# mlvlab/RPO

Measured on AMD Instinct MI355X. Metric: images/sec (train step, ViT-B/16 K=24), higher is better.
Workload: dtype bf16

## Files before the change

### include/rpo_amd.h

```cpp
#ifndef RPO_AMD_H
#define RPO_AMD_H

#include <stddef.h>
#include <stdint.h>

#if defined(__GNUC__)
#pragma GCC visibility push(default)
#endif
#ifdef __cplusplus
extern "C" {
#endif

#define RPO_ABI_VERSION 8

enum { RPO_F32 = 0, RPO_BF16 = 1, RPO_F16 = 2 };

enum {
  RPO_E_BADARG = -1,
  RPO_E_SHAPE = -2,
  RPO_E_DTYPE = -3,
  RPO_E_ALIGN = -4,
  RPO_E_WORKSPACE = -5,
  RPO_E_JPEG_CORRUPT = -20,
  RPO_E_JPEG_PROGRESSIVE = -21,
// ... 33 lines not shown
  int32_t group;
  int32_t split_k;
  int64_t split_stride;
  int32_t tile_config;
  void* out2; int64_t ldout2;
  float* ln_stats;
  const float* ln_colsum;
  float ln_eps;
  int32_t seg_rows0, seg_rows1, seg1_row0;
  int32_t ln_group;
  int32_t aux_dtype;
  const void* prefetch;
  int64_t prefetch_bytes;
  const void* resid_hi; const void* resid_lo; int64_t ldr16;
  void* out_lo;
  int32_t c_row0;
} rpo_gemm_args;

int rpo_version(void);
const char* rpo_error_string(int code);

int rpo_gemm_nt(const rpo_gemm_args* args, void* stream);

int rpo_gemm_ws(const rpo_gemm_args* args, void* stream);
int rpo_gemm_ws_pack(const void* W, int64_t ldw, void* Wp, int N, int K, int dtype, void* stream);
int rpo_gemm_ws_ok(const rpo_gemm_args* args);

int rpo_gemm_stats_group(const rpo_gemm_args* args);

int rpo_gemm_hilo_ok(const rpo_gemm_args* args);

int rpo_gemm_nt_plan(const rpo_gemm_args* args);
int rpo_gemm_ws_plan(const rpo_gemm_args* args);

int rpo_layernorm_fwd(const float* x, int64_t ldx, const float* gamma, const float* beta,
                      void* y, int64_t ldy, int y_dtype, int rows, int d, float eps, void* stream);

int rpo_layernorm_bwd(const void* dy, int dy_dtype, int64_t lddy, const float* x, int64_t ldx,
                      const float* gamma, const float* dres, int64_t lddres,
                      float* dx, int64_t lddx, void* dx_cast, int cast_dtype, int64_t ldcast,
                      int rows, int d, float eps, int dy_splits, int64_t dy_split_stride, void* stream);

int rpo_im2col_patches(const float* img, void* out, int out_dtype, int64_t ldo,
                       int B, int H, int W, int patch, void* stream);

int rpo_img_assemble(float* x, int64_t ldx, const float* cls, const float* pos0,
                     const float* img_prompt, int B, int N, int Kp, int d, void* stream);

int rpo_img_embed_norm(float* x_pre, int64_t ldx, const float* cls, const float* pos0, const float* img_prompt,
                       const float* g_pre, const float* b_pre, float* x0, int64_t ldx0, const float* g1, const float* b1,
                       void* h, int64_t ldh, int h_dtype, int B, int N, int Kp, int d, float eps, void* stream);
int rpo_img_embed_norm_rows(float* x_pre, int64_t ldx, const float* cls, const float* pos0, const float* img_prompt,
                            const float* g_pre, const float* b_pre, float* x0, int64_t ldx0, const float* g1,
                            const float* b1, void* h, int64_t ldh, int h_dtype, int B, int N, int Kp, int d,
                            float eps, int row0, int row1, void* stream);

int rpo_img_embed_norm_grouped(float* x_pre, int64_t ldx, const float* cls, const float* pos0, const float* img_prompt,
                               const float* g_pre, const float* b_pre, float* x0, int64_t ldx0, const float* g1,
                               const float* b1, void* h, int64_t ldh, int h_dtype, int B, int N, int Kp, int d,
                               float eps, int row0, int row1, int images_per_group, int64_t prompt_stride, void* stream);

int rpo_broadcast_rows(const float* src, float* dst, int64_t ld, int groups, int rows, int d, void* stream);

int rpo_reduce_groups(const float* src, int64_t ld, float* out, int groups, int rows, int d, void* stream);

int rpo_broadcast_rows_sets(const float* src, int64_t src_set_stride, float* dst, int64_t ld, int sets, int groups, int rows,
                            int d, void* stream);
int rpo_reduce_groups_sets(const float* src, int64_t ld, float* out, int64_t out_set_stride, int sets, int groups, int rows,
                           int d, void* stream);

int rpo_attn_readonly_fwd(const void* q, const void* k, const void* v, int64_t ld,
                          void* out, int64_t ldo, int dtype, int B, int H, int N, int Kp,
                          float scale, void* stream);
int rpo_attn_readonly_fwd_rows(const void* q, const void* k, const void* v, int64_t ld,
                               void* out, int64_t ldo, int dtype, int B, int H, int N, int Kp, float scale,
                               int q_first, void* stream);

int rpo_attn_prompt_fwd(const void* q_rows, int64_t ldq, const void* k, const void* v, int64_t ldkv,
                        void* out, int64_t ldo, int dtype, int B, int H, int N, int Kp, int sets,
                        const int32_t* first_image, float scale, void* stream);

int rpo_attn_readonly_bwd(const void* q_rows, int64_t ldq, const void* k, const void* v, int64_t ldkv,
                          const void* da, int64_t ldda, void* dq, int64_t lddq, int dtype,
                          int B, int H, int N, int Kp, float scale, void* stream);

int rpo_attn_readonly_bwd_proj(const void* q_rows, int64_t ldq, const void* k, const void* v, int64_t ldkv,
                               const void* dx, int64_t lddx, const void* w_out_t, int64_t ldw, void* dq, int64_t lddq,
                               int dtype, int B, int H, int N, int Kp, float scale, void* stream);

int rpo_text_attn_fwd(const void* q, int64_t ldq, const void* kc, const void* vc, int64_t ldkv,
                      void* out, int64_t ldo, int dtype, const int32_t* len, int n_cls, int rows,
                      int Lmax, int H, int causal, float scale, void* stream);

int rpo_text_attn_bwd(const void* q, int64_t ldq, const void* kc, const void* vc, int64_t ldkv,
                      const void* da, int64_t ldda, void* dq, int64_t lddq, int dtype,
                      const int32_t* len, int n_cls, int rows, int Lmax, int H, float scale, void* stream);

int rpo_text_attn_fwd_shared(const void* q, int64_t ldq, const void* kc, const void* vc, int64_t ldkv,
                             void* out, int64_t ldo, int dtype, const int32_t* len, int n_cls, int n_kv, int rows,
                             int Lmax, int H, float scale, void* stream);
int rpo_text_attn_bwd_shared(const void* q, int64_t ldq, const void* kc, const void* vc, int64_t ldkv,
                             const void* da, int64_t ldda, void* dq, int64_t lddq, int dtype,
                             const int32_t* len, int n_cls, int n_kv, int rows, int Lmax, int H, float scale, void* stream);

int rpo_text_attn_bwd_dense(const void* q, const void* k, const void* v, int64_t ld, const void* d_out, int64_t lddo,
                            void* dq, void* dk, void* dv, int64_t ldd, int dtype, const int32_t* len, int n_cls,
                            int Lmax, int H, float scale, void* stream);

int rpo_metanet_fwd(const float* img_f, const float* w1, const float* b1, const float* w2, const float* b2,
                    float* f_norm, float* hidden, float* bias, int B, int e, int h, int d, void* stream);
int rpo_metanet_bwd(const float* d_bias, const float* f_norm, const float* hidden, const float* w2,
                    float* g_w1, float* g_b1, float* g_w2, float* g_b2, int B, int e, int h, int d, void* stream);

int64_t rpo_head_workspace_floats(int B, int C, int K, int e);
int rpo_head_fwd_bwd(const float* img_f, const float* text_f, const int64_t* label, float scale_exp,
                     float* logits, float* loss, float* d_img_f, float* d_text_f,
                     int B, int C, int K, int e, float* workspace, void* stream);
int rpo_head_fwd_bwd_act(const float* img_f, const float* text_f, const int64_t* label, float scale_exp,
                         float* logits, float* loss, float* d_img_f, float* d_text_f, void* d_img_f_act,
                         void* d_text_f_act, int act_dtype, int B, int C, int K, int e, float* workspace, void* stream);

int rpo_head_fwd_bwd_grouped(const float* img_f, const float* text_f, const int64_t* label, float scale_exp,
                             float* logits, float* loss, float* d_img_f, float* d_text_f,
                             int S, int B, int C, int K, int e, float* workspace, void* stream);
int rpo_head_fwd_bwd_grouped_act(const float* img_f, const float* text_f, const int64_t* label, float scale_exp,
                                 float* logits, float* loss, float* d_img_f, float* d_text_f, void* d_img_f_act,
                                 void* d_text_f_act, int act_dtype, int S, int B, int C, int K, int e, float* workspace,
                                 void* stream);

int64_t rpo_lp_head_workspace_floats(int B, int C, int e);
int rpo_lp_head_fwd_bwd(const float* img_f, const float* w, const float* bias, const float* text_f_n,
                        const int64_t* label, float scale_exp, float* z, float* logits, float* loss,
                        float* g_w, float* g_bias, int B, int C, int e, float* workspace, void* stream);

int rpo_eval_accumulate(const float* logits, int64_t ldl, const int64_t* label, int B, int C, int64_t* counts,
                        int32_t* cmat, int32_t* pred, void* stream);

int rpo_conv2d_plan(int B, int H, int W, int Cout);
int rpo_conv2d_nhwc(const void* x, const void* w, const float* bias, const void* resid, void* y, int dtype,
                    int B, int H, int W, int Cin, int Cout, int ksize, int relu, int tile_config, void* stream);
int rpo_conv_stem(const float* image, const void* w, const float* bias, void* y, int dtype, int B, int H, int W,
                  int Cout, int relu, void* stream);
int rpo_avgpool_nhwc(const void* x, void* y, int dtype, int B, int H, int W, int C, int k, void* stream);
int rpo_attnpool_tokens(const void* x, const float* pos, void* tokens, int dtype, int B, int HW, int C, void* stream);
int rpo_attnpool_attn(const float* q, int64_t ldq, const void* kv, void* out, int dtype, int B, int T, int C, int heads,
                      float scale, void* stream);

int rpo_sgd_step(float* p, const float* g, float* buf, int64_t n, float lr, float momentum, float wd,
                 float grad_scale, int first_step, void* stream);

int rpo_sgd_step_guarded(float* p, const float* g, float* buf, int64_t n, float lr, float momentum, float wd,
                         float grad_scale, int first_step, int32_t* found_inf, void* stream);

int rpo_convert(const float* src, int64_t lds, void* dst, int dst_dtype, int64_t ldd,
                int rows, int cols, void* stream);

int rpo_probe_mfma(int which, const float* a, const float* b, float* d, void* stream);

typedef struct rpo_image_desc {
  int64_t src_offset;
  int32_t width, height;
  int32_t crop_x, crop_y, crop_w, crop_h;
  int32_t resize_w, resize_h;
  int32_t win_x, win_y;
  int32_t flip;
  int32_t reserved;
} rpo_image_desc;

int rpo_preprocess_ksize(int in_size, int out_size);
size_t rpo_preprocess_workspace_bytes(int B, int size, int max_rows, int kmax);
int rpo_preprocess_batch(const uint8_t* src, int64_t src_bytes, const rpo_image_desc* desc_host,
                         const rpo_image_desc* desc_dev, int B, int size, int max_rows, int kmax,
                         const float* mean3, const float* std3, float* out, void* workspace,
                         size_t workspace_bytes, void* stream);

typedef struct rpo_jpeg_info {
  int32_t width, height;
  int32_t components;
  int32_t h_samp, v_samp;
  int32_t restart_interval;
  int32_t mcus_x, mcus_y;
  int32_t units;
  int32_t reserved;
  int64_t scan_offset;
  int64_t scan_bytes;
  int64_t table_bytes;
  int64_t coef_bytes;
} rpo_jpeg_info;

typedef struct rpo_jpeg_desc {
  int64_t file_offset;
  int64_t file_bytes;
  int64_t table_offset;
  int64_t out_offset;
  int64_t coef_offset;
  int32_t unit_base;
  int32_t reserved;
  rpo_jpeg_info info;
} rpo_jpeg_desc;

enum {
  RPO_JPEG_OK = 0,
  RPO_JPEG_TRUNCATED = 1,
  RPO_JPEG_BAD_CODE = 2,
  RPO_JPEG_BAD_INDEX = 3,
  RPO_JPEG_NO_RESTART = 4
};

int rpo_jpeg_probe(const uint8_t* file, int64_t nbytes, rpo_jpeg_info* info);
int rpo_jpeg_tables(const uint8_t* file, int64_t nbytes, void* blob, int64_t blob_bytes);
size_t rpo_jpeg_workspace_bytes(rpo_jpeg_desc* descs, int n);
int rpo_jpeg_decode_batch(const uint8_t* files, int64_t files_bytes, const rpo_jpeg_desc* desc_host,
                          const rpo_jpeg_desc* desc_dev, int n, uint8_t* out, int64_t out_bytes, void* workspace,
                          size_t workspace_bytes, int32_t* status, void* stream);

int rpo_jpeg_prog_probe(const uint8_t* file, int64_t nbytes, rpo_jpeg_info* info);
int rpo_jpeg_prog_plan(const uint8_t* file, int64_t nbytes, void* blob, int64_t blob_bytes);
size_t rpo_jpeg_prog_workspace_bytes(rpo_jpeg_desc* descs, int n);
int rpo_jpeg_prog_decode_batch(const uint8_t* files, int64_t files_bytes, const rpo_jpeg_desc* desc_host,
                               const rpo_jpeg_desc* desc_dev, int n, uint8_t* out, int64_t out_bytes, void* workspace,
                               size_t workspace_bytes, int32_t* status, void* stream);

int rpo_probe_peak_mfma(int which, int blocks, int iters, float* sink, double* flops, void* stream);
int rpo_probe_peak_copy(const void* src, void* dst, int64_t bytes, void* stream);

#ifdef __cplusplus
}
#endif
#if defined(__GNUC__)
#pragma GCC visibility pop
#endif

#ifdef RPO_EXPERIMENTAL
#include "rpo_amd_experimental.h"
#endif
#endif
```

### rpo_amd/_lib.py

```python
from __future__ import annotations

import ctypes as C
import os

_HERE = os.path.dirname(os.path.abspath(__file__))
LIB_PATH = os.path.join(_HERE, "librpo_hip.so")

RPO_F32, RPO_BF16, RPO_F16 = 0, 1, 2
EPI_NONE, EPI_BIAS, EPI_BIAS_QGELU, EPI_BIAS_RESID, EPI_QGELU_BWD, EPI_PATCH, EPI_LN_BIAS, EPI_LN_BIAS_QGELU = range(8)
E_BADARG, E_SHAPE, E_DTYPE, E_ALIGN, E_WORKSPACE = -1, -2, -3, -4, -5
(E_JPEG_CORRUPT, E_JPEG_PROGRESSIVE, E_JPEG_ARITHMETIC, E_JPEG_LOSSLESS, E_JPEG_PRECISION, E_JPEG_COMPONENTS, E_JPEG_RGB,
 E_JPEG_SAMPLING, E_JPEG_MULTISCAN, E_JPEG_SCRIPT, E_JPEG_SEQUENTIAL) = range(-20, -31, -1)

c_i64, c_i32, c_f32, c_vp = C.c_int64, C.c_int32, C.c_float, C.c_void_p


class ImageDesc(C.Structure):
    _fields_ = [("src_offset", c_i64), ("width", c_i32), ("height", c_i32),
                ("crop_x", c_i32), ("crop_y", c_i32), ("crop_w", c_i32), ("crop_h", c_i32),
                ("resize_w", c_i32), ("resize_h", c_i32), ("win_x", c_i32), ("win_y", c_i32),
                ("flip", c_i32), ("reserved", c_i32)]


class JpegInfo(C.Structure):
    _fields_ = [("width", c_i32), ("height", c_i32), ("components", c_i32), ("h_samp", c_i32), ("v_samp", c_i32),
                ("restart_interval", c_i32), ("mcus_x", c_i32), ("mcus_y", c_i32), ("units", c_i32), ("reserved", c_i32),
                ("scan_offset", c_i64), ("scan_bytes", c_i64), ("table_bytes", c_i64), ("coef_bytes", c_i64)]


class JpegDesc(C.Structure):
    _fields_ = [("file_offset", c_i64), ("file_bytes", c_i64), ("table_offset", c_i64), ("out_offset", c_i64),
                ("coef_offset", c_i64), ("unit_base", c_i32), ("reserved", c_i32), ("info", JpegInfo)]


class GemmArgs(C.Structure):
    _fields_ = [
        ("A", c_vp), ("lda", c_i64),
        ("W", c_vp), ("ldw", c_i64),
        ("C", c_vp), ("ldc", c_i64),
        ("M", c_i32), ("N", c_i32), ("K", c_i32),
        ("in_dtype", c_i32), ("out_dtype", c_i32), ("epilogue", c_i32),
        ("bias", c_vp),
        ("resid", c_vp), ("ldr", c_i64),
        ("aux", c_vp), ("ldaux", c_i64),
        ("aux_row0", c_i32),
        ("skip_row0", c_i32), ("skip_col0", c_i32),
        ("group", c_i32),
        ("split_k", c_i32),
        ("split_stride", c_i64),
        ("tile_config", c_i32),
        ("out2", c_vp), ("ldout2", c_i64),
        ("ln_stats", c_vp),
        ("ln_colsum", c_vp),
        ("ln_eps", c_f32),
        ("seg_rows0", c_i32), ("seg_rows1", c_i32), ("seg1_row0", c_i32),
        ("ln_group", c_i32),
        ("aux_dtype", c_i32),
        ("prefetch", c_vp), ("prefetch_bytes", c_i64),
        ("resid_hi", c_vp), ("resid_lo", c_vp), ("ldr16", c_i64),
        ("out_lo", c_vp),
        ("c_row0", c_i32),
    ]


class LnBwdArgs(C.Structure):
    _fields_ = [("dy", c_vp), ("lddy", c_i64), ("x", c_vp), ("ldx", c_i64), ("gamma", c_vp),
                ("dres", c_vp), ("lddres", c_i64), ("dx", c_vp), ("lddx", c_i64),
                ("dx_cast", c_vp), ("cast_dtype", c_i32), ("ldcast", c_i64),
                ("rows", c_i32), ("d", c_i32), ("eps", c_f32), ("dy_splits", c_i32), ("dy_split_stride", c_i64)]


class AttnBwdArgs(C.Structure):
    _fields_ = [("q_rows", c_vp), ("ldq", c_i64), ("k", c_vp), ("v", c_vp), ("ldkv", c_i64),
                ("dx", c_vp), ("lddx", c_i64), ("w_out_t", c_vp), ("ldw", c_i64), ("dq", c_vp), ("lddq", c_i64),
                ("groups", c_i32), ("H", c_i32), ("keys", c_i32), ("Kp", c_i32),
                ("key_len", c_vp), ("key_stride", c_i32), ("scale", c_f32)]


class ChainLayer(C.Structure):
    _fields_ = [("w_proj_t", c_vp), ("w_fc_t", c_vp), ("w_out_t", c_vp), ("w_q_t", c_vp), ("aux", c_vp),
                ("x_ln2", c_vp), ("x_ln1", c_vp), ("ln2_w", c_vp), ("ln1_w", c_vp),
                ("q_rows", c_vp), ("k", c_vp), ("v", c_vp)]


class ChainBwdArgs(C.Structure):
    _fields_ = [("layer", C.POINTER(ChainLayer)),
                ("layers", c_i32), ("units", c_i32), ("Kp", c_i32), ("d", c_i32), ("H", c_i32), ("keys", c_i32),
                ("dtype", c_i32),
                ("key_len", c_vp), ("key_stride", c_i32),
                ("ldx", c_i64), ("ldq", c_i64), ("ldkv", c_i64),
                ("dxa", c_vp), ("dxb", c_vp), ("dxc", c_vp), ("du", c_vp), ("dq", c_vp),
                ("dy", c_vp), ("dy_stride", c_i64),
                ("scale", c_f32), ("eps", c_f32),
                ("wgs_per_group", c_i32),
                ("state", c_vp),
                ("timeline", c_vp)]


SIGNATURES = {
    "rpo_version": (c_i32, []),
    "rpo_gemm_stats_group": (c_i32, [C.POINTER(GemmArgs)]),
    "rpo_gemm_hilo_ok": (c_i32, [C.POINTER(GemmArgs)]),
    "rpo_gemm_nt_plan": (c_i32, [C.POINTER(GemmArgs)]),
    "rpo_gemm_ws_plan": (c_i32, [C.POINTER(GemmArgs)]),
    "rpo_error_string": (C.c_char_p, [c_i32]),
    "rpo_gemm_nt": (c_i32, [C.POINTER(GemmArgs), c_vp]),
    "rpo_gemm_ws": (c_i32, [C.POINTER(GemmArgs), c_vp]),
    "rpo_gemm_ws_pack": (c_i32, [c_vp, c_i64, c_vp, c_i32, c_i32, c_i32, c_vp]),
    "rpo_gemm_ws_ok": (c_i32, [C.POINTER(GemmArgs)]),
    "rpo_layernorm_fwd": (c_i32, [c_vp, c_i64, c_vp, c_vp, c_vp, c_i64, c_i32, c_i32, c_i32, c_f32, c_vp]),
    "rpo_layernorm_bwd": (c_i32, [c_vp, c_i32, c_i64, c_vp, c_i64, c_vp, c_vp, c_i64, c_vp, c_i64, c_vp,
                                  c_i32, c_i64, c_i32, c_i32, c_f32, c_i32, c_i64, c_vp]),
    "rpo_im2col_patches": (c_i32, [c_vp, c_vp, c_i32, c_i64, c_i32, c_i32, c_i32, c_i32, c_vp]),
    "rpo_img_embed_norm": (c_i32, [c_vp, c_i64, c_vp, c_vp, c_vp, c_vp, c_vp, c_vp, c_i64, c_vp, c_vp, c_vp, c_i64, c_i32,
                                   c_i32, c_i32, c_i32, c_i32, c_f32, c_vp]),
    "rpo_img_embed_norm_rows": (c_i32, [c_vp, c_i64, c_vp, c_vp, c_vp, c_vp, c_vp, c_vp, c_i64, c_vp, c_vp, c_vp, c_i64, c_i32,
                                        c_i32, c_i32, c_i32, c_i32, c_f32, c_i32, c_i32, c_vp]),
    "rpo_img_embed_norm_grouped": (c_i32, [c_vp, c_i64, c_vp, c_vp, c_vp, c_vp, c_vp, c_vp, c_i64, c_vp, c_vp, c_vp, c_i64,
                                           c_i32, c_i32, c_i32, c_i32, c_i32, c_f32, c_i32, c_i32, c_i32, c_i64, c_vp]),
    "rpo_img_assemble": (c_i32, [c_vp, c_i64, c_vp, c_vp, c_vp, c_i32, c_i32, c_i32, c_i32, c_vp]),
    "rpo_broadcast_rows": (c_i32, [c_vp, c_vp, c_i64, c_i32, c_i32, c_i32, c_vp]),
    "rpo_reduce_groups": (c_i32, [c_vp, c_i64, c_vp, c_i32, c_i32, c_i32, c_vp]),
    "rpo_broadcast_rows_sets": (c_i32, [c_vp, c_i64, c_vp, c_i64, c_i32, c_i32, c_i32, c_i32, c_vp]),
    "rpo_reduce_groups_sets": (c_i32, [c_vp, c_i64, c_vp, c_i64, c_i32, c_i32, c_i32, c_i32, c_vp]),
    "rpo_attn_readonly_fwd": (c_i32, [c_vp, c_vp, c_vp, c_i64, c_vp, c_i64, c_i32, c_i32, c_i32, c_i32, c_i32,
                                      c_f32, c_vp]),
    "rpo_attn_readonly_fwd_rows": (c_i32, [c_vp, c_vp, c_vp, c_i64, c_vp, c_i64, c_i32, c_i32, c_i32, c_i32, c_i32,
                                      c_f32, c_i32, c_vp]),
    "rpo_attn_prompt_fwd": (c_i32, [c_vp, c_i64, c_vp, c_vp, c_i64, c_vp, c_i64, c_i32, c_i32, c_i32, c_i32, c_i32, c_i32,
                                    c_vp, c_f32, c_vp]),
    "rpo_attn_readonly_bwd_proj": (c_i32, [c_vp, c_i64, c_vp, c_vp, c_i64, c_vp, c_i64, c_vp, c_i64, c_vp, c_i64, c_i32,
                                           c_i32, c_i32, c_i32, c_i32, c_f32, c_vp]),
    "rpo_attn_readonly_bwd": (c_i32, [c_vp, c_i64, c_vp, c_vp, c_i64, c_vp, c_i64, c_vp, c_i64, c_i32, c_i32,
                                      c_i32, c_i32, c_i32, c_f32, c_vp]),
    "rpo_text_attn_fwd": (c_i32, [c_vp, c_i64, c_vp, c_vp, c_i64, c_vp, c_i64, c_i32, c_vp, c_i32, c_i32,
                                  c_i32, c_i32, c_i32, c_f32, c_vp]),
    "rpo_text_attn_bwd": (c_i32, [c_vp, c_i64, c_vp, c_vp, c_i64, c_vp, c_i64, c_vp, c_i64, c_i32, c_vp,
                                  c_i32, c_i32, c_i32, c_i32, c_f32, c_vp]),
    "rpo_text_attn_fwd_shared": (c_i32, [c_vp, c_i64, c_vp, c_vp, c_i64, c_vp, c_i64, c_i32, c_vp, c_i32, c_i32,
                                         c_i32, c_i32, c_i32, c_f32, c_vp]),
    "rpo_text_attn_bwd_shared": (c_i32, [c_vp, c_i64, c_vp, c_vp, c_i64, c_vp, c_i64, c_vp, c_i64, c_i32, c_vp,
                                         c_i32, c_i32, c_i32, c_i32, c_i32, c_f32, c_vp]),
    "rpo_text_attn_bwd_dense": (c_i32, [c_vp, c_vp, c_vp, c_i64, c_vp, c_i64, c_vp, c_vp, c_vp, c_i64, c_i32, c_vp,
                                        c_i32, c_i32, c_i32, c_f32, c_vp]),
    "rpo_metanet_fwd": (c_i32, [c_vp] * 8 + [c_i32] * 4 + [c_vp]),
    "rpo_metanet_bwd": (c_i32, [c_vp] * 8 + [c_i32] * 4 + [c_vp]),
    "rpo_head_workspace_floats": (c_i64, [c_i32, c_i32, c_i32, c_i32]),
    "rpo_head_fwd_bwd": (c_i32, [c_vp, c_vp, c_vp, c_f32, c_vp, c_vp, c_vp, c_vp, c_i32, c_i32, c_i32, c_i32,
                                 c_vp, c_vp]),
    "rpo_head_fwd_bwd_act": (c_i32, [c_vp, c_vp, c_vp, c_f32, c_vp, c_vp, c_vp, c_vp, c_vp, c_vp, c_i32, c_i32, c_i32,
                                     c_i32, c_i32, c_vp, c_vp]),
    "rpo_head_fwd_bwd_grouped": (c_i32, [c_vp, c_vp, c_vp, c_f32, c_vp, c_vp, c_vp, c_vp, c_i32, c_i32, c_i32, c_i32, c_i32,
                                         c_vp, c_vp]),
    "rpo_head_fwd_bwd_grouped_act": (c_i32, [c_vp, c_vp, c_vp, c_f32, c_vp, c_vp, c_vp, c_vp, c_vp, c_vp, c_i32, c_i32,
                                             c_i32, c_i32, c_i32, c_i32, c_vp, c_vp]),
    "rpo_lp_head_workspace_floats": (c_i64, [c_i32, c_i32, c_i32]),
    "rpo_lp_head_fwd_bwd": (c_i32, [c_vp, c_vp, c_vp, c_vp, c_vp, c_f32, c_vp, c_vp, c_vp, c_vp, c_vp, c_i32, c_i32, c_i32,
                                    c_vp, c_vp]),
    "rpo_eval_accumulate": (c_i32, [c_vp, c_i64, c_vp, c_i32, c_i32, c_vp, c_vp, c_vp, c_vp]),
    "rpo_conv2d_plan": (c_i32, [c_i32, c_i32, c_i32, c_i32]),
    "rpo_conv2d_nhwc": (c_i32, [c_vp, c_vp, c_vp, c_vp, c_vp, c_i32, c_i32, c_i32, c_i32, c_i32, c_i32, c_i32, c_i32, c_i32,
                                c_vp]),
    "rpo_conv_stem": (c_i32, [c_vp, c_vp, c_vp, c_vp, c_i32, c_i32, c_i32, c_i32, c_i32, c_i32, c_vp]),
    "rpo_avgpool_nhwc": (c_i32, [c_vp, c_vp, c_i32, c_i32, c_i32, c_i32, c_i32, c_i32, c_vp]),
    "rpo_attnpool_tokens": (c_i32, [c_vp, c_vp, c_vp, c_i32, c_i32, c_i32, c_i32, c_vp]),
    "rpo_attnpool_attn": (c_i32, [c_vp, c_i64, c_vp, c_vp, c_i32, c_i32, c_i32, c_i32, c_i32, c_f32, c_vp]),
    "rpo_sgd_step": (c_i32, [c_vp, c_vp, c_vp, c_i64, c_f32, c_f32, c_f32, c_f32, c_i32, c_vp]),
    "rpo_sgd_step_guarded": (c_i32, [c_vp, c_vp, c_vp, c_i64, c_f32, c_f32, c_f32, c_f32, c_i32, c_vp, c_vp]),
    "rpo_convert": (c_i32, [c_vp, c_i64, c_vp, c_i32, c_i64, c_i32, c_i32, c_vp]),
    "rpo_probe_mfma": (c_i32, [c_i32, c_vp, c_vp, c_vp, c_vp]),
    "rpo_probe_peak_mfma": (c_i32, [c_i32, c_i32, c_i32, c_vp, c_vp, c_vp]),
    "rpo_probe_peak_copy": (c_i32, [c_vp, c_vp, c_i64, c_vp]),
    "rpo_preprocess_ksize": (c_i32, [c_i32, c_i32]),
    "rpo_preprocess_workspace_bytes": (C.c_size_t, [c_i32, c_i32, c_i32, c_i32]),
    "rpo_preprocess_batch": (c_i32, [c_vp, c_i64, c_vp, c_vp, c_i32, c_i32, c_i32, c_i32, c_vp, c_vp, c_vp, c_vp,
                                     C.c_size_t, c_vp]),
    "rpo_jpeg_probe": (c_i32, [c_vp, c_i64, C.POINTER(JpegInfo)]),
    "rpo_jpeg_tables": (c_i32, [c_vp, c_i64, c_vp, c_i64]),
    "rpo_jpeg_workspace_bytes": (C.c_size_t, [C.POINTER(JpegDesc), c_i32]),
    "rpo_jpeg_decode_batch": (c_i32, [c_vp, c_i64, c_vp, c_vp, c_i32, c_vp, c_i64, c_vp, C.c_size_t, c_vp, c_vp]),
    "rpo_jpeg_prog_probe": (c_i32, [c_vp, c_i64, C.POINTER(JpegInfo)]),
    "rpo_jpeg_prog_plan": (c_i32, [c_vp, c_i64, c_vp, c_i64]),
    "rpo_jpeg_prog_workspace_bytes": (C.c_size_t, [C.POINTER(JpegDesc), c_i32]),
    "rpo_jpeg_prog_decode_batch": (c_i32, [c_vp, c_i64, c_vp, c_vp, c_i32, c_vp, c_i64, c_vp, C.c_size_t, c_vp, c_vp]),
}

EXPERIMENTAL_SIGNATURES = {
    "rpo_gemm_nt_pair": (c_i32, [C.POINTER(GemmArgs), C.POINTER(GemmArgs), c_vp]),
    "rpo_mlp_fused": (c_i32, [C.POINTER(GemmArgs), C.POINTER(GemmArgs), c_vp, c_i32, c_vp]),
    "rpo_layernorm_bwd_pair": (c_i32, [C.POINTER(LnBwdArgs), C.POINTER(LnBwdArgs), c_vp]),
    "rpo_attn_bwd_proj_pair": (c_i32, [C.POINTER(AttnBwdArgs), C.POINTER(AttnBwdArgs), c_i32, c_vp]),
    "rpo_chain_state_bytes": (C.c_size_t, []),
    "rpo_chain_bwd": (c_i32, [C.POINTER(ChainBwdArgs), c_vp]),
    "rpo_chain_bwd_ok": (c_i32, [C.POINTER(ChainBwdArgs)]),
}
EXPERIMENTAL = os.environ.get("RPO_EXPERIMENTAL") == "1"


def xenv(name: str, default: str = "0") -> str:
    return os.environ.get(name, default) if EXPERIMENTAL else default

_lib = None


class RPOLibraryError(RuntimeError):
    pass


def load(path: str | None = None):
    global _lib
    if _lib is not None and path is None:
        return _lib
    p = path or os.environ.get("RPO_HIP_LIB")
    if p is None and EXPERIMENTAL:
        from .build import build_library
        p = build_library(experimental=True)
    p = p or LIB_PATH
    import torch
    if not os.path.exists(p):
        raise RPOLibraryError(
            f"{p} not found: build it with `python -m rpo_amd.build` (hipcc, gfx950). "
            "rpo_amd has no CPU fallback.")
    try:
        lib = C.CDLL(p)
    except OSError as e:
        raise RPOLibraryError(f"cannot load {p}: {e}") from e
    for name, (res, args) in SIGNATURES.items():
        try:
            fn = getattr(lib, name)
        except AttributeError as e:
            raise RPOLibraryError(f"{p} does not export {name}") from e
        fn.restype = res
        fn.argtypes = args
    for name, (res, args) in EXPERIMENTAL_SIGNATURES.items():
        fn = getattr(lib, name, None)
        if fn is not None:
            fn.restype = res
            fn.argtypes = args
    if path is None:
        _lib = lib
    return lib


def experimental():
    lib = load()
    if not hasattr(lib, "rpo_chain_bwd"):
        raise RPOLibraryError("this entry point belongs to the measured-slower experiments of rounds 3 / 4: set "
                              "RPO_EXPERIMENTAL=1 (loads rpo_amd/build/librpo_hip_exp.so, built with -DRPO_EXPERIMENTAL)")
    return lib


def check(rc: int, what: str = "") -> None:
    if rc != 0:
        msg = load().rpo_error_string(int(rc))
        raise RPOLibraryError(f"{what or 'rpo call'} failed: {msg.decode() if msg else rc} (code {rc})")
```

### rpo_amd/csrc/common.h

```cpp
#pragma once
#include <hip/hip_runtime.h>
#include <atomic>
#include <stdint.h>

#include "../../include/rpo_amd.h"
#include "../../include/rpo_amd_experimental.h"

typedef uint16_t bf16_t;
struct f16_t { uint16_t v; };
typedef __attribute__((ext_vector_type(8))) __bf16 bf16x8_t;
typedef __attribute__((ext_vector_type(8))) _Float16 f16x8_t;
typedef __attribute__((ext_vector_type(2))) _Float16 f16x2_t;
typedef __attribute__((ext_vector_type(8))) short short8_t;
typedef __attribute__((ext_vector_type(4))) short short4_t;
typedef __attribute__((ext_vector_type(16))) float f32x16_t;
typedef __attribute__((ext_vector_type(4))) float f32x4_t;

#define RPO_WAVE 64

__device__ __forceinline__ float bf16_to_f32(bf16_t v) { return __uint_as_float(((uint32_t)v) << 16); }

typedef __attribute__((ext_vector_type(2))) float f32x2_t;
typedef __attribute__((ext_vector_type(2))) __bf16 bf16x2_t;
__device__ __forceinline__ uint32_t pack_bf16x2(float lo, float hi) {
  const f32x2_t v = {lo, hi};
  return __builtin_bit_cast(uint32_t, __builtin_convertvector(v, bf16x2_t));
}
__device__ __forceinline__ bf16_t f32_to_bf16(float f) { return (bf16_t)(pack_bf16x2(f, 0.0f) & 0xffffu); }

template <typename T> __device__ __forceinline__ uint32_t pack2(float lo, float hi);
template <> __device__ __forceinline__ uint32_t pack2<bf16_t>(float lo, float hi) { return pack_bf16x2(lo, hi); }
template <> __device__ __forceinline__ uint32_t pack2<f16_t>(float lo, float hi) {
  const f32x2_t v = {lo, hi};
  return __builtin_bit_cast(uint32_t, __builtin_convertvector(v, f16x2_t));
}
template <typename T> __device__ __forceinline__ float unpack1(uint16_t bits);
template <> __device__ __forceinline__ float unpack1<bf16_t>(uint16_t bits) { return bf16_to_f32(bits); }
template <> __device__ __forceinline__ float unpack1<f16_t>(uint16_t bits) { return (float)__builtin_bit_cast(_Float16, bits); }
template <typename T> struct One16;
template <> struct One16<bf16_t> { static constexpr uint32_t lo = 0x3F80u, hi = 0x3F800000u; };
template <> struct One16<f16_t> { static constexpr uint32_t lo = 0x3C00u, hi = 0x3C000000u; };
template <typename T> __device__ __forceinline__ f32x16_t mfma16(bf16x8_t a, bf16x8_t b, f32x16_t c);
template <> __device__ __forceinline__ f32x16_t mfma16<bf16_t>(bf16x8_t a, bf16x8_t b, f32x16_t c) {
  return __builtin_amdgcn_mfma_f32_32x32x16_bf16(a, b, c, 0, 0, 0);
}
template <> __device__ __forceinline__ f32x16_t mfma16<f16_t>(bf16x8_t a, bf16x8_t b, f32x16_t c) {
  return __builtin_amdgcn_mfma_f32_32x32x16_f16(__builtin_bit_cast(f16x8_t, a), __builtin_bit_cast(f16x8_t, b), c, 0, 0, 0);
}

template <typename T> struct ActIO;
template <> struct ActIO<float> {
  static __device__ __forceinline__ float ld(const float* p) { return *p; }
  static __device__ __forceinline__ void st(float* p, float v) { *p = v; }
  static __device__ __forceinline__ void st4(float* p, float a, float b, float c, float d) {
    *reinterpret_cast<float4*>(p) = make_float4(a, b, c, d);
  }
};
template <> struct ActIO<bf16_t> {
  static __device__ __forceinline__ float ld(const bf16_t* p) { return bf16_to_f32(*p); }
  static __device__ __forceinline__ void st(bf16_t* p, float v) { *p = f32_to_bf16(v); }
  static __device__ __forceinline__ void st4(bf16_t* p, float a, float b, float c, float d) {
    *reinterpret_cast<uint2*>(p) = make_uint2(pack_bf16x2(a, b), pack_bf16x2(c, d));
  }
};

template <> struct ActIO<f16_t> {
  static __device__ __forceinline__ float ld(const f16_t* p) { return unpack1<f16_t>(p->v); }
  static __device__ __forceinline__ void st(f16_t* p, float v) { p->v = (uint16_t)(pack2<f16_t>(v, 0.0f) & 0xffffu); }
  static __device__ __forceinline__ void st4(f16_t* p, float a, float b, float c, float d) {
    *reinterpret_cast<uint2*>(p) = make_uint2(pack2<f16_t>(a, b), pack2<f16_t>(c, d));
  }
};

__device__ __forceinline__ float wave_sum(float v) {
#pragma unroll
  for (int o = 32; o > 0; o >>= 1) v += __shfl_xor(v, o, 64);
  return v;
}
__device__ __forceinline__ float row16_sum(float v) {
  v += __int_as_float(__builtin_amdgcn_update_dpp(0, __float_as_int(v), 0x128, 0xf, 0xf, false));
  v += __int_as_float(__builtin_amdgcn_update_dpp(0, __float_as_int(v), 0x124, 0xf, 0xf, false));
  v += __int_as_float(__builtin_amdgcn_update_dpp(0, __float_as_int(v), 0x122, 0xf, 0xf, false));
  v += __int_as_float(__builtin_amdgcn_update_dpp(0, __float_as_int(v), 0x121, 0xf, 0xf, false));
  return v;
}
__device__ __forceinline__ float wave_max(float v) {
#pragma unroll
  for (int o = 32; o > 0; o >>= 1) v = fmaxf(v, __shfl_xor(v, o, 64));
  return v;
}

#define RPO_QG 1.702f
#define RPO_QG_L2 (-2.4554669595930156f)
__device__ __forceinline__ float qg_sigmoid(float u) {
  return __builtin_amdgcn_rcpf(1.0f + __builtin_amdgcn_exp2f(RPO_QG_L2 * u));
}
__device__ __forceinline__ float quick_gelu(float u) { return u * qg_sigmoid(u); }
__device__ __forceinline__ float quick_gelu_grad(float u) {
  float s = qg_sigmoid(u);
  return s * fmaf(RPO_QG * u, 1.0f - s, 1.0f);
}
__device__ __forceinline__ float4 quick_gelu4(float4 v) {
  typedef __attribute__((ext_vector_type(2))) float f32x2_t;
  const f32x2_t a = {v.x, v.y}, b = {v.z, v.w};
  const f32x2_t za = a * RPO_QG_L2, zb = b * RPO_QG_L2;
  f32x2_t ea = {__builtin_amdgcn_exp2f(za.x), __builtin_amdgcn_exp2f(za.y)};
  f32x2_t eb = {__builtin_amdgcn_exp2f(zb.x), __builtin_amdgcn_exp2f(zb.y)};
  ea = ea + 1.0f; eb = eb + 1.0f;
  const f32x2_t ra = {__builtin_amdgcn_rcpf(ea.x), __builtin_amdgcn_rcpf(ea.y)};
  const f32x2_t rb = {__builtin_amdgcn_rcpf(eb.x), __builtin_amdgcn_rcpf(eb.y)};
  const f32x2_t oa = a * ra, ob = b * rb;
  return make_float4(oa.x, oa.y, ob.x, ob.y);
}

__device__ __forceinline__ void quick_gelu4_du(const float4 v, float4& o, float4& d) {
  typedef __attribute__((ext_vector_type(2))) float f32x2_t;
  const f32x2_t a = {v.x, v.y}, b = {v.z, v.w};
  const f32x2_t za = a * RPO_QG_L2, zb = b * RPO_QG_L2;
  f32x2_t ea = {__builtin_amdgcn_exp2f(za.x), __builtin_amdgcn_exp2f(za.y)};
  f32x2_t eb = {__builtin_amdgcn_exp2f(zb.x), __builtin_amdgcn_exp2f(zb.y)};
  ea = ea + 1.0f; eb = eb + 1.0f;
  const f32x2_t ra = {__builtin_amdgcn_rcpf(ea.x), __builtin_amdgcn_rcpf(ea.y)};
  const f32x2_t rb = {__builtin_amdgcn_rcpf(eb.x), __builtin_amdgcn_rcpf(eb.y)};
  const f32x2_t oa = a * ra, ob = b * rb;
  const f32x2_t qa = a * RPO_QG, qb = b * RPO_QG;
  const f32x2_t ta = 1.0f - ra, tb = 1.0f - rb;
  const f32x2_t wa = {fmaf(qa.x, ta.x, 1.0f), fmaf(qa.y, ta.y, 1.0f)};
  const f32x2_t wb = {fmaf(qb.x, tb.x, 1.0f), fmaf(qb.y, tb.y, 1.0f)};
  const f32x2_t da = ra * wa, db = rb * wb;
  o = make_float4(oa.x, oa.y, ob.x, ob.y);
  d = make_float4(da.x, da.y, db.x, db.y);
}

template <typename V>
__device__ __forceinline__ void store_out16(V* dst, const V v) {
#if defined(RPO_SC1_STORE)
  typedef __attribute__((ext_vector_type(4))) uint32_t u32x4_wt;
  static_assert(sizeof(V) == 16, "16-byte stores only");
  asm volatile("global_store_dwordx4 %0, %1, off sc1" :: "v"(dst), "v"(__builtin_bit_cast(u32x4_wt, v)) : "memory");
#elif defined(RPO_NT_STORE)
  typedef __attribute__((ext_vector_type(4))) uint32_t u32x4_nt;
  static_assert(sizeof(V) == 16, "16-byte stores only");
  __builtin_nontemporal_store(__builtin_bit_cast(u32x4_nt, v), reinterpret_cast<u32x4_nt*>(dst));
#else
  *dst = v;
#endif
}

__device__ __forceinline__ void store_out8(void* dst, const uint2 v) {
#if defined(RPO_SC1_STORE)
  typedef __attribute__((ext_vector_type(2))) uint32_t u32x2_wt;
  asm volatile("global_store_dwordx2 %0, %1, off sc1" :: "v"(dst), "v"(__builtin_bit_cast(u32x2_wt, v)) : "memory");
#else
  *reinterpret_cast<uint2*>(dst) = v;
#endif
}

using rpo_lds_mask_t = std::atomic<unsigned long long>;
static inline int rpo_allow_lds(const void* kern, int bytes, rpo_lds_mask_t* mask) {
  int dev = 0;
  hipError_t e = hipGetDevice(&dev);
  if (e != hipSuccess) return (int)e;
  const unsigned long long bit = dev < 64 ? 1ull << dev : 0ull;
  if (bit && (mask->load(std::memory_order_relaxed) & bit)) return 0;
  e = hipFuncSetAttribute(kern, hipFuncAttributeMaxDynamicSharedMemorySize, bytes);
  if (e != hipSuccess) return (int)e;
  mask->fetch_or(bit, std::memory_order_relaxed);
  return 0;
}

static inline int rpo_launch_status() {
  hipError_t e = hipGetLastError();
  return e == hipSuccess ? 0 : (int)e;
}

static inline int rpo_cu_count() {
  static std::atomic<int> cached{0};
  int n = cached.load(std::memory_order_relaxed);
  if (n > 0) return n;
  int dev = 0;
  n = 256;
  if (hipGetDevice(&dev) != hipSuccess || hipDeviceGetAttribute(&n, hipDeviceAttributeMultiprocessorCount, dev) != hipSuccess || n <= 0)
    n = 256;
  cached.store(n, std::memory_order_relaxed);
  return n;
}

static inline bool aligned16(const void* p) { return (reinterpret_cast<uintptr_t>(p) & 15u) == 0; }

int rpo_text_attn_wave(int bwd, const void* q, int64_t ldq, const void* kc, const void* vc, int64_t ldkv, const void* da,
                       int64_t ldda, void* out, int64_t ldo, int dtype, const int32_t* len, int n_cls, int n_kv, int rows,
                       int Lmax, int H, float scale, hipStream_t s);

#ifdef RPO_TIMELINE
extern __device__ unsigned long long* g_timeline;
#define RPO_STAMP(slot)                                                                               \
  do {                                                                                                \
    if (g_timeline != nullptr && threadIdx.x == 0 && (blockIdx.x % 97) == 0 && blockIdx.x / 97 < 8)   \
      g_timeline[(blockIdx.x / 97) * 64 + (slot)] = __builtin_amdgcn_s_memtime();                     \
  } while (0)
#define RPO_STAMP_RT(slot)                                                                            \
  do {                                                                                                \
    if (g_timeline != nullptr && threadIdx.x == 0 && (blockIdx.x % 97) == 0 && blockIdx.x / 97 < 8)   \
      g_timeline[(blockIdx.x / 97) * 64 + (slot)] = __builtin_amdgcn_s_memrealtime();                 \
  } while (0)
#else
#define RPO_STAMP(slot) do { } while (0)
#define RPO_STAMP_RT(slot) do { } while (0)
#endif
```

### rpo_amd/csrc/misc.hip

```cpp
#include "common.h"

namespace {

template <typename TO>
__global__ void im2col_kernel(const float* __restrict__ img, TO* out, int64_t ldo, int B, int H, int W,
                              int p, int64_t total) {
  const int64_t idx = (int64_t)blockIdx.x * blockDim.x + threadIdx.x;
  if (idx >= total) return;
  const int w2 = W >> 1;
  const int x = (int)(idx % w2) * 2;
  const int64_t row = idx / w2;
  const int y = (int)(row % H);
  const int c = (int)((row / H) % 3);
  const int b = (int)(row / (3 * (int64_t)H));
  const float2 v = *reinterpret_cast<const float2*>(img + row * W + x);
  const int g = W / p;
  const int py = y / p, ky = y - py * p, px = x / p, kx = x - px * p;
  const int64_t m = ((int64_t)b * (H / p) + py) * g + px;
  TO* dst = out + m * ldo + (c * p + ky) * p + kx;
  ActIO<TO>::st(dst, v.x);
  ActIO<TO>::st(dst + 1, v.y);
  if (c == 2 && ky == p - 1 && kx + 2 >= p)
    for (int k = 3 * p * p; k < ldo; ++k) ActIO<TO>::st(out + m * ldo + k, 0.f);
}

template <typename TO>
__global__ void im2col8_kernel(const float* __restrict__ img, TO* out, int64_t ldo, int B, int H, int W,
                               int p, int64_t total) {
  const int64_t idx = (int64_t)blockIdx.x * blockDim.x + threadIdx.x;
  if (idx >= total) return;
  const int w8 = W >> 3;
  const int x = (int)(idx % w8) * 8;
  const int64_t row = idx / w8;
  const int y = (int)(row % H);
  const int c = (int)((row / H) % 3);
  const int b = (int)(row / (3 * (int64_t)H));
  const float4 v0 = *reinterpret_cast<const float4*>(img + row * W + x);
  const float4 v1 = *reinterpret_cast<const float4*>(img + row * W + x + 4);
  const int g = W / p;
  const int py = y / p, ky = y - py * p, px = x / p, kx = x - px * p;
  const int64_t m = ((int64_t)b * (H / p) + py) * g + px;
  TO* dst = out + m * ldo + (c * p + ky) * p + kx;
  if constexpr (sizeof(TO) == 2) {
    uint4 o;
    o.x = pack2<TO>(v0.x, v0.y); o.y = pack2<TO>(v0.z, v0.w);
    o.z = pack2<TO>(v1.x, v1.y); o.w = pack2<TO>(v1.z, v1.w);
    *reinterpret_cast<uint4*>(dst) = o;
  } else {
    *reinterpret_cast<float4*>(dst) = v0;
    *reinterpret_cast<float4*>(dst + 4) = v1;
  }
  if (c == 2 && ky == p - 1 && kx + 8 >= p)
    for (int k = 3 * p * p; k < ldo; ++k) ActIO<TO>::st(out + m * ldo + k, 0.f);
}

__global__ void assemble_kernel(float* x, int64_t ldx, const float* __restrict__ cls,
                                const float* __restrict__ pos0, const float* __restrict__ prompt, int B, int N,
                                int Kp, int d) {
  const int r = blockIdx.x;
  float* dst;
  if (r < B) {
    dst = x + (int64_t)r * N * ldx;
    for (int i = threadIdx.x; i < d; i += blockDim.x) dst[i] = cls[i] + pos0[i];
  } else {
    const int pr = r - B;
    dst = x + ((int64_t)B * N + pr) * ldx;
    const float* src = prompt + (int64_t)(pr % Kp) * d;
    for (int i = threadIdx.x; i < d; i += blockDim.x) dst[i] = src[i];
  }
}

__global__ void broadcast_rows_kernel(const float* __restrict__ src, float* dst, int64_t ld, int rows, int d,
                                      int set_rows, int64_t src_stride) {
  const int r = blockIdx.x;
  const float* s = src + (int64_t)(r / set_rows) * src_stride + (int64_t)(r % rows) * d;
  float* o = dst + (int64_t)r * ld;
  for (int i = threadIdx.x; i < d; i += blockDim.x) o[i] = s[i];
}

__global__ void reduce_groups_kernel(const float* __restrict__ src, int64_t ld, float* out, int groups, int rows,
                                     int d, int64_t out_stride) {
  src += (int64_t)blockIdx.y * groups * rows * ld;
  out += (int64_t)blockIdx.y * out_stride;
  const int idx = blockIdx.x * blockDim.x + threadIdx.x;
  if (idx >= rows * d) return;
  const int i = idx / d, c = idx % d;
  float s = 0.f;
  for (int g = 0; g < groups; ++g) s += src[((int64_t)g * rows + i) * ld + c];
  out[idx] = s;
}

__global__ __launch_bounds__(256) void reduce_groups_wide_kernel(const float* __restrict__ src, int64_t ld, float* out,
                                                                 int groups, int rows, int d, int64_t out_stride) {
  __shared__ float part[8][32];
  src += (int64_t)blockIdx.y * groups * rows * ld;
  out += (int64_t)blockIdx.y * out_stride;
  const int cols = (d + 31) / 32;
  const int i = blockIdx.x / cols, c = (blockIdx.x % cols) * 32 + (threadIdx.x & 31), j = threadIdx.x >> 5;
  float s = 0.f;
  if (c < d)
    for (int g = j; g < groups; g += 8) s += src[((int64_t)g * rows + i) * ld + c];
  part[j][threadIdx.x & 31] = s;
  __syncthreads();
  if (j == 0 && c < d) {
    float t = part[0][threadIdx.x];
#pragma unroll
    for (int k = 1; k < 8; ++k) t += part[k][threadIdx.x];
    out[(int64_t)i * d + c] = t;
  }
}

__global__ void sgd_kernel(float* p, const float* __restrict__ g, float* buf, int64_t n, float lr, float mom,
                           float wd, float gs, int first) {
  const int64_t i = (int64_t)blockIdx.x * blockDim.x + threadIdx.x;
  if (i >= n) return;
  const float pi = p[i];
  const float gi = gs * g[i] + wd * pi;
  const float bi = first ? gi : mom * buf[i] + gi;
  buf[i] = bi;
  p[i] = pi - lr * bi;
}

__global__ __launch_bounds__(1024) void sgd_guarded_kernel(float* p, const float* __restrict__ g, float* buf, int64_t n,
                                                           float lr, float mom, float wd, float gs, int first,
                                                           int32_t* found) {
  __shared__ int bad;
  if (threadIdx.x == 0) bad = 0;
  __syncthreads();
  int mine = 0;
  for (int64_t i = threadIdx.x; i < n; i += 1024) {
    const float gi = g[i];
    mine |= !(fabsf(gi) <= 3.402823466e38f);
  }
  if (mine) bad = 1;
  __syncthreads();
  const int skip = bad;
  if (threadIdx.x == 0) { found[0] = skip; found[1] += skip; }
  if (skip) return;
  for (int64_t i = threadIdx.x; i < n; i += 1024) {
    const float pi = p[i];
    const float gi = gs * g[i] + wd * pi;
    const float bi = first ? gi : mom * buf[i] + gi;
    buf[i] = bi;
    p[i] = pi - lr * bi;
  }
}

template <typename TO>
__global__ void convert_kernel(const float* __restrict__ src, int64_t lds, TO* dst, int64_t ldd, int rows,
                               int cols) {
  const int64_t idx = (int64_t)blockIdx.x * blockDim.x + threadIdx.x;
  if (idx >= (int64_t)rows * cols) return;
  const int64_t r = idx / cols, c = idx % cols;
  ActIO<TO>::st(dst + r * ldd + c, src[r * lds + c]);
}

__device__ __forceinline__ float block_sum(float v, float* red) {
  v = wave_sum(v);
  const int lane = threadIdx.x & 63, wave = threadIdx.x >> 6;
  __syncthreads();
  if (lane == 0) red[wave] = v;
  __syncthreads();
  return (red[0] + red[1]) + (red[2] + red[3]);
}
__device__ __forceinline__ float block_max(float v, float* red) {
  v = wave_max(v);
  const int lane = threadIdx.x & 63, wave = threadIdx.x >> 6;
  __syncthreads();
  if (lane == 0) red[wave] = v;
  __syncthreads();
  return fmaxf(fmaxf(red[0], red[1]), fmaxf(red[2], red[3]));
}

struct HeadGroups {
  int64_t img;
  int64_t txt;
  int64_t bc;
  int64_t lab;
  int64_t ws;
};
template <typename T> __device__ __forceinline__ T* head_shift(T* p, int64_t off) { return p == nullptr ? p : p + off; }
__device__ __forceinline__ void* head_shift16(void* p, int64_t off) {
  return p == nullptr ? p : static_cast<void*>(static_cast<uint16_t*>(p) + off);
}

template <bool VEC>
__global__ __launch_bounds__(256) void head_logits_kernel(const float* __restrict__ f_img, const float* __restrict__ f_txt,
                                                          float* ni, float* nt, float* logits, int C, int K, int e,
                                                          float mul, HeadGroups hg) {
  __shared__ float red[4];
  {
    const int64_t s = blockIdx.z;
    f_img += s * hg.img; f_txt += s * hg.txt; ni += s * hg.ws; nt += s * hg.ws; logits += s * hg.bc;
  }
  const int c = blockIdx.x, b = blockIdx.y;
  const int lane = threadIdx.x & 63, wave = threadIdx.x >> 6;
  float acc = 0.f;
#pragma unroll 2
  for (int i = wave; i < K; i += 4) {
    const float* x = f_img + ((int64_t)b * K + i) * e;
    const float* t = f_txt + ((int64_t)c * K + i) * e;
    float dot = 0.f, sx = 0.f, st = 0.f;
    if constexpr (VEC) {
      float4 xv[4], tv[4];
      const int nv = e >> 8;
#pragma unroll
      for (int j = 0; j < 4; ++j)
        if (j < nv) {
          xv[j] = *reinterpret_cast<const float4*>(x + j * 256 + lane * 4);
          tv[j] = *reinterpret_cast<const float4*>(t + j * 256 + lane * 4);
        }
#pragma unroll
      for (int j = 0; j < 4; ++j)
        if (j < nv) {
          dot += xv[j].x * tv[j].x + xv[j].y * tv[j].y + xv[j].z * tv[j].z + xv[j].w * tv[j].w;
          sx += xv[j].x * xv[j].x + xv[j].y * xv[j].y + xv[j].z * xv[j].z + xv[j].w * xv[j].w;
          st += tv[j].x * tv[j].x + tv[j].y * tv[j].y + tv[j].z * tv[j].z + tv[j].w * tv[j].w;
        }
    } else {
      for (int idx = lane; idx < e; idx += 64) {
        const float xv = x[idx], tv = t[idx];
        dot = fmaf(xv, tv, dot); sx = fmaf(xv, xv, sx); st = fmaf(tv, tv, st);
      }
    }
    dot = wave_sum(dot); sx = wave_sum(sx); st = wave_sum(st);
    const float ix = 1.0f / sqrtf(sx), it = 1.0f / sqrtf(st);
    acc += dot * ix * it;
    if (lane == 0) {
      if (c == 0) ni[(int64_t)b * K + i] = ix;
      if (b == 0) nt[(int64_t)c * K + i] = it;
    }
  }
  if (lane == 0) red[wave] = acc;
  __syncthreads();
  if (threadIdx.x == 0) logits[(int64_t)b * C + c] = ((red[0] + red[1]) + (red[2] + red[3])) * mul;
}

__global__ __launch_bounds__(256) void head_ce_kernel(const float* __restrict__ logits,
                                                      const int64_t* __restrict__ label, float* dl,
                                                      float* loss_b, int C, float gmul, float* dlT, int B,
                                                      HeadGroups hg) {
  __shared__ float red[4];
  {
    const int64_t s = blockIdx.y;
    logits += s * hg.bc; label += s * hg.lab; dl += s * hg.ws; loss_b += s * hg.ws; dlT = head_shift(dlT, s * hg.ws);
  }
  const int b = blockIdx.x;
  const float* z = logits + (int64_t)b * C;
  float m = -INFINITY;
  for (int c = threadIdx.x; c < C; c += 256) m = fmaxf(m, z[c]);
  m = block_max(m, red);
  float s = 0.f;
  for (int c = threadIdx.x; c < C; c += 256) s += expf(z[c] - m);
  s = block_sum(s, red);
  const int64_t lb64 = label[b];
  const bool lb_ok = lb64 >= 0 && lb64 < C;
  const int lb = lb_ok ? (int)lb64 : -1;
  const float inv = 1.0f / s;
  const float poison = lb_ok ? 0.0f : __builtin_nanf("");
  for (int c = threadIdx.x; c < C; c += 256) {
    const float w = (expf(z[c] - m) * inv - (c == lb ? 1.0f : 0.0f)) * gmul + poison;
    dl[(int64_t)b * C + c] = w;
    if (dlT != nullptr) dlT[(int64_t)c * B + b] = w;
  }
  if (threadIdx.x == 0) loss_b[b] = lb_ok ? (m + logf(s)) - z[lb] : __builtin_nanf("");
}

template <bool FUSED_CE>
__global__ __launch_bounds__(256) void head_bwd_kernel(const float* __restrict__ dl, const float* __restrict__ f_img,
                                                       const float* __restrict__ ni, const float* __restrict__ f_txt,
                                                       const float* __restrict__ nt, float* d_img_f, float* d_text_f,
                                                       int B, int C, int K, int e, const float* loss_b, float* loss,
                                                       const float* __restrict__ logits,
                                                       const int64_t* __restrict__ label, float gmul,
                                                       void* d_img_a, void* d_text_a, int act_dtype, HeadGroups hg) {
  extern __shared__ __attribute__((aligned(16))) char head_smem[];
  __shared__ float red[4];
  {
    const int64_t s = blockIdx.y;
    dl += s * hg.ws; ni += s * hg.ws; nt += s * hg.ws; loss_b += s * hg.ws;
    f_img += s * hg.img; f_txt += s * hg.txt; d_img_f += s * hg.img; d_text_f += s * hg.txt;
    d_img_a = head_shift16(d_img_a, s * hg.img); d_text_a = head_shift16(d_text_a, s * hg.txt);
    logits += s * hg.bc; label = head_shift(label, s * hg.lab); loss = head_shift(loss, s);
  }
  const int lane = threadIdx.x & 63, wave = threadIdx.x >> 6;
  const bool img = (int)blockIdx.x < B * K;
  const int row = img ? blockIdx.x : blockIdx.x - B * K;
  const int g = row / K, i = row % K;
  const float* self_raw = img ? f_img : f_txt;
  const float* self_inv = img ? ni : nt;
  const float* other_raw = img ? f_txt : f_img;
  const float* other_inv = img ? nt : ni;
  float* df = img ? d_img_f : d_text_f;
  const int n_other = img ? C : B;
  float* wts = reinterpret_cast<float*>(head_smem);
  if constexpr (FUSED_CE) {
    float* smax = wts + max(B, C);
// ... 718 lines not shown
```

### rpo_amd/csrc/norm.hip

```cpp
#include "common.h"

#ifndef RPO_LN_RPB
#define RPO_LN_RPB 1
#endif

namespace {

constexpr int MAXV = 8;

template <typename TY, int NV>
__global__ __launch_bounds__(64 * RPO_LN_RPB) void ln_fwd_kernel(const float* __restrict__ x, int64_t ldx,
                                                     const float* __restrict__ gamma,
                                                     const float* __restrict__ beta, TY* y, int64_t ldy,
                                                     int rows, int d, float eps) {
  const int lane = threadIdx.x & 63;
  const int row = blockIdx.x * RPO_LN_RPB + (threadIdx.x >> 6);
  if (row >= rows) return;
  const int nv4 = d >> 2;
  const float* xr = x + (int64_t)row * ldx;
  float4 v[NV], gm[NV], bt[NV];
  float s = 0.f;
#pragma unroll
  for (int i = 0; i < NV; ++i) {
    const int c = lane + 64 * i;
    v[i] = make_float4(0.f, 0.f, 0.f, 0.f);
    if (c < nv4) {
      v[i] = *reinterpret_cast<const float4*>(xr + 4 * c);
      gm[i] = *reinterpret_cast<const float4*>(gamma + 4 * c);
      bt[i] = *reinterpret_cast<const float4*>(beta + 4 * c);
      s += (v[i].x + v[i].y) + (v[i].z + v[i].w);
    }
  }
  const float mu = wave_sum(s) / (float)d;
  float q = 0.f;
#pragma unroll
  for (int i = 0; i < NV; ++i) {
    const int c = lane + 64 * i;
    if (c < nv4) {
      const float a = v[i].x - mu, b = v[i].y - mu, cc = v[i].z - mu, dd = v[i].w - mu;
      q += (a * a + b * b) + (cc * cc + dd * dd);
    }
  }
  const float rstd = rsqrtf(wave_sum(q) / (float)d + eps);
  TY* yr = y + (int64_t)row * ldy;
#pragma unroll
  for (int i = 0; i < NV; ++i) {
    const int c = lane + 64 * i;
    if (c < nv4) {
      const float4 g = gm[i], b = bt[i];
      ActIO<TY>::st4(yr + 4 * c, (v[i].x - mu) * rstd * g.x + b.x, (v[i].y - mu) * rstd * g.y + b.y,
                     (v[i].z - mu) * rstd * g.z + b.z, (v[i].w - mu) * rstd * g.w + b.w);
    }
  }
}

template <typename TY, int NV>
__global__ __launch_bounds__(64 * RPO_LN_RPB) void img_embed_norm_kernel(float* x_pre, int64_t ldx,
    const float* __restrict__ cls, const float* __restrict__ pos0, const float* __restrict__ prompt,
    const float* __restrict__ g_pre, const float* __restrict__ b_pre, float* x0, int64_t ldx0,
    const float* __restrict__ g1, const float* __restrict__ b1, TY* h, int64_t ldh, int B, int N, int Kp, int d,
    float eps, int row0, int row1, int ipg, int64_t pstride) {
  const int lane = threadIdx.x & 63;
  const int row = row0 + blockIdx.x * RPO_LN_RPB + (threadIdx.x >> 6);
  if (row >= row1) return;
  const int nv4 = d >> 2;
  const bool is_prompt = row >= B * N;
  const bool is_cls = !is_prompt && row % N == 0;
  const int pr = is_prompt ? row - B * N : 0;
  const float* src = is_prompt ? prompt + (int64_t)(pr / Kp / ipg) * pstride + (int64_t)(pr % Kp) * d
                               : (is_cls ? cls : x_pre + (int64_t)row * ldx);
  float4 v[NV], ga[NV], ba[NV], gb[NV], bb[NV];
  float s = 0.f;
#pragma unroll
  for (int i = 0; i < NV; ++i) {
    const int c = lane + 64 * i;
    v[i] = make_float4(0.f, 0.f, 0.f, 0.f);
    if (c < nv4) {
      v[i] = *reinterpret_cast<const float4*>(src + 4 * c);
      if (is_cls) {
        const float4 p4 = *reinterpret_cast<const float4*>(pos0 + 4 * c);
        v[i].x += p4.x; v[i].y += p4.y; v[i].z += p4.z; v[i].w += p4.w;
      }
      ga[i] = *reinterpret_cast<const float4*>(g_pre + 4 * c); ba[i] = *reinterpret_cast<const float4*>(b_pre + 4 * c);
      gb[i] = *reinterpret_cast<const float4*>(g1 + 4 * c);    bb[i] = *reinterpret_cast<const float4*>(b1 + 4 * c);
      if (is_cls || is_prompt) *reinterpret_cast<float4*>(x_pre + (int64_t)row * ldx + 4 * c) = v[i];
      s += (v[i].x + v[i].y) + (v[i].z + v[i].w);
    }
  }
  auto norm = [&](float4 (&g)[NV], float4 (&b)[NV], float ssum) {
    const float mu = wave_sum(ssum) / (float)d;
    float q = 0.f;
#pragma unroll
    for (int i = 0; i < NV; ++i) {
      const int c = lane + 64 * i;
      if (c < nv4) {
        const float a = v[i].x - mu, b2 = v[i].y - mu, cc = v[i].z - mu, dd = v[i].w - mu;
        q += (a * a + b2 * b2) + (cc * cc + dd * dd);
      }
    }
    const float rstd = rsqrtf(wave_sum(q) / (float)d + eps);
    float sn = 0.f;
#pragma unroll
    for (int i = 0; i < NV; ++i) {
      const int c = lane + 64 * i;
      if (c < nv4) {
        v[i] = make_float4((v[i].x - mu) * rstd * g[i].x + b[i].x, (v[i].y - mu) * rstd * g[i].y + b[i].y,
                           (v[i].z - mu) * rstd * g[i].z + b[i].z, (v[i].w - mu) * rstd * g[i].w + b[i].w);
        sn += (v[i].x + v[i].y) + (v[i].z + v[i].w);
      }
    }
    return sn;
  };
  const float s1 = norm(ga, ba, s);
#pragma unroll
  for (int i = 0; i < NV; ++i) {
    const int c = lane + 64 * i;
    if (c < nv4) *reinterpret_cast<float4*>(x0 + (int64_t)row * ldx0 + 4 * c) = v[i];
  }
  (void)norm(gb, bb, s1);
#pragma unroll
  for (int i = 0; i < NV; ++i) {
    const int c = lane + 64 * i;
    if (c < nv4) ActIO<TY>::st4(h + (int64_t)row * ldh + 4 * c, v[i].x, v[i].y, v[i].z, v[i].w);
  }
}

template <typename T> __device__ __forceinline__ float4 load4f(const T* p);
template <> __device__ __forceinline__ float4 load4f<float>(const float* p) {
  return *reinterpret_cast<const float4*>(p);
}
template <> __device__ __forceinline__ float4 load4f<bf16_t>(const bf16_t* p) {
  const uint2 u = *reinterpret_cast<const uint2*>(p);
  return make_float4(__uint_as_float(u.x << 16), __uint_as_float(u.x & 0xffff0000u),
                     __uint_as_float(u.y << 16), __uint_as_float(u.y & 0xffff0000u));
}

template <> __device__ __forceinline__ float4 load4f<f16_t>(const f16_t* p) {
  const uint2 u = *reinterpret_cast<const uint2*>(p);
  return make_float4(unpack1<f16_t>((uint16_t)(u.x & 0xffffu)), unpack1<f16_t>((uint16_t)(u.x >> 16)),
                     unpack1<f16_t>((uint16_t)(u.y & 0xffffu)), unpack1<f16_t>((uint16_t)(u.y >> 16)));
}

template <typename TDY, typename TC, int NV>
__device__ __forceinline__ void ln_bwd_row(const TDY* __restrict__ dy, int64_t lddy,
                                           const float* __restrict__ x, int64_t ldx,
                                           const float* __restrict__ gamma,
                                           const float* __restrict__ dres, int64_t lddres,
                                           float* dx, int64_t lddx, TC* dxc, int64_t ldc,
                                           int rows, int d, float eps, int splits,
                                           int64_t split_stride, const int blk) {
  const int lane = threadIdx.x & 63;
  const int row = blk * RPO_LN_RPB + (threadIdx.x >> 6);
  if (row >= rows) return;
  const int nv4 = d >> 2;
  const float* xr = x + (int64_t)row * ldx;
  const TDY* dyr = dy + (int64_t)row * lddy;
  float4 v[NV], g[NV];
#pragma unroll
  for (int i = 0; i < NV; ++i) {
    const int c = lane + 64 * i;
    v[i] = make_float4(0.f, 0.f, 0.f, 0.f);
    g[i] = make_float4(0.f, 0.f, 0.f, 0.f);
    if (c < nv4) {
      v[i] = *reinterpret_cast<const float4*>(xr + 4 * c);
      const float4 w = *reinterpret_cast<const float4*>(gamma + 4 * c);
      float4 t = load4f<TDY>(dyr + 4 * c);
      float4 ts[3];
#pragma unroll
      for (int sp = 1; sp < 4; ++sp) ts[sp - 1] = load4f<TDY>(dyr + (int64_t)min(sp, splits - 1) * split_stride + 4 * c);
#pragma unroll
      for (int sp = 1; sp < 4; ++sp) {
        const float m = sp < splits ? 1.0f : 0.0f;
        t.x = fmaf(m, ts[sp - 1].x, t.x); t.y = fmaf(m, ts[sp - 1].y, t.y);
        t.z = fmaf(m, ts[sp - 1].z, t.z); t.w = fmaf(m, ts[sp - 1].w, t.w);
      }
      for (int sp = 4; sp < splits; ++sp) {
        const float4 t2 = load4f<TDY>(dyr + (int64_t)sp * split_stride + 4 * c);
        t.x += t2.x; t.y += t2.y; t.z += t2.z; t.w += t2.w;
      }
      g[i] = make_float4(t.x * w.x, t.y * w.y, t.z * w.z, t.w * w.w);
    }
  }
  float4 rr[NV];
#pragma unroll
  for (int i = 0; i < NV; ++i) {
    const int c = lane + 64 * i;
    rr[i] = make_float4(0.f, 0.f, 0.f, 0.f);
    if (dres != nullptr && c < nv4) rr[i] = *reinterpret_cast<const float4*>(dres + (int64_t)row * lddres + 4 * c);
  }
  float s = 0.f;
#pragma unroll
  for (int i = 0; i < NV; ++i) s += (v[i].x + v[i].y) + (v[i].z + v[i].w);
  const float mu = wave_sum(s) / (float)d;
  float q = 0.f;
#pragma unroll
  for (int i = 0; i < NV; ++i) {
    const int c = lane + 64 * i;
    if (c < nv4) {
      v[i].x -= mu; v[i].y -= mu; v[i].z -= mu; v[i].w -= mu;
      q += (v[i].x * v[i].x + v[i].y * v[i].y) + (v[i].z * v[i].z + v[i].w * v[i].w);
    }
  }
  const float rstd = rsqrtf(wave_sum(q) / (float)d + eps);
  float sg = 0.f, sgx = 0.f;
#pragma unroll
  for (int i = 0; i < NV; ++i) {
    const int c = lane + 64 * i;
    if (c < nv4) {
      v[i].x *= rstd; v[i].y *= rstd; v[i].z *= rstd; v[i].w *= rstd;
      sg += (g[i].x + g[i].y) + (g[i].z + g[i].w);
      sgx += (g[i].x * v[i].x + g[i].y * v[i].y) + (g[i].z * v[i].z + g[i].w * v[i].w);
    }
  }
  const float mg = wave_sum(sg) / (float)d;
  const float mgx = wave_sum(sgx) / (float)d;
#pragma unroll
  for (int i = 0; i < NV; ++i) {
    const int c = lane + 64 * i;
    if (c < nv4) {
      float4 o = make_float4(rstd * (g[i].x - mg - v[i].x * mgx), rstd * (g[i].y - mg - v[i].y * mgx),
                             rstd * (g[i].z - mg - v[i].z * mgx), rstd * (g[i].w - mg - v[i].w * mgx));
      o.x += rr[i].x; o.y += rr[i].y; o.z += rr[i].z; o.w += rr[i].w;
      *reinterpret_cast<float4*>(dx + (int64_t)row * lddx + 4 * c) = o;
      if (dxc != nullptr) ActIO<TC>::st4(dxc + (int64_t)row * ldc + 4 * c, o.x, o.y, o.z, o.w);
    }
  }
}

template <typename TDY, typename TC, int NV>
__global__ __launch_bounds__(64 * RPO_LN_RPB) void ln_bwd_kernel(const TDY* __restrict__ dy, int64_t lddy,
                                                     const float* __restrict__ x, int64_t ldx,
                                                     const float* __restrict__ gamma,
                                                     const float* __restrict__ dres, int64_t lddres,
                                                     float* dx, int64_t lddx, TC* dxc, int64_t ldc,
                                                     int rows, int d, float eps, int splits,
                                                     int64_t split_stride) {
  ln_bwd_row<TDY, TC, NV>(dy, lddy, x, ldx, gamma, dres, lddres, dx, lddx, dxc, ldc, rows, d, eps, splits, split_stride,
                          blockIdx.x);
}

struct LnBwdProblem {
  const float* dy; int64_t lddy; const float* x; int64_t ldx; const float* gamma; const float* dres; int64_t lddres;
  float* dx; int64_t lddx; void* dxc; int64_t ldc; int rows, d; float eps; int splits; int64_t split_stride;
};
struct LnBwdPair { LnBwdProblem p[2]; int blocks0; };
template <typename TC, int NV>
__global__ __launch_bounds__(64 * RPO_LN_RPB) void ln_bwd_pair_kernel(const LnBwdPair g) {
  const int second = (int)blockIdx.x >= g.blocks0;
  const LnBwdProblem& q = g.p[second];
  ln_bwd_row<float, TC, NV>(q.dy, q.lddy, q.x, q.ldx, q.gamma, q.dres, q.lddres, q.dx, q.lddx, static_cast<TC*>(q.dxc),
                            q.ldc, q.rows, q.d, q.eps, q.splits, q.split_stride,
                            second ? (int)blockIdx.x - g.blocks0 : (int)blockIdx.x);
}

}

extern "C" int rpo_layernorm_fwd(const float* x, int64_t ldx, const float* gamma, const float* beta,
                                 void* y, int64_t ldy, int y_dtype, int rows, int d, float eps,
                                 void* stream) {
  if (!x || !gamma || !beta || !y || rows <= 0 || d <= 0) return RPO_E_BADARG;
  if (d % 4 != 0 || d > 64 * 4 * MAXV) return RPO_E_SHAPE;
  if (!aligned16(x) || !aligned16(gamma) || !aligned16(beta) || ldx % 4 != 0 || ldy % 4 != 0) return RPO_E_ALIGN;
  hipStream_t s = static_cast<hipStream_t>(stream);
  const dim3 grid((rows + RPO_LN_RPB - 1) / RPO_LN_RPB), block(64 * RPO_LN_RPB);
  const int nv = (d / 4 + 63) / 64;
#define RPO_LN_FWD(TY, NV)                                                                          \
  hipLaunchKernelGGL((ln_fwd_kernel<TY, NV>), grid, block, 0, s, x, ldx, gamma, beta, static_cast<TY*>(y), \
                     ldy, rows, d, eps)
#define RPO_LN_FWD_NV(TY)                                                                           \
  do {                                                                                              \
    if (nv <= 2) RPO_LN_FWD(TY, 2); else if (nv == 3) RPO_LN_FWD(TY, 3);                            \
    else if (nv == 4) RPO_LN_FWD(TY, 4); else RPO_LN_FWD(TY, 8);                                    \
  } while (0)
  if (y_dtype == RPO_F32) {
    if (!aligned16(y)) return RPO_E_ALIGN;
    RPO_LN_FWD_NV(float);
  } else if (y_dtype == RPO_BF16) {
    if (reinterpret_cast<uintptr_t>(y) % 8) return RPO_E_ALIGN;
    RPO_LN_FWD_NV(bf16_t);
  } else if (y_dtype == RPO_F16) {
    if (reinterpret_cast<uintptr_t>(y) % 8) return RPO_E_ALIGN;
    RPO_LN_FWD_NV(f16_t);
  } else {
    return RPO_E_DTYPE;
  }
#undef RPO_LN_FWD_NV
#undef RPO_LN_FWD
  return rpo_launch_status();
}

static int ln_bwd_check(const void* dy, int dy_dtype, int64_t lddy, const float* x, int64_t ldx, const float* gamma,
                        const float* dres, int64_t lddres, float* dx, int64_t lddx, void* dx_cast, int64_t ldcast, int rows,
                        int d, int& dy_splits, int64_t dy_split_stride) {
  if (!dy || !x || !gamma || !dx || rows <= 0 || d <= 0) return RPO_E_BADARG;
  if (d % 4 != 0 || d > 64 * 4 * MAXV) return RPO_E_SHAPE;
  if (dy_splits < 1) dy_splits = 1;
  if (dy_splits > 1 && (dy_dtype != RPO_F32 || dy_split_stride % 4 != 0)) return RPO_E_SHAPE;
  if (!aligned16(x) || !aligned16(gamma) || !aligned16(dx) || ldx % 4 || lddx % 4 || lddy % 4) return RPO_E_ALIGN;
  if (dres && (!aligned16(dres) || lddres % 4)) return RPO_E_ALIGN;
  if (dx_cast && (reinterpret_cast<uintptr_t>(dx_cast) % 8 || ldcast % 4)) return RPO_E_ALIGN;
  if (reinterpret_cast<uintptr_t>(dy) % (dy_dtype == RPO_F32 ? 16 : 8)) return RPO_E_ALIGN;
  return 0;
}

#ifdef RPO_EXPERIMENTAL
extern "C" int rpo_layernorm_bwd_pair(const rpo_ln_bwd_args* a0, const rpo_ln_bwd_args* a1, void* stream) {
  if (!a0 || !a1) return RPO_E_BADARG;
  LnBwdPair g;
  int nv = 0;
  for (int i = 0; i < 2; ++i) {
    const rpo_ln_bwd_args* a = i ? a1 : a0;
    int splits = a->dy_splits;
    if (int rc = ln_bwd_check(a->dy, RPO_F32, a->lddy, a->x, a->ldx, a->gamma, a->dres, a->lddres, a->dx, a->lddx,
                              a->dx_cast, a->ldcast, a->rows, a->d, splits, a->dy_split_stride)) return rc;
    g.p[i] = LnBwdProblem{a->dy, a->lddy, a->x, a->ldx, a->gamma, a->dres, a->lddres, a->dx, a->lddx, a->dx_cast,
                          a->ldcast, a->rows, a->d, a->eps, splits, a->dy_split_stride};
    { const int n = (a->d / 4 + 63) / 64; if (n > nv) nv = n; }
  }
  const int cast = a0->dx_cast ? a0->cast_dtype : (a1->dx_cast ? a1->cast_dtype : RPO_F32);
  if ((a0->dx_cast && a0->cast_dtype != cast) || (a1->dx_cast && a1->cast_dtype != cast)) return RPO_E_DTYPE;
  if (cast != RPO_F32 && cast != RPO_BF16 && cast != RPO_F16) return RPO_E_DTYPE;
  g.blocks0 = (a0->rows + RPO_LN_RPB - 1) / RPO_LN_RPB;
  const dim3 grid(g.blocks0 + (a1->rows + RPO_LN_RPB - 1) / RPO_LN_RPB), block(64 * RPO_LN_RPB);
  hipStream_t s = static_cast<hipStream_t>(stream);
#define RPO_LN_PAIR_(TC, NV) hipLaunchKernelGGL((ln_bwd_pair_kernel<TC, NV>), grid, block, 0, s, g)
#define RPO_LN_PAIR(TC)                                                                                    \
  do {                                                                                                     \
    if (nv <= 2) RPO_LN_PAIR_(TC, 2); else if (nv == 3) RPO_LN_PAIR_(TC, 3);                               \
    else if (nv == 4) RPO_LN_PAIR_(TC, 4); else RPO_LN_PAIR_(TC, 8);                                       \
  } while (0)
  if (cast == RPO_BF16) RPO_LN_PAIR(bf16_t); else if (cast == RPO_F16) RPO_LN_PAIR(f16_t); else RPO_LN_PAIR(float);
#undef RPO_LN_PAIR
#undef RPO_LN_PAIR_
  return rpo_launch_status();
}
#endif

extern "C" int rpo_layernorm_bwd(const void* dy, int dy_dtype, int64_t lddy, const float* x, int64_t ldx,
                                 const float* gamma, const float* dres, int64_t lddres, float* dx,
                                 int64_t lddx, void* dx_cast, int cast_dtype, int64_t ldcast, int rows,
                                 int d, float eps, int dy_splits, int64_t dy_split_stride, void* stream) {
  if (int rc = ln_bwd_check(dy, dy_dtype, lddy, x, ldx, gamma, dres, lddres, dx, lddx, dx_cast, ldcast, rows, d, dy_splits,
                            dy_split_stride)) return rc;
  hipStream_t s = static_cast<hipStream_t>(stream);
  const dim3 grid((rows + RPO_LN_RPB - 1) / RPO_LN_RPB), block(64 * RPO_LN_RPB);
  const int nv = (d / 4 + 63) / 64;
#define RPO_LN_BWD_(TDY, TC, NV)                                                                          \
  hipLaunchKernelGGL((ln_bwd_kernel<TDY, TC, NV>), grid, block, 0, s, static_cast<const TDY*>(dy), lddy, \
                     x, ldx, gamma, dres, lddres, dx, lddx, static_cast<TC*>(dx_cast), ldcast, rows,     \
                     d, eps, dy_splits, dy_split_stride)
#define RPO_LN_BWD(TDY, TC)                                                                    \
  do {                                                                                         \
    if (nv <= 2) RPO_LN_BWD_(TDY, TC, 2); else if (nv == 3) RPO_LN_BWD_(TDY, TC, 3);           \
    else if (nv == 4) RPO_LN_BWD_(TDY, TC, 4); else RPO_LN_BWD_(TDY, TC, 8);                   \
  } while (0)
  const bool cast_bf16 = dx_cast != nullptr && cast_dtype == RPO_BF16;
  const bool cast_f16 = dx_cast != nullptr && cast_dtype == RPO_F16;
  if (dx_cast != nullptr && cast_dtype != RPO_BF16 && cast_dtype != RPO_F16 && cast_dtype != RPO_F32) return RPO_E_DTYPE;
  if (dy_dtype == RPO_F32) {
    if (cast_bf16) RPO_LN_BWD(float, bf16_t); else if (cast_f16) RPO_LN_BWD(float, f16_t); else RPO_LN_BWD(float, float);
  } else if (dy_dtype == RPO_BF16) {
    if (cast_bf16) RPO_LN_BWD(bf16_t, bf16_t); else RPO_LN_BWD(bf16_t, float);
  } else if (dy_dtype == RPO_F16) {
    if (cast_f16) RPO_LN_BWD(f16_t, f16_t); else RPO_LN_BWD(f16_t, float);
  } else {
    return RPO_E_DTYPE;
  }
#undef RPO_LN_BWD
#undef RPO_LN_BWD_
  return rpo_launch_status();
}

extern "C" int rpo_img_embed_norm(float* x_pre, int64_t ldx, const float* cls, const float* pos0, const float* img_prompt,
                                  const float* g_pre, const float* b_pre, float* x0, int64_t ldx0, const float* g1,
                                  const float* b1, void* h, int64_t ldh, int h_dtype, int B, int N, int Kp, int d,
                                  float eps, void* stream) {
  return rpo_img_embed_norm_rows(x_pre, ldx, cls, pos0, img_prompt, g_pre, b_pre, x0, ldx0, g1, b1, h, ldh, h_dtype, B, N, Kp,
                                 d, eps, 0, B * (N + Kp), stream);
}

extern "C" int rpo_img_embed_norm_rows(float* x_pre, int64_t ldx, const float* cls, const float* pos0,
                                       const float* img_prompt, const float* g_pre, const float* b_pre, float* x0,
                                       int64_t ldx0, const float* g1, const float* b1, void* h, int64_t ldh, int h_dtype,
                                       int B, int N, int Kp, int d, float eps, int row0, int row1, void* stream) {
  return rpo_img_embed_norm_grouped(x_pre, ldx, cls, pos0, img_prompt, g_pre, b_pre, x0, ldx0, g1, b1, h, ldh, h_dtype, B, N,
                                    Kp, d, eps, row0, row1, B, (int64_t)Kp * d, stream);
}

extern "C" int rpo_img_embed_norm_grouped(float* x_pre, int64_t ldx, const float* cls, const float* pos0,
                                          const float* img_prompt, const float* g_pre, const float* b_pre, float* x0,
                                          int64_t ldx0, const float* g1, const float* b1, void* h, int64_t ldh,
                                          int h_dtype, int B, int N, int Kp, int d, float eps, int row0, int row1,
                                          int images_per_group, int64_t prompt_stride, void* stream) {
  if (!x_pre || !cls || !pos0 || !g_pre || !b_pre || !x0 || !g1 || !b1 || !h || B <= 0 || N <= 0 || Kp < 0 || d <= 0 ||
      row0 < 0 || row1 > B * (N + Kp) || row0 >= row1 || (Kp > 0 && row1 > B * N && !img_prompt) ||
      images_per_group <= 0 || prompt_stride < 0) return RPO_E_BADARG;
  if (d % 4 != 0 || d > 64 * 4 * 4 || B % images_per_group != 0 ||
      (B > images_per_group && prompt_stride < (int64_t)Kp * d)) return RPO_E_SHAPE;
  if (B > images_per_group && prompt_stride % 4 != 0) return RPO_E_ALIGN;
  if (!aligned16(x_pre) || !aligned16(cls) || !aligned16(pos0) || (Kp > 0 && !aligned16(img_prompt)) || !aligned16(g_pre) ||
      !aligned16(b_pre) || !aligned16(x0) || !aligned16(g1) || !aligned16(b1) || ldx % 4 != 0 || ldx0 % 4 != 0 ||
      ldh % 4 != 0 || reinterpret_cast<uintptr_t>(h) % (h_dtype == RPO_F32 ? 16 : 8)) return RPO_E_ALIGN;
  hipStream_t s = static_cast<hipStream_t>(stream);
  const int rows = row1 - row0;
  const dim3 grid((rows + RPO_LN_RPB - 1) / RPO_LN_RPB), block(64 * RPO_LN_RPB);
  const int nv = (d / 4 + 63) / 64;
#define RPO_IEN(TY, NV)                                                                                       \
  hipLaunchKernelGGL((img_embed_norm_kernel<TY, NV>), grid, block, 0, s, x_pre, ldx, cls, pos0, img_prompt, g_pre, \
                     b_pre, x0, ldx0, g1, b1, static_cast<TY*>(h), ldh, B, N, Kp, d, eps, row0, row1, images_per_group, prompt_stride)
#define RPO_IEN_NV(TY) do { if (nv <= 2) RPO_IEN(TY, 2); else if (nv == 3) RPO_IEN(TY, 3); else RPO_IEN(TY, 4); } while (0)
  if (h_dtype == RPO_F32) RPO_IEN_NV(float);
  else if (h_dtype == RPO_BF16) RPO_IEN_NV(bf16_t);
  else if (h_dtype == RPO_F16) RPO_IEN_NV(f16_t);
  else return RPO_E_DTYPE;
#undef RPO_IEN_NV
#undef RPO_IEN
  return rpo_launch_status();
}
```

### rpo_amd/engine.py

```python
from __future__ import annotations

import math
from dataclasses import dataclass
from typing import Dict, List, Optional

import numpy as np
import torch

from . import ops
import os

from ._lib import (EPI_BIAS, EPI_BIAS_QGELU, EPI_BIAS_RESID, EPI_LN_BIAS, EPI_LN_BIAS_QGELU, EPI_NONE, EPI_PATCH,
                   EPI_QGELU_BWD)
from .config import RPOConfig
from .engine_coop import CoopEngineMixin
from .engine_lp import LpEngineMixin
from .engine_multi import MultiEngineMixin
from .engine_prompt_rows import PromptRowsEngineMixin
from .engine_rn import RnEngineMixin

import contextlib

SCALE = 1.0 / math.sqrt(64.0)
_NO_PROBE = contextlib.nullcontext()


SPLIT_FC, SPLIT_Q = 3, 2


def _round_up(x: int, m: int) -> int:
    return (x + m - 1) // m * m


@dataclass
class _Block:
    ln1_w: torch.Tensor; ln1_b: torch.Tensor; ln2_w: torch.Tensor; ln2_b: torch.Tensor
    w_in: torch.Tensor; b_in: torch.Tensor
    w_out: torch.Tensor; b_out: torch.Tensor
    w_fc: torch.Tensor; b_fc: torch.Tensor
    w_proj: torch.Tensor; b_proj: torch.Tensor
    w_q_t: torch.Tensor
    w_out_t: torch.Tensor
    w_fc_t: torch.Tensor
    w_proj_t: torch.Tensor
    w_oq_t: Optional[torch.Tensor] = None
    w_in_ln: Optional[torch.Tensor] = None; s_in: Optional[torch.Tensor] = None; b_in_ln: Optional[torch.Tensor] = None
    w_fc_ln: Optional[torch.Tensor] = None; s_fc: Optional[torch.Tensor] = None; b_fc_ln: Optional[torch.Tensor] = None


class Engine(CoopEngineMixin, LpEngineMixin, RnEngineMixin, MultiEngineMixin, PromptRowsEngineMixin):
    def __init__(self, cfg: RPOConfig, state_dict: Dict[str, np.ndarray], tokens: np.ndarray,
                 device: torch.device, act_dtype: torch.dtype = torch.bfloat16, max_batch: int = 32):
        if not torch.cuda.is_available():
            raise RuntimeError("rpo_amd.Engine needs a HIP device; there is no CPU path")
        ops.version()
        device = torch.device(device)
        if device.index is None:
            device = torch.device("cuda", torch.cuda.current_device())
        self.cfg, self.dev, self.act = cfg, device, act_dtype
        self.max_batch = max_batch
        self.kmult = 32 if act_dtype == torch.float32 else 64
        self.fold_ln = act_dtype != torch.float32 and os.environ.get("RPO_NO_LN_FOLD") != "1"
        self._pf_chains = (act_dtype != torch.float32 and os.environ.get("RPO_NO_WPREFETCH") != "1"
                           and os.environ.get("RPO_NO_CHAIN_PREFETCH") != "1")
        self.use_ws = act_dtype != torch.float32 and os.environ.get("RPO_NO_WS") != "1"
        self._wsp: Dict[tuple, "ops.PackedWeight"] = {}
        self._ws_okc: Dict[tuple, bool] = {}
        self._ws_cfg = 0
        big = max_batch * (cfg.n_frozen + cfg.K) >= 6000
        self._ws_text_cfg = int(os.environ.get("RPO_WS_TEXT_CFG", "220" if big else "0"))
        self._text_tiles = dict((k, int(v)) for k, v in (kv.split("=") for kv in os.environ.get("RPO_WS_TEXT_TILES", "").split(",") if kv))
        self._ws_text_cfg_bwd = int(os.environ.get("RPO_WS_TEXT_CFG_BWD", os.environ.get("RPO_WS_TEXT_CFG", "120" if big else "0")))
        self._text_fc_units = self._text_fc_units_for(cfg.n_cls * cfg.K)
        tokens = np.asarray(tokens, dtype=np.int64)
        assert tokens.shape == (cfg.n_cls, cfg.context)
        self.len_np = tokens.argmax(-1) + 1
        assert int(self.len_np.max()) + cfg.K <= cfg.context, "len_c + K must fit the context (rpo.py:176)"
        self.Lmax = int(self.len_np.max())
        self.len_i32 = torch.tensor(self.len_np, dtype=torch.int32, device=device)
        self.logit_scale_exp = float(np.exp(np.float32(state_dict["logit_scale"])))
        with torch.cuda.device(device):
            self._pack(state_dict, tokens)
            self._alloc()
        self.text_cache_ready = False
        self._stats_group = {}
        self.img_cls_f = self.rn_img_f if cfg.is_rn else None
        self.plain_text_f = None
        self.text_x_final = None
        self._eval_graphs = {}
        self.probe = None
        self.text_f_version = -1
        self.params_version = 0

    def _f32(self, a: np.ndarray) -> torch.Tensor:
        return torch.from_numpy(np.ascontiguousarray(a, dtype=np.float32)).to(self.dev)

    def _act(self, w: torch.Tensor) -> torch.Tensor:
        w = w.contiguous()
        if self.act == torch.float32:
            return w
        out = torch.empty(w.shape, dtype=self.act, device=self.dev)
        return ops.convert(w, out)

    def _fold(self, w: np.ndarray, b: np.ndarray, gamma: np.ndarray, beta: np.ndarray):
        w64, g64 = np.asarray(w, dtype=np.float64), np.asarray(gamma, dtype=np.float64)
        wq = torch.from_numpy((w64 * g64[None, :]).astype(np.float32)).to(self.act)
        s = wq.double().sum(1).float()
        bq = torch.from_numpy((np.asarray(b, dtype=np.float64) + w64 @ np.asarray(beta, dtype=np.float64)).astype(np.float32))
        return wq.contiguous().to(self.dev), s.contiguous().to(self.dev), bq.contiguous().to(self.dev)

    def _block(self, sd, p: str, fold: bool = False) -> _Block:
        g = lambda k: self._f32(sd[p + k])
        w_in, w_out, w_fc, w_proj = g("attn.in_proj_weight"), g("attn.out_proj.weight"), g("mlp.c_fc.weight"), g("mlp.c_proj.weight")
        d = w_out.shape[0]
        extra = {}
        if fold:
            extra["w_in_ln"], extra["s_in"], extra["b_in_ln"] = self._fold(
                sd[p + "attn.in_proj_weight"], sd[p + "attn.in_proj_bias"], sd[p + "ln_1.weight"], sd[p + "ln_1.bias"])
            extra["w_fc_ln"], extra["s_fc"], extra["b_fc_ln"] = self._fold(
                sd[p + "mlp.c_fc.weight"], sd[p + "mlp.c_fc.bias"], sd[p + "ln_2.weight"], sd[p + "ln_2.bias"])
        return _Block(**extra, **dict(
            ln1_w=g("ln_1.weight"), ln1_b=g("ln_1.bias"), ln2_w=g("ln_2.weight"), ln2_b=g("ln_2.bias"),
            w_in=self._act(w_in), b_in=g("attn.in_proj_bias"), w_out=self._act(w_out), b_out=g("attn.out_proj.bias"),
            w_fc=self._act(w_fc), b_fc=g("mlp.c_fc.bias"), w_proj=self._act(w_proj), b_proj=g("mlp.c_proj.bias"),
            w_fc_t=self._act(w_fc.t()), w_proj_t=self._act(w_proj.t()), **self._oq_t(w_out, w_in[:d])))

    def _oq_t(self, w_out: torch.Tensor, w_q: torch.Tensor) -> dict:
        d = w_out.shape[0]
        if not self.use_ws:
            both = torch.empty(2, d, d, dtype=self.act, device=self.dev)
            both[0].copy_(self._act(w_out.t()))
            both[1].copy_(self._act(w_q.t()))
            return dict(w_out_t=both[0], w_q_t=both[1], w_oq_t=both)
        both = torch.empty(4, d, d, dtype=self.act, device=self.dev)
        both[0].copy_(self._act(w_q.t()))
        both[1].copy_(self._act(w_out.t()))
        for src, dst in ((0, 2), (1, 3)):
            pw = ops.gemm_ws_pack(both[src])
            both[dst].view(-1).copy_(pw.data)
            self._wsp[(both[src].data_ptr(), (d, d))] = ops.PackedWeight(both[dst].view(-1), d, d)
        return dict(w_out_t=both[1], w_q_t=both[0], w_oq_t=both)

    def _tt(self, name: str) -> dict:
        return {"tile_config": self._text_tiles[name]} if name in self._text_tiles else {}

    def _oq_hint(self, blk: _Block, fold_out: bool, ws: bool = True) -> torch.Tensor:
        if not self.use_ws:
            return blk.w_oq_t
        if not ws:
            return blk.w_oq_t[0:2]
        return blk.w_oq_t[1:3] if fold_out else blk.w_oq_t[2:4]

    def _ws_reg(self, w: Optional[torch.Tensor]) -> None:
        if not self.use_ws or w is None or w.dim() != 2 or w.dtype != self.act or w.stride(1) != 1:
            return
        N, K = w.shape
        key = (w.data_ptr(), (N, K))
        if key in self._wsp or N % 32 != 0 or K % 64 != 0:
            return
        self._wsp[key] = ops.gemm_ws_pack(w)

    def _gemm(self, a: torch.Tensor, w: torch.Tensor, out: torch.Tensor, epilogue: int = EPI_NONE, **kw) -> torch.Tensor:
        pw = self._wsp.get((w.data_ptr(), tuple(w.shape))) if self.use_ws else None
        if pw is not None:
            M, split = a.shape[0], kw.get("split_k", 1)
            key = (M, pw.N, pw.K, out.dtype, epilogue, split, kw.get("ln_stats") is not None and epilogue == EPI_BIAS_RESID)
            ok = self._ws_okc.get(key)
            if ok is None:
                ok = self._ws_okc[key] = (M < 2048 and ops.gemm_ws_ok(M, pw.N, pw.K, self.act, out.dtype, epilogue, split, key[-1]))
            if ok:
                kws = dict(kw)
                if self._ws_cfg and "tile_config" not in kws:
                    kws["tile_config"] = self._ws_cfg
                pf = kws.get("prefetch")
                if pf is not None:
                    kws["prefetch"] = self._wsp.get((pf.data_ptr(), tuple(pf.shape)), pf)
                if ops.gemm_ws_try(a, pw, out, epilogue, **kws):
                    return out
                kw.pop("tile_config", None)
        return ops.gemm_nt(a, w, out, epilogue, **kw)

    def _pack(self, sd, tokens) -> None:
        cfg = self.cfg
        self.vis = [] if cfg.is_rn else [self._block(sd, f"visual.transformer.resblocks.{l}.", fold=self.fold_ln)
                                         for l in range(cfg.layers_v)]
        self.txt = [self._block(sd, f"transformer.resblocks.{l}.", fold=self.fold_ln) for l in range(cfg.layers_t)]
        for blk in self.vis + self.txt:
            self._ws_reg(blk.w_proj_t); self._ws_reg(blk.w_fc_t)
        for blk, d in [(b, cfg.d_t) for b in self.txt] + ([(self.vis[-1], cfg.d_v)] if self.vis else []):
            for w in (blk.w_in[:d], None if blk.w_in_ln is None else blk.w_in_ln[:d], blk.w_out, blk.w_fc, blk.w_fc_ln, blk.w_proj):
                self._ws_reg(w)
        if cfg.is_rn:
            self._rn_pack(sd)
        else:
            self._pack_vit_embed(sd)
        self.ln_final = (self._f32(sd["ln_final.weight"]), self._f32(sd["ln_final.bias"]))
        tp = self._f32(sd["text_projection"])
        self.text_proj_t, self.text_proj = self._act(tp.t()), self._act(tp)
        for w in (self.text_proj_t, self.text_proj):
            self._ws_reg(w)
        self.ws_small = (self.use_ws and self.max_batch * (cfg.n_frozen + cfg.K) < 1024 and os.environ.get("RPO_WS_SMALL", "1") != "0")
        if self.ws_small:
            for blk in self.vis:
                for w in (blk.w_in, blk.w_in_ln, blk.w_out, blk.w_fc, blk.w_fc_ln, blk.w_proj):
                    self._ws_reg(w)
        tx = sd["token_embedding.weight"][tokens] + sd["positional_embedding"][None]
        self.text_x_frozen = self._f32(tx[:, :self.Lmax].reshape(cfg.n_cls * self.Lmax, cfg.d_t))
        self.text_pos = self._f32(sd["positional_embedding"][:self.Lmax])
        self.text_tok = self._f32(sd["token_embedding.weight"][tokens][:, :self.Lmax].reshape(cfg.n_cls * self.Lmax, cfg.d_t))

    def _pack_vit_embed(self, sd) -> None:
        cfg = self.cfg
        self.kpatch = _round_up(cfg.patch_dim, self.kmult)
        conv = torch.zeros(cfg.d_v, self.kpatch, device=self.dev)
        conv[:, :cfg.patch_dim] = self._f32(sd["visual.conv1.weight"]).reshape(cfg.d_v, -1)
        self.conv_w = self._act(conv)
        self.cls = self._f32(sd["visual.class_embedding"])
        self.pos = self._f32(sd["visual.positional_embedding"])
        self.ln_pre = (self._f32(sd["visual.ln_pre.weight"]), self._f32(sd["visual.ln_pre.bias"]))
        self.ln_post = (self._f32(sd["visual.ln_post.weight"]), self._f32(sd["visual.ln_post.bias"]))
        vp = self._f32(sd["visual.proj"])
        self.img_proj_t, self.img_proj = self._act(vp.t()), self._act(vp)
        for w in (self.img_proj_t, self.img_proj):
            self._ws_reg(w)

    def _alloc(self) -> None:
        cfg, dev, act = self.cfg, self.dev, self.act
        B, N, K, dv, dt, e = self.max_batch, cfg.n_frozen, cfg.K, cfg.d_v, cfg.d_t, cfg.embed
        R, Rp = B * (N + K), B * K
        f32 = lambda *s: torch.empty(*s, dtype=torch.float32, device=dev)
        a = lambda *s: torch.empty(*s, dtype=act, device=dev)
        Lv, Lt = cfg.layers_v, cfg.layers_t
        au = f32 if os.environ.get("RPO_AUX_F32") == "1" else a
        if cfg.is_rn:
            self._rn_alloc()
        else:
            self.im2col = a(B * cfg.n_patches, self.kpatch)
            self.x_pre = f32(R, dv)
            self.x = [f32(R, dv) for _ in range(Lv + 1)]
            self.xm = [f32(R, dv) for _ in range(Lv)]
            self.h = a(R, dv)
            self.h_lo = a(R, dv)
            self.ln_stats = f32(R, dv // 64, 2)
            self.qkv = [a(R, 3 * dv) for _ in range(Lv)]
            self.att = a(R, dv)
            self.g = a(R, 4 * dv)
            self.u = [au(Rp, 4 * dv) for _ in range(Lv)]
            self.y_post = a(Rp, dv)
            self.img_f = f32(Rp, e)
            self.d_img_f = f32(Rp, e)
            self.d_img_f_a = a(Rp, e)
            self.dy_v = f32(max(SPLIT_FC, SPLIT_Q, 4), Rp, dv)
            self.dxa_v, self.dxb_v = f32(Rp, dv), f32(Rp, dv)
            self.dxc_v = a(Rp, dv)
            self.du_v = a(Rp, 4 * dv)
            self.da_v, self.dq_v = a(Rp, dv), a(Rp, dv)
        Rt = cfg.n_cls * K
        self.Rt = Rt
        self.xt = [f32(Rt, dt) for _ in range(Lt + 1)]
        self.xtm = [f32(Rt, dt) for _ in range(Lt)]
        self.ht = a(Rt, dt)
        self.qt = [a(Rt, dt) for _ in range(Lt)]
        self.att_t = a(Rt, dt)
        self.gt = a(Rt, 4 * dt)
        self.ut = [au(Rt, 4 * dt) for _ in range(Lt)]
        self.y_final = a(Rt, dt)
        self.text_f = f32(Rt, e)
        self.d_text_f = f32(Rt, e)
        self.d_text_f_a = a(Rt, e)
        self.ln_stats_t = f32(Rt, dt // 64, 2)
        self.dy_t = f32(max(SPLIT_FC, SPLIT_Q, 4), Rt, dt)
        self.dxa_t, self.dxb_t = f32(Rt, dt), f32(Rt, dt)
        self.dxc_t = a(Rt, dt)
        self.du_t = a(Rt, 4 * dt)
        self.da_t, self.dq_t = a(Rt, dt), a(Rt, dt)
        self.kv_t = [a(cfg.n_cls * self.Lmax, 2 * dt) for _ in range(Lt)]
        self.logits = f32(B, cfg.n_cls)
        self.loss = f32(1)
        self.head_ws = f32(ops.head_workspace_floats(B, cfg.n_cls, K, e))
        nt, ni = K * dt, K * dv
        self.params = f32(nt + ni)
        self.grads = torch.zeros(nt + ni, dtype=torch.float32, device=dev)
        self.mom = torch.zeros(nt + ni, dtype=torch.float32, device=dev)
        self.text_prompt = self.params[:nt].view(K, dt)
        self.img_prompt = self.params[nt:].view(K, dv)
        self.g_text = self.grads[:nt].view(K, dt)
        self.g_img = self.grads[nt:].view(K, dv)
        self.g_text_flat, self.g_img_flat = self.grads[:nt], self.grads[nt:]
        self.side = torch.cuda.Stream(device=dev)

    def hbm_bytes(self) -> int:
        tot = 0
        for v in vars(self).values():
            ts = v if isinstance(v, (list, tuple)) else [v]
            for t in ts:
                if isinstance(t, torch.Tensor) and t.is_cuda:
                    tot += t.numel() * t.element_size()
        return tot

    def cache_text_kv(self) -> None:
        cfg, act = self.cfg, self.act
        n, L, dt, H = cfg.n_cls, self.Lmax, cfg.d_t, cfg.heads_t
        Rf = n * L
        x = self.text_x_frozen.clone()
        xm = torch.empty_like(x)
        h = torch.empty(Rf, dt, dtype=act, device=self.dev)
        qkv = torch.empty(Rf, 3 * dt, dtype=act, device=self.dev)
        att = torch.empty(Rf, dt, dtype=act, device=self.dev)
        g = torch.empty(Rf, 4 * dt, dtype=act, device=self.dev)
        for l, blk in enumerate(self.txt):
            ops.layernorm_fwd(x, blk.ln1_w, blk.ln1_b, h)
            ops.gemm_nt(h, blk.w_in, qkv, EPI_BIAS, bias=blk.b_in)
            ops.text_attn_fwd(qkv[:, :dt], qkv[:, dt:2 * dt], qkv[:, 2 * dt:], att, self.len_i32, n, L, L, H,
                              causal=True, scale=SCALE)
            self.kv_t[l].copy_(qkv[:, dt:])
            ops.gemm_nt(att, blk.w_out, xm, EPI_BIAS_RESID, bias=blk.b_out, resid=x)
            ops.layernorm_fwd(xm, blk.ln2_w, blk.ln2_b, h)
            ops.gemm_nt(h, blk.w_fc, g, EPI_BIAS_QGELU, bias=blk.b_fc, aux=None, aux_row0=Rf)
            ops.gemm_nt(g, blk.w_proj, x, EPI_BIAS_RESID, bias=blk.b_proj, resid=xm)
        self.text_x_final = x
        self.plain_text_f = None
        self.text_cache_ready = True

    def _timed(self, name: str):
        return _NO_PROBE if self.probe is None else self.probe(name)

    def _text_forward(self, train: bool) -> None:
        self._ws_cfg = self._ws_text_cfg
        try:
            self._text_forward_(train)
        finally:
            self._ws_cfg = 0

    def _text_forward_(self, train: bool) -> None:
        cfg = self.cfg
        n, K, dt, H, Rt = cfg.n_cls, cfg.K, cfg.d_t, cfg.heads_t, self.Rt
        if self._multi: self._m_text_embed(n)
        else: ops.broadcast_rows(self.text_prompt, self.xt[0], n)
        fold, st, last = self.fold_ln and os.environ.get("RPO_NO_TEXT_FOLD") != "1", self.ln_stats_t, len(self.txt) - 1
        pf = self._pf_chains
        nxt_q = lambda l: ((self.txt[l + 1].w_in_ln if fold else self.txt[l + 1].w_in)[:dt] if (pf and l < last) else None)
        for l, blk in enumerate(self.txt):
            kv = self.kv_t[l]
            if fold and l > 0:
                self._gemm(self.ht, blk.w_in_ln[:dt], self.qt[l], EPI_LN_BIAS, bias=blk.b_in_ln[:dt], ln_stats=st,
                            ln_colsum=blk.s_in[:dt], prefetch=blk.w_out if pf else None, **self._tt("q"))
            else:
                ops.layernorm_fwd(self.xt[l], blk.ln1_w, blk.ln1_b, self.ht)
                self._gemm(self.ht, blk.w_in[:dt], self.qt[l], EPI_BIAS, bias=blk.b_in[:dt],
                            prefetch=blk.w_out if pf else None)
            if self._multi: self._m_text_attn(l, None, None)
            else: ops.text_attn_fwd(self.qt[l], kv[:, :dt], kv[:, dt:], self.att_t, self.len_i32, n, K, self.Lmax, H,
                                    causal=False, scale=SCALE)
            prod = dict(out2=self.ht, ln_stats=st) if fold else {}
            self._gemm(self.att_t, blk.w_out, self.xtm[l], EPI_BIAS_RESID, bias=blk.b_out, resid=self.xt[l], **prod,
                        prefetch=(blk.w_fc_ln if fold else blk.w_fc) if pf else None, **self._tt("out"))
            if fold:
                self._gemm(self.ht, blk.w_fc_ln, self.gt, EPI_LN_BIAS_QGELU, bias=blk.b_fc_ln,
                            aux=self.ut[l] if train else None, aux_row0=0, ln_stats=st, ln_colsum=blk.s_fc,
                            prefetch=blk.w_proj if pf else None, **self._tt("fc"), **self._text_fc_units)
            else:
                ops.layernorm_fwd(self.xtm[l], blk.ln2_w, blk.ln2_b, self.ht)
                self._gemm(self.ht, blk.w_fc, self.gt, EPI_BIAS_QGELU, bias=blk.b_fc,
                            aux=self.ut[l] if train else None, aux_row0=0, prefetch=blk.w_proj if pf else None)
            prod = dict(out2=self.ht, ln_stats=st) if (fold and l < last) else {}
            self._gemm(self.gt, blk.w_proj, self.xt[l + 1], EPI_BIAS_RESID, bias=blk.b_proj, resid=self.xtm[l], **prod,
                        prefetch=nxt_q(l), **self._tt("proj"))
        ops.layernorm_fwd(self.xt[-1], self.ln_final[0], self.ln_final[1], self.y_final)
        self._gemm(self.y_final, self.text_proj_t, self.text_f, EPI_NONE)

    def _patch_embed(self, image: torch.Tensor) -> None:
        cfg = self.cfg
        B = image.shape[0]
        R = B * (cfg.n_frozen + cfg.K)
        ops.im2col_patches(image, self.im2col[:B * cfg.n_patches], cfg.patch)
        ops.gemm_nt(self.im2col[:B * cfg.n_patches], self.conv_w, self.x_pre[:R], EPI_PATCH, resid=self.pos,
                    group=cfg.n_patches,
                    prefetch=self.vis[0].w_in if (self._pf_chains and len(self.vis)) else None)

    def _embed_norm(self, B: int, rows: Optional[tuple] = None) -> None:
        cfg = self.cfg
        R = B * (cfg.n_frozen + cfg.K)
        if self._multi: return self._m_img_embed(B, R, rows)
        ops.img_embed_norm(self.x_pre[:R], self.cls, self.pos, self.img_prompt, self.ln_pre[0], self.ln_pre[1], self.x[0][:R],
                           self.vis[0].ln1_w, self.vis[0].ln1_b, self.h[:R], B, cfg.n_frozen, cfg.K, rows=rows)

    def _patch_embed_early(self, image: torch.Tensor) -> None:
        self._patch_embed(image)
        self._embed_norm(image.shape[0], rows=(0, image.shape[0] * self.cfg.n_frozen))

    def _image_forward(self, image: torch.Tensor, train: bool, full_last: bool = False, patch_done: bool = False) -> None:
        cfg = self.cfg
        B, N, K, dv, H = image.shape[0], cfg.n_frozen, cfg.K, cfg.d_v, cfg.heads_v
        Rf, Rp = B * N, B * K
        R = Rf + Rp
        x_pre = self.x_pre[:R]
        if not patch_done:
            self._patch_embed(image)
        h, att, g = self.h[:R], self.att[:R], self.g[:R]
        self._embed_norm(B, rows=(Rf, R) if (patch_done and K > 0) else None)
        fold = self.fold_ln
        units = (N, K, Rf)
        which = os.environ.get("RPO_RESID_UNITS", "all")
        split = self._split_rows(B)
        small = self.ws_small and R < 1024 and not split and not full_last
        if small:
            units = None
        Mw = Rf if split else R
        if split:
            units = (N, 0, Rf)
        u_out, u_proj = (units if which == "all" else None), (units if which in ("all", "c_proj") else None)
        if small:
            u_out = u_proj = None
        grps = self._stats_group.get((B, split, small))
        if grps is None:
            grps = self._stats_group[(B, split, small)] = ((ops.gemm_stats_group(Mw, dv, dv, self.act, u_out),
                                                     ops.gemm_stats_group(Mw, dv, 4 * dv, self.act, u_proj)) if fold else (64, 64))
        g_out, g_proj = grps
        hilo = (fold and not full_last and u_out is not None and u_proj is not None and len(self.vis) > 1
                and os.environ.get("RPO_NO_HILO") != "1"
                and ops.gemm_hilo_ok(Mw, dv, dv, self.act, u_out, g_out) and ops.gemm_hilo_ok(Mw, dv, 4 * dv, self.act, u_proj, g_proj))
        h_lo = self.h_lo[:R]
        if hilo and os.environ.get("RPO_RESID16") == "1":
            h_lo = None
        stv = lambda grp: self.ln_stats.view(-1)[:R * (dv // grp) * 2].view(R, dv // grp, 2)
        st_out, st_proj, st64 = stv(g_out), stv(g_proj), self.ln_stats[:R]
        last = len(self.vis) - 1
        pf = os.environ.get("RPO_NO_WPREFETCH") != "1" and self.act != torch.float32
        table = dict(in_="out", out="fc", fc="proj", proj="in+")

        def pf_of(host: str, l: int):
            what = table[host] if pf else None
            if what is None:
                return None
            if what.endswith("+"):
                if l >= last:
                    return None
                b, what = self.vis[l + 1], what[:-1]
            else:
                b = self.vis[l]
            return {"out": b.w_out, "proj": b.w_proj, "fc": b.w_fc_ln if fold else b.w_fc,
                    "in": b.w_in_ln if (fold and b is not self.vis[0]) else b.w_in}[what]
        no_probe = lambda name: _NO_PROBE
        for l, blk in enumerate(self.vis):
            x, xm, xo, qkv = self.x[l][:R], self.xm[l][:R], self.x[l + 1][:R], self.qkv[l][:R]
            folded_in = fold and l > 0
            if not folded_in and l > 0:
                ops.layernorm_fwd(x, blk.ln1_w, blk.ln1_b, h)
            w_in, b_in = (blk.w_in_ln, blk.b_in_ln) if folded_in else (blk.w_in, blk.b_in)
            epi_in = EPI_LN_BIAS if folded_in else EPI_BIAS
            lnk = lambda r0, r1, c0, c1, own=False: (dict(ln_stats=(st64 if own else st_proj)[r0:r1], ln_colsum=blk.s_in[c0:c1],
                                                          ln_group=64 if own else g_proj) if folded_in else {})
            if l < last or full_last:
                if split:
                    with self._timed("in_proj"):
                        ops.gemm_nt(h[:Rf], w_in, qkv[:Rf], epi_in, bias=b_in, **lnk(0, Rf, 0, 3 * dv), prefetch=pf_of("in_", l))
                    ops.gemm_nt(h[Rf:], w_in[:dv], qkv[Rf:, :dv], epi_in, bias=b_in[:dv], **lnk(Rf, R, 0, dv, own=True))
                elif small:
                    with self._timed("in_proj"):
                        self._gemm(h, w_in, qkv, epi_in, bias=b_in, **lnk(0, R, 0, 3 * dv), prefetch=pf_of("in_", l))
                else:
                    with self._timed("in_proj"):
                        ops.gemm_nt(h, w_in, qkv, epi_in, bias=b_in, skip_row0=Rf, skip_col0=dv, **lnk(0, R, 0, 3 * dv),
                                    prefetch=pf_of("in_", l))
                with self._timed("attn_fwd"):
                    ops.attn_readonly_fwd(qkv[:, :dv], qkv[:, dv:2 * dv], qkv[:, 2 * dv:], att, B, H, N, K, SCALE)
                segs = [(0, Rf, True), (Rf, R, False)] if split else [(0, R, True)]
            else:
                ops.gemm_nt(h[:Rf], w_in[dv:], qkv[:Rf, dv:], epi_in, bias=b_in[dv:], **lnk(0, Rf, dv, 3 * dv))
                self._gemm(h[Rf:], w_in[:dv], qkv[Rf:, :dv], epi_in, bias=b_in[:dv], **lnk(Rf, R, 0, dv, own=split))
                ops.attn_readonly_fwd(qkv[:, :dv], qkv[:, dv:2 * dv], qkv[:, 2 * dv:], att, B, H, N, K, SCALE,
                                      q_first=N)
                segs = [(Rf, R, False)]
            for lo, hi, wide in segs:
                timed = self._timed if wide else no_probe
                un_o, go, so = (u_out, g_out, st_out) if wide else (None, 64, st64)
                un_p, gp, sp = (u_proj, g_proj, st_proj) if wide else (None, 64, st64)
                un = units if wide else None
                has_prompt = hi > Rf
                aux = self.u[l][:Rp] if (train and has_prompt) else None
                aux_row0 = max(Rf - lo, 0) if has_prompt else hi - lo
                prod = dict(out2=h[lo:hi], ln_stats=so[lo:hi], ln_group=go) if fold else {}
                hl = hilo and wide
                res_o = dict(resid_hi=h[:hi], resid_lo=None if h_lo is None else h_lo[:hi]) if (hl and l > 0) else dict(resid=x[lo:hi])
                if hl:
                    prod.update(out_lo=None if h_lo is None else h_lo[:hi], c_row0=Rf)
                gemm = ops.gemm_nt if (wide and not small) else self._gemm
                with timed("out_proj"):
                    gemm(att[lo:hi], blk.w_out, xm[lo:hi], EPI_BIAS_RESID, bias=blk.b_out, row_units=un_o,
                         **res_o, **prod, prefetch=pf_of("out", l) if wide else None)
                prod_p = dict(out2=h[lo:hi], ln_stats=sp[lo:hi], ln_group=gp) if (fold and l < last) else {}
                res_p = dict(resid_hi=h[:hi], resid_lo=None if h_lo is None else h_lo[:hi]) if hl else dict(resid=xm[lo:hi])
                if hl:
                    prod_p.update(out_lo=None if h_lo is None else h_lo[:hi], c_row0=Rf)
                proj_kw = dict(a=g[lo:hi], w=blk.w_proj, out=xo[lo:hi], epilogue=EPI_BIAS_RESID, bias=blk.b_proj, row_units=un_p,
                               **res_p, **prod_p, prefetch=pf_of("proj", l) if wide else None)
                if not wide or small:
                    proj_kw.pop("row_units"); proj_kw.pop("ln_group", None)
                if fold and wide and self._fused_mlp is not None:
                    fc_kw = dict(a=h[lo:hi], w=blk.w_fc_ln, out=g[lo:hi], epilogue=EPI_LN_BIAS_QGELU, bias=blk.b_fc_ln,
                                 aux=aux, aux_row0=aux_row0, ln_stats=so[lo:hi], ln_colsum=blk.s_fc, row_units=un,
                                 ln_group=go, prefetch=pf_of("fc", l))
                    with timed("c_fc"):
                        done = self._fused_mlp(fc_kw, proj_kw)
                    if done:
                        continue
                if fold:
                    with timed("c_fc"):
                        gemm(h[lo:hi], blk.w_fc_ln, g[lo:hi], EPI_LN_BIAS_QGELU, bias=blk.b_fc_ln,
                             aux=aux, aux_row0=aux_row0,
                             ln_stats=so[lo:hi], ln_colsum=blk.s_fc, row_units=un, ln_group=go,
                             prefetch=pf_of("fc", l) if wide else None)
                else:
                    with timed("ln_2"):
                        ops.layernorm_fwd(xm[lo:hi], blk.ln2_w, blk.ln2_b, h[lo:hi])
                    with timed("c_fc"):
                        gemm(h[lo:hi], blk.w_fc, g[lo:hi], EPI_BIAS_QGELU, bias=blk.b_fc,
                             aux=aux, aux_row0=aux_row0, row_units=un)
                with timed("c_proj"):
                    if wide and not small:
                        ops.gemm_nt(**proj_kw)
                    else:
                        pk = dict(proj_kw)
                        self._gemm(pk.pop("a"), pk.pop("w"), pk.pop("out"), pk.pop("epilogue"), **pk)
        ops.layernorm_fwd(self.x[-1][Rf:R], self.ln_post[0], self.ln_post[1], self.y_post[:Rp])
        self._gemm(self.y_post[:Rp], self.img_proj_t, self.img_f[:Rp], EPI_NONE)

    _fused_mlp = None

    def _split_rows(self, B: int) -> bool:
        return False

    def joint_backward_ok(self, B: Optional[int] = None) -> bool:
        return False

    def _bwd_fold_limits(self) -> tuple:
        return 64, (512, 768, 1024)

    def _rows_backward(self, blocks: List[_Block], x: List[torch.Tensor], xm: List[torch.Tensor],
                       u: List[torch.Tensor], dxa, dxb, dxc, du, da, dq, dy, attn_bwd, fold_out: bool = False,
                       tt: Optional[dict] = None) -> torch.Tensor:
        pf = self._pf_chains
        tc = lambda n: ({"tile_config": tt[n]} if (tt and n in tt) else {})
        ws = self.use_ws and dxa.shape[0] < 2048
        s_fc, s_q = (SPLIT_FC, SPLIT_Q) if not ws else (2, 1)
        if dxa.shape[0] >= 2048:
            s_fc = s_q = 1
        if ws and "RPO_WS_SPLITS" in os.environ:
            s_fc, s_q = (int(v) for v in os.environ["RPO_WS_SPLITS"].split("x"))
        for l in reversed(range(len(blocks))):
            blk = blocks[l]
            a_in = dxa if self.act == torch.float32 else dxc
            self._gemm(a_in, blk.w_proj_t, du, EPI_QGELU_BWD, aux=u[l], prefetch=blk.w_fc_t if pf else None, **tc("dproj"))
            dyf = dy[0] if s_fc == 1 else dy[:s_fc]
            self._gemm(du, blk.w_fc_t, dyf, EPI_NONE, split_k=s_fc,
                       prefetch=self._oq_hint(blk, fold_out, ws) if pf else None, **tc("dfc"))
            ops.layernorm_bwd(dyf, xm[l], blk.ln2_w, dxa, dxb,
                              None if self.act == torch.float32 else dxc)
            a_in = dxb if self.act == torch.float32 else dxc
            if fold_out:
                attn_bwd(l, a_in, dq)
            else:
                self._gemm(a_in, blk.w_out_t, da, EPI_NONE)
                attn_bwd(l, da, dq)
            dyq = dy[0] if s_q == 1 else dy[:s_q]
            self._gemm(dq, blk.w_q_t, dyq, EPI_NONE, split_k=s_q,
                       prefetch=blocks[l - 1].w_proj_t if (pf and l > 0) else None, **tc("dq"))
            ops.layernorm_bwd(dyq, x[l], blk.ln1_w, dxb, dxa,
                              None if self.act == torch.float32 else dxc)
        return dxa

    def _image_backward(self, B: int) -> None:
        self._image_backward_rows(B, 0, B)
        self._image_backward_finish(B)

    def _image_backward_rows(self, B: int, b0: int, b1: int) -> None:
        cfg = self.cfg
        N, K, dv, H = cfg.n_frozen, cfg.K, cfg.d_v, cfg.heads_v
        Rf = B * N
        r0, r1 = b0 * K, b1 * K
        f0, f1 = b0 * N, b1 * N
        nb = b1 - b0
        dxa, dxb, dxc = self.dxa_v[r0:r1], self.dxb_v[r0:r1], self.dxc_v[r0:r1]
        if self.act == torch.float32:
            d_f = self.d_img_f[r0:r1]
        else:
            d_f = self.d_img_f_a[r0:r1]
        self._gemm(d_f, self.img_proj, self.dy_v[0, r0:r1], EPI_NONE,
                   prefetch=self.vis[-1].w_proj_t if self._pf_chains else None)
        ops.layernorm_bwd(self.dy_v[0, r0:r1], self.x[-1][Rf + r0:Rf + r1], self.ln_post[0], None, dxa,
                          None if self.act == torch.float32 else dxc)

        kmax, widths = self._bwd_fold_limits()
        fold_out = (self.act != torch.float32 and K <= kmax and dv in widths and os.environ.get("RPO_NO_BWD_FOLD") != "1")

        def attn_bwd(l, da, dq):
            qkv = self.qkv[l]
            if fold_out:
                with self._timed("attn_bwd_proj"):
                    ops.attn_readonly_bwd_proj(qkv[Rf + r0:Rf + r1, :dv], qkv[f0:f1, dv:2 * dv], qkv[f0:f1, 2 * dv:], da,
                                               self.vis[l].w_out_t, dq, nb, H, N, K, SCALE)
            else:
                ops.attn_readonly_bwd(qkv[Rf + r0:Rf + r1, :dv], qkv[f0:f1, dv:2 * dv], qkv[f0:f1, 2 * dv:], da, dq,
                                      nb, H, N, K, SCALE)

        dx = self._image_chain(B, b0, b1, attn_bwd, fold_out)
        ops.layernorm_bwd(dx, self.x_pre[Rf + r0:Rf + r1], self.ln_pre[0], None, dxb)

    def _image_chain(self, B: int, b0: int, b1: int, attn_bwd, fold_out: bool) -> torch.Tensor:
        K, Rf = self.cfg.K, B * self.cfg.n_frozen
        r0, r1 = b0 * K, b1 * K
        return self._rows_backward(self.vis, [t[Rf + r0:Rf + r1] for t in self.x[:-1]], [t[Rf + r0:Rf + r1] for t in self.xm],
                                   [t[r0:r1] for t in self.u], self.dxa_v[r0:r1], self.dxb_v[r0:r1], self.dxc_v[r0:r1],
                                   self.du_v[r0:r1], self.da_v[r0:r1], self.dq_v[r0:r1], self.dy_v[:, r0:r1], attn_bwd,
                                   fold_out=fold_out)

    def _image_backward_finish(self, B: int) -> None:
        if self._multi: return self._m_img_reduce(B)
        ops.reduce_groups(self.dxb_v[:B * self.cfg.K], self.g_img, B)

    def _text_backward(self) -> None:
        self._ws_cfg = self._ws_text_cfg_bwd
        try:
            self._text_backward_()
        finally:
            self._ws_cfg = 0

    def _text_backward_(self) -> None:
        cfg = self.cfg
        n, K, dt, H, Rt = cfg.n_cls, cfg.K, cfg.d_t, cfg.heads_t, self.Rt
        dxa, dxb, dxc = self.dxa_t, self.dxb_t, self.dxc_t
        d_f = self.d_text_f if self.act == torch.float32 else self.d_text_f_a
        self._gemm(d_f, self.text_proj, self.dy_t[0], EPI_NONE,
                   prefetch=self.txt[-1].w_proj_t if self._pf_chains else None)
        ops.layernorm_bwd(self.dy_t[0], self.xt[-1], self.ln_final[0], None, dxa,
                          None if self.act == torch.float32 else dxc)

        dx = self._text_chain()
        if self._multi: return self._m_text_reduce(dx, n)
        ops.reduce_groups(dx, self.g_text, n)

    def _text_chain(self) -> torch.Tensor:
        cfg = self.cfg
        n, K, dt, H = cfg.n_cls, cfg.K, cfg.d_t, cfg.heads_t

        def attn_bwd(l, da, dq):
            kv = self.kv_t[l]
            if self._multi: return self._m_text_attn(l, da, dq)
            ops.text_attn_bwd(self.qt[l], kv[:, :dt], kv[:, dt:], da, dq, self.len_i32, n, K, self.Lmax, H, SCALE)

        return self._rows_backward(self.txt, self.xt[:-1], self.xtm, self.ut, self.dxa_t, self.dxb_t, self.dxc_t, self.du_t,
                                   self.da_t, self.dq_t, self.dy_t, attn_bwd, fold_out=False, tt=self._text_tiles)

    def forward_eval(self, image: torch.Tensor, use_graph: bool = True) -> torch.Tensor:
        self._refuse_rn("forward_eval")
        B = self._check(image)
        main = torch.cuda.current_stream()
        text_stale = self.text_f_version != self.params_version
        if text_stale:
            self.side.wait_stream(main)
            with torch.cuda.stream(self.side):
                self._text_forward(train=False)
            main.wait_stream(self.side)
            self.text_f_version = self.params_version
        if not use_graph:
            self._eval_body(image, B)
            return self.logits[:B]
        entry = self._eval_graphs.get(B)
        if entry is None:
            static = torch.empty_like(image)
            static.copy_(image)
            self._eval_body(static, B)
            torch.cuda.synchronize(self.dev)
            g = torch.cuda.CUDAGraph()
            with torch.cuda.graph(g, capture_error_mode="thread_local"):
                self._eval_body(static, B)
            entry = self._eval_graphs[B] = (g, static)
        g, static = entry
        if static.data_ptr() != image.data_ptr():
            static.copy_(image, non_blocking=True)
        g.replay()
        return self.logits[:B]

    def _eval_body(self, image: torch.Tensor, B: int) -> None:
        self._image_forward(image, train=False)
        K, e = self.cfg.K, self.cfg.embed
        ops.head_fwd_bwd(self.img_f[:B * K].view(B, K, e), self.text_f.view(self.cfg.n_cls, K, e), None,
                         self.logit_scale_exp, self.logits[:B], None, None, None, self.head_ws)

    def _head_act(self, B: int) -> dict:
        if self.act == torch.float32:
            return {}
        return dict(d_img_f_act=self.d_img_f_a[:B * self.cfg.K], d_text_f_act=self.d_text_f_a)

    def set_context(self, ctx) -> None:
        c = torch.as_tensor(np.asarray(ctx, dtype=np.float32), device=self.dev)
        n_ctx = c.shape[0]
        assert c.ndim == 2 and c.shape[1] == self.cfg.d_t and 1 + n_ctx < self.Lmax, "ctx: [n_ctx, d_t], 1 + n_ctx < prompt length"
        x = self.text_x_frozen.view(self.cfg.n_cls, self.Lmax, self.cfg.d_t)
        x[:, 1:1 + n_ctx] = (c + self.text_pos[1:1 + n_ctx])[None]
        self.text_cache_ready = False
        self.plain_text_f = None
        self.text_f_version = -1

    def forward_plain(self, image: torch.Tensor) -> torch.Tensor:
        cfg = self.cfg
        B = self._check(image)
        N, dv, e, n = cfg.n_frozen, cfg.d_v, cfg.embed, cfg.n_cls
        if not self.text_cache_ready:
            self.cache_text_kv()
        if self.plain_text_f is None:
            rows = torch.arange(n, device=self.dev) * self.Lmax + (self.len_i32.to(torch.int64) - 1)
            eot = self.text_x_final.index_select(0, rows).contiguous()
            y = torch.empty(n, cfg.d_t, dtype=self.act, device=self.dev)
            ops.layernorm_fwd(eot, self.ln_final[0], self.ln_final[1], y)
            self.plain_text_f = torch.empty(n, e, dtype=torch.float32, device=self.dev)
            ops.gemm_nt(y, self.text_proj_t, self.plain_text_f, EPI_NONE)
        if cfg.is_rn:
            self.rn_forward(image)
        else:
            self._image_forward(image, train=False, full_last=True)
            cls_rows = self.x[-1][:B * N].view(B, N, dv)[:, 0, :]
            ops.layernorm_fwd(cls_rows, self.ln_post[0], self.ln_post[1], self.y_post[:B])
            if self.img_cls_f is None:
                self.img_cls_f = torch.empty(self.max_batch, e, dtype=torch.float32, device=self.dev)
            ops.gemm_nt(self.y_post[:B], self.img_proj_t, self.img_cls_f[:B], EPI_NONE)
        ops.head_fwd_bwd(self.img_cls_f[:B].view(B, 1, e), self.plain_text_f.view(n, 1, e), None, self.logit_scale_exp,
                         self.logits[:B], None, None, None, self.head_ws)
        return self.logits[:B]

    def forward_backward(self, image: torch.Tensor, label: torch.Tensor) -> None:
        self._refuse_rn("forward_backward")
        B = self._check(image)
        self.text_f_version = -1
        assert label.dtype == torch.int64 and label.shape == (B,)
        K, e, n = self.cfg.K, self.cfg.embed, self.cfg.n_cls
        main = torch.cuda.current_stream()
        self.side.wait_stream(main)
        with torch.cuda.stream(self.side):
            self._text_forward(train=True)
        self._image_forward(image, train=True)
        main.wait_stream(self.side)
        ops.head_fwd_bwd(self.img_f[:B * K].view(B, K, e), self.text_f.view(n, K, e), label, self.logit_scale_exp,
                         self.logits[:B], self.loss, self.d_img_f[:B * K].view(B, K, e),
                         self.d_text_f.view(n, K, e), self.head_ws, **self._head_act(B))
        if self.joint_backward_ok(B):
            self._joint_backward(B)
            return
        self.side.wait_stream(main)
        with torch.cuda.stream(self.side):
            self._text_backward()
        self._image_backward(B)
        main.wait_stream(self.side)

    def head(self, B: int, label: torch.Tensor) -> None:
        K, e, n = self.cfg.K, self.cfg.embed, self.cfg.n_cls
        ops.head_fwd_bwd(self.img_f[:B * K].view(B, K, e), self.text_f.view(n, K, e), label, self.logit_scale_exp,
                         self.logits[:B], self.loss, self.d_img_f[:B * K].view(B, K, e),
                         self.d_text_f.view(n, K, e), self.head_ws, **self._head_act(B))

    def _refuse_rn(self, what: str) -> None:
        from .custom_clip import refuse_rn
        refuse_rn(self.cfg, f"Engine.{what} (the RPO step)")

    def _check(self, image: torch.Tensor) -> int:
        cfg = self.cfg
        assert image.is_cuda and image.dtype == torch.float32 and image.is_contiguous()
        assert image.device == self.dev and torch.cuda.current_device() == self.dev.index, \
            f"engine lives on {self.dev}: make it the current device and pass tensors that live there"
        B = image.shape[0]
        assert 1 <= B <= self.max_batch and tuple(image.shape[1:]) == (3, cfg.image_size, cfg.image_size)
        if not self.text_cache_ready:
            self.cache_text_kv()
        return B


def make_engine(*args, **kw) -> Engine:
    from ._lib import EXPERIMENTAL
    if EXPERIMENTAL:
        from .experimental import ExperimentalEngine
        return ExperimentalEngine(*args, **kw)
    return Engine(*args, **kw)
```

### rpo_amd/ops.py

```python
from __future__ import annotations

import ctypes as C
from typing import Optional

import torch

from . import _lib
from ._lib import (EPI_BIAS, EPI_BIAS_QGELU, EPI_BIAS_RESID, EPI_NONE, EPI_PATCH, EPI_QGELU_BWD, RPO_BF16,
                   RPO_F16, RPO_F32, GemmArgs, check)

LN_EPS = 1e-5


def dtype_code(t: torch.dtype) -> int:
    if t == torch.float32:
        return RPO_F32
    if t == torch.bfloat16:
        return RPO_BF16
    if t == torch.float16:
        return RPO_F16
    raise TypeError(f"unsupported dtype {t}")


def _stream() -> int:
# ... 391 lines not shown

def text_attn_fwd(q, kc, vc, out, len_i32, n_cls: int, rows: int, Lmax: int, H: int, causal: bool = False,
                  scale: float = 0.125):
    assert _ld(kc) == _ld(vc) and len_i32.dtype == torch.int32
    check(_lib.load().rpo_text_attn_fwd(q.data_ptr(), _ld(q), kc.data_ptr(), vc.data_ptr(), _ld(kc),
                                        out.data_ptr(), _ld(out), dtype_code(q.dtype), len_i32.data_ptr(), n_cls,
                                        rows, Lmax, H, int(causal), scale, _stream()), "rpo_text_attn_fwd")
    return out


def text_attn_bwd_dense(q, k, v, d_out, dq, dk, dv, len_i32, n_cls: int, Lmax: int, H: int, scale: float = 0.125):
    assert _ld(q) == _ld(k) == _ld(v) and _ld(dq) == _ld(dk) == _ld(dv) and len_i32.dtype == torch.int32
    assert q.dtype == d_out.dtype == dq.dtype
    check(_lib.load().rpo_text_attn_bwd_dense(q.data_ptr(), k.data_ptr(), v.data_ptr(), _ld(q), d_out.data_ptr(),
                                              _ld(d_out), dq.data_ptr(), dk.data_ptr(), dv.data_ptr(), _ld(dq),
                                              dtype_code(q.dtype), len_i32.data_ptr(), n_cls, Lmax, H, scale, _stream()),
          "rpo_text_attn_bwd_dense")
    return dq


def text_attn_bwd(q, kc, vc, da, dq, len_i32, n_cls: int, rows: int, Lmax: int, H: int, scale: float = 0.125):
    assert _ld(kc) == _ld(vc) and len_i32.dtype == torch.int32
    check(_lib.load().rpo_text_attn_bwd(q.data_ptr(), _ld(q), kc.data_ptr(), vc.data_ptr(), _ld(kc),
                                        da.data_ptr(), _ld(da), dq.data_ptr(), _ld(dq), dtype_code(q.dtype),
                                        len_i32.data_ptr(), n_cls, rows, Lmax, H, scale, _stream()),
          "rpo_text_attn_bwd")
    return dq


def text_attn_fwd_shared(q, kc, vc, out, len_i32, n_cls: int, n_kv: int, rows: int, Lmax: int, H: int, scale: float = 0.125):
    assert _ld(kc) == _ld(vc) and len_i32.dtype == torch.int32 and len_i32.numel() >= n_kv
    assert kc.shape[0] >= n_kv * Lmax and q.shape[0] >= n_cls * rows and out.shape[0] >= n_cls * rows
    check(_lib.load().rpo_text_attn_fwd_shared(q.data_ptr(), _ld(q), kc.data_ptr(), vc.data_ptr(), _ld(kc),
                                               out.data_ptr(), _ld(out), dtype_code(q.dtype), len_i32.data_ptr(), n_cls,
                                               n_kv, rows, Lmax, H, scale, _stream()), "rpo_text_attn_fwd_shared")
    return out


def text_attn_bwd_shared(q, kc, vc, da, dq, len_i32, n_cls: int, n_kv: int, rows: int, Lmax: int, H: int, scale: float = 0.125):
    assert _ld(kc) == _ld(vc) and len_i32.dtype == torch.int32 and len_i32.numel() >= n_kv
    assert kc.shape[0] >= n_kv * Lmax and q.shape[0] >= n_cls * rows and da.shape[0] >= n_cls * rows and dq.shape[0] >= n_cls * rows
    check(_lib.load().rpo_text_attn_bwd_shared(q.data_ptr(), _ld(q), kc.data_ptr(), vc.data_ptr(), _ld(kc),
                                               da.data_ptr(), _ld(da), dq.data_ptr(), _ld(dq), dtype_code(q.dtype),
                                               len_i32.data_ptr(), n_cls, n_kv, rows, Lmax, H, scale, _stream()),
          "rpo_text_attn_bwd_shared")
    return dq


def head_workspace_floats(B: int, Cc: int, K: int, e: int) -> int:
    return int(_lib.load().rpo_head_workspace_floats(B, Cc, K, e))


def head_fwd_bwd(img_f, text_f, label, scale_exp: float, logits, loss, d_img_f, d_text_f, ws,
                 d_img_f_act=None, d_text_f_act=None):
    B, K, e = img_f.shape
    Cc = text_f.shape[0]
    assert img_f.is_contiguous() and text_f.is_contiguous() and logits.is_contiguous()
    assert label is None or label.dtype == torch.int64
    act = d_img_f_act if d_img_f_act is not None else d_text_f_act
    assert act is None or (act.is_contiguous() and (d_text_f_act is None or d_text_f_act.is_contiguous()))
    check(_lib.load().rpo_head_fwd_bwd_act(img_f.data_ptr(), text_f.data_ptr(), _p(label), scale_exp,
                                           logits.data_ptr(), _p(loss), _p(d_img_f), _p(d_text_f), _p(d_img_f_act),
                                           _p(d_text_f_act), _lib.RPO_F32 if act is None else dtype_code(act.dtype),
                                           B, Cc, K, e, ws.data_ptr(), _stream()), "rpo_head_fwd_bwd_act")
    return logits


def head_fwd_bwd_grouped(img_f, text_f, label, scale_exp: float, logits, loss, d_img_f, d_text_f, ws, S: int,
                         d_img_f_act=None, d_text_f_act=None):
    SB, K, e = img_f.shape
    assert SB % S == 0 and text_f.shape[0] % S == 0
    B, Cc = SB // S, text_f.shape[0] // S
    assert img_f.is_contiguous() and text_f.is_contiguous() and logits.is_contiguous() and logits.numel() >= SB * Cc
    assert label is None or (label.dtype == torch.int64 and label.numel() == SB and label.is_contiguous())
    assert label is None or (loss.numel() >= S and loss.is_contiguous())
    assert ws.numel() >= S * head_workspace_floats(B, Cc, K, e)
    act = d_img_f_act if d_img_f_act is not None else d_text_f_act
    assert act is None or (act.is_contiguous() and (d_text_f_act is None or d_text_f_act.is_contiguous()))
    check(_lib.load().rpo_head_fwd_bwd_grouped_act(img_f.data_ptr(), text_f.data_ptr(), _p(label), scale_exp,
                                                   logits.data_ptr(), _p(loss), _p(d_img_f), _p(d_text_f),
                                                   _p(d_img_f_act), _p(d_text_f_act),
                                                   _lib.RPO_F32 if act is None else dtype_code(act.dtype),
                                                   S, B, Cc, K, e, ws.data_ptr(), _stream()), "rpo_head_fwd_bwd_grouped_act")
    return logits


def lp_head_workspace_floats(B: int, Cc: int, e: int) -> int:
    return int(_lib.load().rpo_lp_head_workspace_floats(B, Cc, e))


def lp_head_fwd_bwd(img_f, w, bias, text_f_n, label, scale_exp: float, z, logits, loss, g_w, g_bias, ws):
    B, e = img_f.shape
    Cc = text_f_n.shape[0]
    assert w.shape == (e, e) and bias.shape == (e,) and text_f_n.shape == (Cc, e)
    assert z.shape == (B, e) and logits.shape == (B, Cc)
    ts = [img_f, w, bias, text_f_n, z, logits] + ([] if label is None else [loss, g_w, g_bias])
    assert all(t.dtype == torch.float32 and t.is_contiguous() for t in ts + [ws])
    assert label is None or (label.dtype == torch.int64 and label.numel() == B)
    assert label is None or (g_w.shape == (e, e) and g_bias.shape == (e,))
    assert ws.numel() >= lp_head_workspace_floats(B, Cc, e)
    check(_lib.load().rpo_lp_head_fwd_bwd(img_f.data_ptr(), w.data_ptr(), bias.data_ptr(), text_f_n.data_ptr(), _p(label),
                                          scale_exp, z.data_ptr(), logits.data_ptr(), _p(loss), _p(g_w), _p(g_bias),
                                          B, Cc, e, ws.data_ptr(), _stream()), "rpo_lp_head_fwd_bwd")
    return logits


def eval_accumulate(logits, label, counts, cmat=None, pred=None):
    B, Cc = logits.shape
    assert logits.dtype == torch.float32 and logits.stride(1) == 1
    assert label.dtype == torch.int64 and label.numel() == B and label.is_contiguous()
    assert counts.dtype == torch.int64 and counts.numel() == 2 and counts.is_contiguous()
    assert cmat is None or (cmat.dtype == torch.int32 and cmat.numel() == Cc * Cc and cmat.is_contiguous())
    assert pred is None or (pred.dtype == torch.int32 and pred.numel() == B and pred.is_contiguous())
    check(_lib.load().rpo_eval_accumulate(logits.data_ptr(), logits.stride(0), label.data_ptr(), B, Cc, counts.data_ptr(),
                                          _p(cmat), _p(pred), _stream()), "rpo_eval_accumulate")
    return counts


def metanet_fwd(img_f, w1, b1, w2, b2, f_norm, hidden, bias):
    B, e = img_f.shape
    h, d = w1.shape[0], w2.shape[0]
    assert all(t.dtype == torch.float32 and t.is_contiguous() for t in (img_f, w1, b1, w2, b2, f_norm, hidden, bias))
    check(_lib.load().rpo_metanet_fwd(img_f.data_ptr(), w1.data_ptr(), b1.data_ptr(), w2.data_ptr(), b2.data_ptr(),
                                      f_norm.data_ptr(), hidden.data_ptr(), bias.data_ptr(), B, e, h, d, _stream()),
          "rpo_metanet_fwd")
    return bias


def metanet_bwd(d_bias, f_norm, hidden, w2, g_w1, g_b1, g_w2, g_b2):
    B, d = d_bias.shape
    e, h = f_norm.shape[1], hidden.shape[1]
    assert all(t.dtype == torch.float32 and t.is_contiguous() for t in (d_bias, f_norm, hidden, w2, g_w1, g_b1, g_w2, g_b2))
    check(_lib.load().rpo_metanet_bwd(d_bias.data_ptr(), f_norm.data_ptr(), hidden.data_ptr(), w2.data_ptr(),
                                      g_w1.data_ptr(), g_b1.data_ptr(), g_w2.data_ptr(), g_b2.data_ptr(), B, e, h, d,
                                      _stream()), "rpo_metanet_bwd")


def sgd_step(p, g, buf, lr: float, momentum: float, wd: float, grad_scale: float, first_step: bool):
    assert p.is_contiguous() and g.is_contiguous() and buf.is_contiguous()
    check(_lib.load().rpo_sgd_step(p.data_ptr(), g.data_ptr(), buf.data_ptr(), p.numel(), lr, momentum, wd,
                                   grad_scale, int(first_step), _stream()), "rpo_sgd_step")
    return p


def sgd_step_guarded(p, g, buf, lr: float, momentum: float, wd: float, grad_scale: float, first_step: bool, found_inf):
    assert p.is_contiguous() and g.is_contiguous() and buf.is_contiguous()
    assert found_inf.dtype == torch.int32 and found_inf.numel() >= 2 and found_inf.is_contiguous()
    check(_lib.load().rpo_sgd_step_guarded(p.data_ptr(), g.data_ptr(), buf.data_ptr(), p.numel(), lr, momentum, wd,
                                           grad_scale, int(first_step), found_inf.data_ptr(), _stream()),
          "rpo_sgd_step_guarded")
    return p


def convert(src: torch.Tensor, dst: torch.Tensor) -> torch.Tensor:
    assert src.dtype == torch.float32 and src.shape == dst.shape
    check(_lib.load().rpo_convert(src.data_ptr(), _ld(src), dst.data_ptr(), dtype_code(dst.dtype), _ld(dst),
                                  src.shape[0], src.shape[1], _stream()), "rpo_convert")
    return dst


def probe_mfma(which: int, a: torch.Tensor, b: torch.Tensor) -> torch.Tensor:
    d = torch.empty(32, 32, dtype=torch.float32, device=a.device)
    check(_lib.load().rpo_probe_mfma(which, a.data_ptr(), b.data_ptr(), d.data_ptr(), _stream()),
          "rpo_probe_mfma")
    return d


def probe_peaks(device: torch.device, which: int = 0, copy: bool = True) -> dict:
    import ctypes
    lib = _lib.load()
    sink = torch.zeros(4, dtype=torch.float32, device=device)
    flops = ctypes.c_double(0.0)
    ev = [torch.cuda.Event(enable_timing=True) for _ in range(4)]
    blocks, iters = 256 * 8, 4096 if which != 1 else 2048
    for timed in (False, True):
        if timed:
            ev[0].record()
        check(lib.rpo_probe_peak_mfma(which, blocks, iters, sink.data_ptr(), ctypes.byref(flops), _stream()),
              "rpo_probe_peak_mfma")
        if timed:
            ev[1].record()
    if not copy:
        torch.cuda.synchronize(device)
        return {"mfma_tflops": flops.value / (ev[0].elapsed_time(ev[1]) * 1e-3) / 1e12}
    n = 1 << 29
    src = torch.empty(n, dtype=torch.uint8, device=device).fill_(1)
    dst = torch.empty_like(src)
    reps = 5
    for timed in (False, True):
        if timed:
            ev[2].record()
        for _ in range(reps if timed else 1):
            check(lib.rpo_probe_peak_copy(src.data_ptr(), dst.data_ptr(), n, _stream()), "rpo_probe_peak_copy")
        if timed:
            ev[3].record()
    torch.cuda.synchronize(device)
    return {"mfma_tflops": flops.value / (ev[0].elapsed_time(ev[1]) * 1e-3) / 1e12,
            "copy_gbs": 2.0 * n * reps / (ev[2].elapsed_time(ev[3]) * 1e-3) / 1e9}



def _nhwc(t: torch.Tensor, what: str) -> None:
    assert t.is_cuda and t.is_contiguous() and t.dim() == 4, f"{what}: contiguous [B, H, W, C] device tensor"


def conv2d_nhwc(x, w, bias, y, resid=None, relu: bool = True, tile_config: int = 0):
    _nhwc(x, "x"); _nhwc(y, "y")
    B, H, W, Cin = x.shape
    Cout, kh, kw, cin_w = w.shape
    assert kh == kw and cin_w == Cin and w.is_contiguous() and w.dtype == x.dtype == y.dtype
    assert tuple(y.shape) == (B, H, W, Cout) and bias.dtype == torch.float32 and bias.numel() == Cout
    if resid is not None:
        _nhwc(resid, "resid")
        assert resid.shape == y.shape and resid.dtype == y.dtype
    check(_lib.load().rpo_conv2d_nhwc(x.data_ptr(), w.data_ptr(), bias.data_ptr(), _p(resid), y.data_ptr(),
                                      dtype_code(x.dtype), B, H, W, Cin, Cout, kh, int(relu), tile_config, _stream()),
          "rpo_conv2d_nhwc")
    return y


def conv_stem(image, w, bias, y, relu: bool = True):
    assert image.dtype == torch.float32 and image.is_contiguous() and image.dim() == 4 and image.shape[1] == 3
    _nhwc(y, "y")
    B, _, H, W = image.shape
    Cout = w.shape[0]
    assert tuple(w.shape) == (Cout, 3, 3, 3) and w.is_contiguous() and w.dtype == y.dtype
    assert tuple(y.shape) == (B, H // 2, W // 2, Cout) and bias.dtype == torch.float32 and bias.numel() == Cout
    check(_lib.load().rpo_conv_stem(image.data_ptr(), w.data_ptr(), bias.data_ptr(), y.data_ptr(), dtype_code(y.dtype),
                                    B, H, W, Cout, int(relu), _stream()), "rpo_conv_stem")
    return y


def avgpool_nhwc(x, y, k: int):
    _nhwc(x, "x"); _nhwc(y, "y")
    B, H, W, C = x.shape
    assert tuple(y.shape) == (B, H // k, W // k, C) and y.dtype == x.dtype
    check(_lib.load().rpo_avgpool_nhwc(x.data_ptr(), y.data_ptr(), dtype_code(x.dtype), B, H, W, C, k, _stream()),
          "rpo_avgpool_nhwc")
    return y


def attnpool_tokens(x, pos, tokens):
    _nhwc(x, "x")
    B, H, W, C = x.shape
    assert pos.dtype == torch.float32 and pos.is_contiguous() and tuple(pos.shape) == (H * W + 1, C)
    assert tokens.is_contiguous() and tuple(tokens.shape) == (B, H * W + 1, C) and tokens.dtype == x.dtype
    check(_lib.load().rpo_attnpool_tokens(x.data_ptr(), pos.data_ptr(), tokens.data_ptr(), dtype_code(x.dtype), B, H * W, C,
                                          _stream()), "rpo_attnpool_tokens")
    return tokens


def attnpool_attn(q, kv, out, heads: int, scale: float):
    B, T, C2 = kv.shape
    C = C2 // 2
    assert q.dtype == torch.float32 and q.dim() == 2 and q.stride(1) == 1 and tuple(q.shape) == (B, C)
    assert kv.is_contiguous() and out.is_contiguous() and tuple(out.shape) == (B, C) and out.dtype == kv.dtype
    check(_lib.load().rpo_attnpool_attn(q.data_ptr(), q.stride(0), kv.data_ptr(), out.data_ptr(), dtype_code(kv.dtype), B, T,
                                        C, heads, scale, _stream()), "rpo_attnpool_attn")
    return out
```

### rpo_amd/trainer.py

```python
from __future__ import annotations

import collections
import math
import os
from dataclasses import dataclass
from typing import Dict, Optional

import numpy as np
import torch

from . import ops
from .config import RPOConfig
from .custom_clip import CustomCLIP
from .dist import GradSync
from .loop import LoopMixin
from ._lib import xenv as _xenv


@dataclass
class OptimConfig:
    lr: float = 0.01
    max_epoch: int = 15
    lr_scheduler: str = "cosine"
    warmup_epoch: int = 1
    warmup_type: str = "constant"
    warmup_cons_lr: float = 1e-5
    momentum: float = 0.9
    weight_decay: float = 5e-4


def lr_at_epoch(oc: OptimConfig, epoch: int) -> float:
    warm = oc.warmup_epoch if oc.warmup_type == "constant" else 0
    if epoch < warm:
        return oc.warmup_cons_lr
    if oc.lr_scheduler == "cosine":
        return 0.5 * oc.lr * (1.0 + math.cos(math.pi * (epoch - warm) / oc.max_epoch))
    return oc.lr


class RPO(LoopMixin):
    _takes_next_image = True
    _takes_frozen = True

    def __init__(self, cfg: RPOConfig, state_dict: Dict[str, np.ndarray], tokens: Optional[np.ndarray] = None,
                 optim: Optional[OptimConfig] = None, device: str | torch.device = "cuda:0",
                 act_dtype: torch.dtype = torch.bfloat16, batch_size: int = 4, num_batches: int = 1,
                 use_graph: bool = True, sync: Optional[GradSync] = None, prompts=None, amp: bool = False):
        from .custom_clip import refuse_rn
        refuse_rn(cfg, "RPO")
        self.cfg = cfg
        self.amp = amp
        self.optim_cfg = optim or OptimConfig()
        self.sync = sync or GradSync()
        self.device = torch.device(device)
        if self.device.index is None:
            idx = self.sync.local_rank if (self.sync.enabled and torch.cuda.device_count() > self.sync.local_rank) \
                else torch.cuda.current_device()
            self.device = torch.device("cuda", idx)
        self.batch_size = batch_size
        self.num_batches = num_batches
        self.use_graph = use_graph
        self.epoch = 0
        self.batch_idx = 0
        self._steps = 0
        self._graph = None
        self._joint_bwd = False
        self._split_collective = False
        self._graph_collectives = False
        self._graph_collectives_note = None
        self._text_ar_in_graph = False
        self._tail_graphs = {}
        self.best_result = -float("inf")
        self._found_inf = None
        self.detect_anomaly = os.environ.get("RPO_DETECT_ANOMALY") == "1"
        with torch.cuda.device(self.device):
            self.build_model(state_dict, tokens, act_dtype, prompts)

    def build_model(self, state_dict, tokens, act_dtype, prompts) -> None:
        self.model = CustomCLIP(self.cfg, state_dict, tokens, self.device, act_dtype,
                                max_batch=self.batch_size, prompts=prompts)
        self.engine = self.model.engine
        self.lr = lr_at_epoch(self.optim_cfg, 0)
        cfg = self.cfg
        self._image = torch.zeros(self.batch_size, 3, cfg.image_size, cfg.image_size, device=self.device)
        self._label = torch.zeros(self.batch_size, dtype=torch.int64, device=self.device)
        if self.sync.enabled:
            self.sync.broadcast(self.engine.params)

    def transform(self, is_train: bool):
        from .input_pipeline import InputConfig, build_transform
        key = "_tf_train" if is_train else "_tf_test"
        if getattr(self, key, None) is None:
            icfg = InputConfig(SIZE=(self.cfg.image_size, self.cfg.image_size))
            setattr(self, key, build_transform(icfg, is_train, self.device, self.batch_size))
        return getattr(self, key)

    def parse_batch_train(self, batch):
        img = batch["img"]
        if isinstance(img, (list, tuple)):
            img = self.transform(True)(img, out=self._image if len(img) == self.batch_size else None)
        else:
            img = img.to(self.device, dtype=torch.float32, non_blocking=True)
        label = torch.as_tensor(batch["label"])
        if not label.is_cuda:
            lo, hi = int(label.min()), int(label.max())
            if lo < 0 or hi >= self.cfg.n_cls:
                raise IndexError(f"Target {hi if hi >= self.cfg.n_cls else lo} is out of bounds "
                                 f"(n_cls = {self.cfg.n_cls}; labels must be renumbered after the base/new split)")
        return img, label.to(self.device, dtype=torch.int64, non_blocking=True)

    def _capture(self) -> None:
        eng, B = self.engine, self.batch_size
        eng.forward_backward(self._image, self._label)
        torch.cuda.synchronize()
        self._graph_collectives = (self.sync.enabled and self.sync.backend == "nccl"
                                   and os.environ.get("RPO_NO_GRAPH_COLLECTIVES") != "1")
        if self._graph_collectives:
            self.sync.all_reduce_sum(eng.grads)
            torch.cuda.synchronize()
        self._tail_graphs = {}

        def cap(fn):
            g = torch.cuda.CUDAGraph()
            with torch.cuda.graph(g, capture_error_mode="thread_local"):
                fn()
            return g

        self._g_text_fwd = cap(lambda: eng._text_forward(train=True))
        self._g_img_fwd = cap(lambda: eng._image_forward(self._image, train=True))
        self._g_head = cap(lambda: eng.head(B, self._label))
        self._joint_bwd = eng.joint_backward_ok(B)
        self._bwd_parts = 1
        self._split_collective = (self.sync.enabled and os.environ.get("RPO_ONE_COLLECTIVE") != "1"
                                  and self.sync.backend == "nccl")
        if self._joint_bwd:
            self._g_bwd = cap(lambda: eng._joint_backward(B))
        else:
            self._text_ar_in_graph = False
            if self._split_collective and self._graph_collectives:
                try:
                    self._g_text_bwd = cap(lambda: (eng._text_backward(), self.sync.all_reduce_sum(eng.g_text_flat)))
                    self._text_ar_in_graph = True
                except Exception as ex:
                    print(f"[rpo_amd] capturing the collective failed ({type(ex).__name__}: {ex}); collectives stay eager")
                    self._graph_collectives = False
                    self._graph_collectives_note = f"capture of the RCCL all-reduce failed ({type(ex).__name__}): eager for this process group"
                    torch.cuda.synchronize()
            if not self._text_ar_in_graph:
                self._g_text_bwd = cap(eng._text_backward)
            P = int(_xenv("RPO_BWD_PARTS", "1"))
            self._bwd_parts = P if (P > 1 and B % P == 0) else 1
            if self._bwd_parts > 1:
                per = B // self._bwd_parts
                self._g_img_bwd_parts = [cap(lambda i=i: eng._image_backward_rows(B, i * per, (i + 1) * per))
                                         for i in range(self._bwd_parts)]
                self._g_img_bwd_fin = cap(lambda: eng._image_backward_finish(B))
                self._part_streams = [torch.cuda.Stream(device=self.device) for _ in range(self._bwd_parts - 1)]
                self._ev_parts = [torch.cuda.Event() for _ in range(self._bwd_parts - 1)]
            else:
                self._g_img_bwd = cap(lambda: eng._image_backward(B))
        self._ev_fork = torch.cuda.Event()
        self._ev_text_fwd = torch.cuda.Event()
        self._ev_head = torch.cuda.Event()
        self._ev_text_bwd = torch.cuda.Event()
        self._g_patch = self._g_img_fwd_np = None
        self._ev_patch = torch.cuda.Event()
        self._patch_tag = None
        self._image_next = None
        want = os.environ.get("RPO_EARLY_TEXT")
        small = self.batch_size * (self.cfg.n_frozen + self.cfg.K) < 2048
        self._early_text = ((want == "1" or (want is None and small)) and not self.amp and not self._joint_bwd
                            and self._bwd_parts == 1 and (not self.sync.enabled or self._split_collective))
        self._text_fwd_for = -1
        self._g_step = None
        if (os.environ.get("RPO_ONE_GRAPH") == "1" and not self._early_text and not self._joint_bwd and self._bwd_parts == 1
                and (not self._split_collective or self._text_ar_in_graph or not self.sync.enabled)):
            def whole():
                main, side = torch.cuda.current_stream(), eng.side
                side.wait_stream(main)
                with torch.cuda.stream(side):
                    eng._text_forward(train=True)
                eng._image_forward(self._image, train=True)
                main.wait_stream(side)
                eng.head(B, self._label)
                side.wait_stream(main)
                with torch.cuda.stream(side):
                    eng._text_backward()
                    if self._text_ar_in_graph:
                        self.sync.all_reduce_sum(eng.g_text_flat)
                eng._image_backward(B)
                main.wait_stream(side)
            try:
                self._g_step = cap(whole)
            except Exception as ex:
                print(f"[rpo_amd] one-graph capture failed ({type(ex).__name__}: {ex}); five graphs per step")
                self._g_step = None
                torch.cuda.synchronize()
        self._graph = True
        torch.cuda.synchronize()

    def _patch_graph(self, next_image: torch.Tensor):
        eng = self.engine
        if self._g_img_fwd_np is None:
            torch.cuda.synchronize()
            g = torch.cuda.CUDAGraph()
            with torch.cuda.graph(g, capture_error_mode="thread_local"):
                eng._image_forward(self._image, train=True, patch_done=True)
            self._g_img_fwd_np = g
            self._g_patch = {}
        src = next_image
        if src.data_ptr() not in self._g_patch and len(self._g_patch) >= 8:
            if self._image_next is None:
                self._image_next = torch.zeros_like(self._image)
            torch.cuda.current_stream().wait_event(self._ev_patch)
            self._image_next.copy_(next_image, non_blocking=True)
            src = self._image_next
        g = self._g_patch.get(src.data_ptr())
        if g is None:
            torch.cuda.synchronize()
            g = torch.cuda.CUDAGraph()
            with torch.cuda.graph(g, capture_error_mode="thread_local"):
                eng._patch_embed_early(src)
            self._g_patch[src.data_ptr()] = (g, src)
            torch.cuda.synchronize()
        else:
            g = g[0]
        return g

    def _replay(self, patch_ready: bool = False, g_patch=None) -> None:
        main, side = torch.cuda.current_stream(), self.engine.side
        if self._g_step is not None and not patch_ready and g_patch is None:
            self._g_step.replay()
            return
        self._ev_fork.record(main)
        if not (self._early_text and self._text_fwd_for == self.engine.params_version):
            side.wait_event(self._ev_fork)
            with torch.cuda.stream(side):
                self._g_text_fwd.replay()
                self._ev_text_fwd.record(side)
        if patch_ready:
            main.wait_event(self._ev_patch)
            self._g_img_fwd_np.replay()
        else:
            self._g_img_fwd.replay()
        main.wait_event(self._ev_text_fwd)
        self._g_head.replay()
        if self._joint_bwd:
            self._g_bwd.replay()
            return
        self._ev_head.record(main)
        side.wait_event(self._ev_head)
        with torch.cuda.stream(side):
            self._g_text_bwd.replay()
            if self._split_collective and not self._text_ar_in_graph:
                self.sync.all_reduce_sum(self.engine.g_text_flat)
            if self._early_text:
                self._run_tail("text")
            self._ev_text_bwd.record(side)
            if g_patch is not None:
                g_patch.replay()
                self._ev_patch.record(side)
            if self._early_text:
                self._g_text_fwd.replay()
                self._ev_text_fwd.record(side)
                self._text_fwd_for = self.engine.params_version + 1
        if self._bwd_parts > 1:
            for st, ev, g in zip(self._part_streams, self._ev_parts, self._g_img_bwd_parts[1:]):
                st.wait_event(self._ev_head)
                with torch.cuda.stream(st):
                    g.replay()
                    ev.record(st)
            self._g_img_bwd_parts[0].replay()
            for ev in self._ev_parts:
                main.wait_event(ev)
            self._g_img_bwd_fin.replay()
        else:
            self._g_img_bwd.replay()
        main.wait_event(self._ev_text_bwd)

    def forward_backward(self, batch) -> Dict[str, float]:
        with torch.cuda.device(self.device):
            image, label = self.parse_batch_train(batch)
            loss = self.step_async(image, label)
            summary = {"loss": float(loss.item())}
            if self.detect_anomaly:
                self.check_finite()
        if (self.batch_idx + 1) == self.num_batches:
            self.update_lr()
            self.batch_idx = 0
        else:
            self.batch_idx += 1
        return summary

    def step_async(self, image: torch.Tensor, label: torch.Tensor, next_image: Optional[torch.Tensor] = None) -> torch.Tensor:
        eng, oc = self.engine, self.optim_cfg
        assert torch.cuda.current_device() == self.device.index, "set the trainer's device current (torch.cuda.set_device)"
        assert image.shape[0] == self.batch_size, "graph path needs the configured batch size"
        tag = (image.data_ptr(), image._version)
        pending = self.use_graph and self._graph is not None and self._patch_tag is not None
        patch_ready = pending and self._patch_tag == tag
        if pending and not patch_ready:
            torch.cuda.current_stream().wait_event(self._ev_patch)
        self._patch_tag = None
        if not patch_ready and image.data_ptr() != self._image.data_ptr():
            self._image.copy_(image, non_blocking=True)
        self._label.copy_(label, non_blocking=True)
        if self.use_graph:
            if self._graph is None:
                self._capture()
            patch_next = (next_image is not None and os.environ.get("RPO_EARLY_PATCH", "1") != "0"
                          and not self._joint_bwd and self._bwd_parts == 1)
            g_patch = None
            if patch_next:
                assert (next_image.shape == self._image.shape and next_image.dtype == torch.float32 and next_image.is_cuda
                        and next_image.is_contiguous())
                g_patch = self._patch_graph(next_image)
                self._patch_tag = (next_image.data_ptr(), next_image._version)
            self._replay(patch_ready, g_patch)
        else:
            eng.forward_backward(self._image, self._label)
        if self.amp and self._found_inf is None:
            self._found_inf = torch.zeros(2, dtype=torch.int32, device=self.device)
        self._run_tail("img" if (self.use_graph and getattr(self, "_early_text", False)) else "all")
        self._steps += 1
        eng.params_version += 1
        eng.text_f_version = -1
        return eng.loss

    def _run_tail(self, which: str) -> None:
        tail = None
        if self.use_graph and getattr(self, "_graph_collectives", False) and self._steps > 0:
            key = (self.lr, which)
            tail = self._tail_graphs.get(key)
            if tail is None:
                try:
                    tail = torch.cuda.CUDAGraph()
                    with torch.cuda.graph(tail, capture_error_mode="thread_local"):
                        self._tail(which)
                    if len(self._tail_graphs) >= 64:
                        self._tail_graphs.clear()
                    self._tail_graphs[key] = tail
                except Exception as ex:
                    print(f"[rpo_amd] capturing the step's tail failed ({type(ex).__name__}: {ex}); it stays eager")
                    self._graph_collectives_note = f"capture of the step's tail failed ({type(ex).__name__}): eager for this process group"
                    self._graph_collectives, tail = False, None
                    torch.cuda.synchronize()
        if tail is not None:
            tail.replay()
        else:
            self._tail(which)

    def _tail(self, which: str = "all") -> None:
        eng, oc = self.engine, self.optim_cfg
        nt = eng.g_text_flat.numel()
        if which == "text":
            sl = slice(0, nt)
        elif which == "img":
            sl = slice(nt, None)
            self.sync.all_reduce_sum(eng.g_img_flat)
        else:
            sl = slice(None)
            if self.use_graph and self._split_collective and not self._joint_bwd:
                self.sync.all_reduce_sum(eng.g_img_flat)
            else:
                self.sync.all_reduce_sum(eng.grads)
        if self.amp:
            ops.sgd_step_guarded(eng.params, eng.grads, eng.mom, self.lr, oc.momentum, oc.weight_decay,
                                 self.sync.grad_scale, first_step=(self._steps == 0), found_inf=self._found_inf)
        else:
            ops.sgd_step(eng.params[sl], eng.grads[sl], eng.mom[sl], self.lr, oc.momentum, oc.weight_decay,
                         self.sync.grad_scale, first_step=(self._steps == 0))

    def update_lr(self) -> None:
        self.epoch += 1
        self.lr = lr_at_epoch(self.optim_cfg, self.epoch)

    def check_finite(self) -> None:
        eng = self.engine
        self._join_side()
        bad = [n for n, t in (("loss", eng.loss), ("logits", eng.logits[:self.batch_size]), ("grad text_prompt", eng.g_text),
                              ("grad img_prompt", eng.g_img), ("prompts", eng.params)) if not bool(torch.isfinite(t).all())]
        if bad:
            raise FloatingPointError(f"non-finite values after step {self._steps}: {', '.join(bad)}")
        for name, t, idx in (("rpo_chain_bwd (image)", getattr(eng, "chain_state_v", None), 0),
                             ("rpo_chain_bwd (text)", getattr(eng, "chain_state_t", None), 0),
                             ("rpo_mlp_fused", getattr(eng, "mlp_counters", None) if _xenv("RPO_MLP_FUSED") != "0" else None, -1)):
            if t is not None and int(t[idx]) != 0:
                raise RuntimeError(f"{name}: a bounded spin gave up in or before step {self._steps}: the results are undefined")

    def _join_side(self) -> None:
        if not self._graph:
            return
        cur = torch.cuda.current_stream(self.device)
        if getattr(self, "_early_text", False):
            cur.wait_event(self._ev_text_fwd)
        if getattr(self, "_patch_tag", None) is not None:
            cur.wait_event(self._ev_patch)
            self._patch_tag = None

    @torch.no_grad()
    def model_inference(self, image) -> torch.Tensor:
        self._join_side()
        with torch.cuda.device(self.device):
            if isinstance(image, (list, tuple)):
                image = self.transform(False)(image)
            self.model.prompt_learner.eval()
            try:
                return self.model(image)
            finally:
                self.model.prompt_learner.train()

    def _eval_logits(self, image: torch.Tensor) -> torch.Tensor:
        self._join_side()
        return self.model.eval_logits(image)

    def _shared_sides(self):
        eng, pl = self.engine, self.model.prompt_learner
        ver = (pl.text_prompt._version, pl.img_prompt._version)
        if ver != getattr(self.model, "_seen_version", None):
            eng.params_version += 1
            self.model._seen_version = ver
        return eng.img_prompt.unsqueeze(0), eng.eval_text_features()

    def test(self, image_set, batch_size: int = 100, verbose: bool = True, per_class_result: bool = False, frozen=None,
             hook=None):
        if frozen is None:
            return super().test(image_set, batch_size, verbose, per_class_result)
        self._join_side()
        return self._test_shared(image_set, 1, self._shared_sides, batch_size, frozen, verbose, per_class_result, hook)[0]

    def save_model(self, directory: str, epoch: Optional[int] = None, is_best: bool = False,
                   val_result: Optional[float] = None) -> str:
        epoch = self.epoch if epoch is None else epoch
        self._join_side()
        ck = checkpoint_dict(self.model.prompt_learner.state_dict(), epoch, self.engine.mom, self.optim_cfg,
                             self.lr, self._steps, self.cfg.K * self.cfg.d_t, val_result)
        return write_checkpoint(directory, ck, epoch, is_best)

    def after_epoch_eval(self, directory: str, val_result: float) -> bool:
        is_best = val_result > self.best_result
        if is_best:
            self.best_result = val_result
            self.save_model(directory, is_best=True, val_result=val_result)
        return is_best

    def load_model(self, directory: str, epoch: Optional[int] = None) -> None:
        if not directory:
            print("Note that load_model() is skipped as no pretrained model is given")
            return
        model_file = "model-best.pth.tar" if epoch is None else f"model.pth.tar-{epoch}"
        model_path = os.path.join(directory, "prompt_learner", model_file)
        if not os.path.exists(model_path):
            raise FileNotFoundError(f'Model not found at "{model_path}"')
        ck = load_checkpoint_file(model_path)
        sd = dict(ck["state_dict"])
        for k in ("token_prefix", "token_suffix"):
            sd.pop(k, None)
        print(f'Loading weights to prompt_learner from "{model_path}" (epoch = {ck["epoch"]})')
        self._join_side()
        with torch.no_grad():
            for name, p in self.model.prompt_learner.named_parameters():
                if name in sd:
                    p.copy_(sd[name].to(p.dtype))
        mom = _momentum_from_optimizer_state(ck.get("optimizer"), self.engine.mom.numel())
        if mom is not None:
            self.engine.mom.copy_(mom)
            self._steps = max(1, int(ck.get("steps", 1)))
        self.engine.params_version += 1
        self.epoch = int(ck.get("epoch", 0))
        self.lr = lr_at_epoch(self.optim_cfg, self.epoch)


_CKPT_ALLOWED = {
    ("collections", "OrderedDict"), ("collections", "defaultdict"), ("collections", "Counter"),
    ("builtins", "dict"), ("builtins", "list"), ("builtins", "tuple"), ("builtins", "set"), ("builtins", "frozenset"),
    ("builtins", "int"), ("builtins", "float"), ("builtins", "bool"), ("builtins", "str"), ("builtins", "bytes"),
    ("builtins", "complex"), ("builtins", "slice"), ("builtins", "range"),
    ("torch", "Size"), ("torch", "device"), ("torch", "Tensor"),
    ("torch._utils", "_rebuild_tensor_v2"), ("torch._utils", "_rebuild_tensor"), ("torch._utils", "_rebuild_parameter"),
    ("torch._utils", "_rebuild_parameter_with_state"), ("torch._tensor", "_rebuild_from_type_v2"),
    ("torch.nn.parameter", "Parameter"), ("torch.serialization", "_get_layout"),
    ("numpy.core.multiarray", "scalar"), ("numpy._core.multiarray", "scalar"), ("numpy", "dtype"),
    ("numpy.core.multiarray", "_reconstruct"), ("numpy._core.multiarray", "_reconstruct"), ("numpy", "ndarray"),
}


class _Inert:
    def __init__(self, *a, **k):
        pass

    def __call__(self, *a, **k):
        return None

    def __setstate__(self, state):
        self.__dict__.update(state if isinstance(state, dict) else {})


import pickle as _pickle


class _RestrictedUnpickler(_pickle.Unpickler):

    def find_class(self, module, name):
        if "." in name or not name:
            raise _pickle.UnpicklingError(f"{module}.{name} is not allowed in a checkpoint (dotted name)")
        top = module.split(".")[0]
        if top == "dassl" or module == "torch.optim" or module.startswith("torch.optim."):
            return _Inert
        key_mod = "builtins" if module == "__builtin__" else module
        ok = (key_mod, name) in _CKPT_ALLOWED
        if not ok and module == "torch":
            obj = getattr(torch, name, None)
            ok = isinstance(obj, torch.dtype) or (isinstance(obj, type) and name.endswith("Storage"))
        if not ok:
            raise _pickle.UnpicklingError(f"{module}.{name} is not allowed in a checkpoint")
        return super().find_class(module, name)


class _RestrictedPickle:
    __name__ = "rpo_amd_restricted_pickle"
    Unpickler = _RestrictedUnpickler
    load = staticmethod(lambda f, **k: _RestrictedUnpickler(f, **k).load())


def load_checkpoint_file(path: str) -> dict:
    pickle = _pickle
    try:
        return torch.load(path, map_location="cpu", weights_only=True)
# ... 53 lines not shown
```

Baseline: 11210.

## Fuse final LayerNorm backward, group reduction and SGD update into one tail kernel

Adds a grad_tail kernel that computes the last LayerNorm backward (optionally chained through a second LayerNorm), sums the per-group gradient rows in shared memory, and applies the SGD momentum update in the same launch. The lr and first-step flag are read from a device control tensor so the fused step can live inside the captured backward graph. This removes the separate reduce_groups and tail SGD launches, along with a round trip of the per-row gradient through memory. In exchange each prompt row is handled by a single block, which limits parallelism, and the trainer has to keep the control tensor in sync with the host.

```diff
diff --git a/include/rpo_amd.h b/include/rpo_amd.h
--- a/include/rpo_amd.h
+++ b/include/rpo_amd.h
@@ -209,6 +209,11 @@
 int rpo_sgd_step_guarded(float* p, const float* g, float* buf, int64_t n, float lr, float momentum, float wd,
                          float grad_scale, int first_step, int32_t* found_inf, void* stream);
 
+int rpo_grad_tail(const float* dy, int64_t lddy, int dy_splits, int64_t dy_split_stride, const float* x, int64_t ldx,
+                  const float* gamma, const float* dres, int64_t lddres, const float* x2, int64_t ldx2, const float* gamma2,
+                  float* grad, float* params, float* mom, const float* ctl, int groups, int rows, int d, float eps,
+                  float momentum, float wd, float grad_scale, void* stream);
+
 int rpo_convert(const float* src, int64_t lds, void* dst, int dst_dtype, int64_t ldd,
                 int rows, int cols, void* stream);
 
diff --git a/rpo_amd/_lib.py b/rpo_amd/_lib.py
--- a/rpo_amd/_lib.py
+++ b/rpo_amd/_lib.py
@@ -167,6 +167,8 @@
     "rpo_attnpool_attn": (c_i32, [c_vp, c_i64, c_vp, c_vp, c_i32, c_i32, c_i32, c_i32, c_i32, c_f32, c_vp]),
     "rpo_sgd_step": (c_i32, [c_vp, c_vp, c_vp, c_i64, c_f32, c_f32, c_f32, c_f32, c_i32, c_vp]),
     "rpo_sgd_step_guarded": (c_i32, [c_vp, c_vp, c_vp, c_i64, c_f32, c_f32, c_f32, c_f32, c_i32, c_vp, c_vp]),
+    "rpo_grad_tail": (c_i32, [c_vp, c_i64, c_i32, c_i64, c_vp, c_i64, c_vp, c_vp, c_i64, c_vp, c_i64, c_vp, c_vp, c_vp, c_vp,
+                              c_vp, c_i32, c_i32, c_i32, c_f32, c_f32, c_f32, c_f32, c_vp]),
     "rpo_convert": (c_i32, [c_vp, c_i64, c_vp, c_i32, c_i64, c_i32, c_i32, c_vp]),
     "rpo_probe_mfma": (c_i32, [c_i32, c_vp, c_vp, c_vp, c_vp]),
     "rpo_probe_peak_mfma": (c_i32, [c_i32, c_i32, c_i32, c_vp, c_vp, c_vp]),
diff --git a/rpo_amd/csrc/common.h b/rpo_amd/csrc/common.h
--- a/rpo_amd/csrc/common.h
+++ b/rpo_amd/csrc/common.h
@@ -88,6 +88,21 @@
 #pragma unroll
   for (int o = 32; o > 0; o >>= 1) v = fmaxf(v, __shfl_xor(v, o, 64));
   return v;
+}
+
+__device__ __forceinline__ void sgd_update_values(float pi, float bold, float g, float lr, float mom, float wd, float gs,
+                                                  int first, float& p_new, float& b_new) {
+  const float gi = gs * g + wd * pi;
+  const float bi = first ? gi : mom * bold + gi;
+  b_new = bi;
+  p_new = pi - lr * bi;
+}
+__device__ __forceinline__ void sgd_update(float* p, float* buf, int64_t i, float g, float lr, float mom, float wd, float gs,
+                                           int first) {
+  float pn, bn;
+  sgd_update_values(p[i], first ? 0.f : buf[i], g, lr, mom, wd, gs, first, pn, bn);
+  buf[i] = bn;
+  p[i] = pn;
 }
 
 #define RPO_QG 1.702f
diff --git a/rpo_amd/csrc/misc.hip b/rpo_amd/csrc/misc.hip
--- a/rpo_amd/csrc/misc.hip
+++ b/rpo_amd/csrc/misc.hip
@@ -114,11 +114,7 @@
                            float wd, float gs, int first) {
   const int64_t i = (int64_t)blockIdx.x * blockDim.x + threadIdx.x;
   if (i >= n) return;
-  const float pi = p[i];
-  const float gi = gs * g[i] + wd * pi;
-  const float bi = first ? gi : mom * buf[i] + gi;
-  buf[i] = bi;
-  p[i] = pi - lr * bi;
+  sgd_update(p, buf, i, g[i], lr, mom, wd, gs, first);
 }
 
 __global__ __launch_bounds__(1024) void sgd_guarded_kernel(float* p, const float* __restrict__ g, float* buf, int64_t n,
@@ -138,11 +134,7 @@
   if (threadIdx.x == 0) { found[0] = skip; found[1] += skip; }
   if (skip) return;
   for (int64_t i = threadIdx.x; i < n; i += 1024) {
-    const float pi = p[i];
-    const float gi = gs * g[i] + wd * pi;
-    const float bi = first ? gi : mom * buf[i] + gi;
-    buf[i] = bi;
-    p[i] = pi - lr * bi;
+    sgd_update(p, buf, i, g[i], lr, mom, wd, gs, first);
   }
 }
 
diff --git a/rpo_amd/csrc/norm.hip b/rpo_amd/csrc/norm.hip
--- a/rpo_amd/csrc/norm.hip
+++ b/rpo_amd/csrc/norm.hip
@@ -141,6 +141,78 @@
                      unpack1<f16_t>((uint16_t)(u.y & 0xffffu)), unpack1<f16_t>((uint16_t)(u.y >> 16)));
 }
 
+template <typename TDY, int NV>
+__device__ __forceinline__ void ln_bwd_load(const TDY* __restrict__ dyr, const float* __restrict__ xr,
+                                            const float* __restrict__ gamma, int nv4, int lane, int splits,
+                                            int64_t split_stride, float4 (&v)[NV], float4 (&g)[NV]) {
+#pragma unroll
+  for (int i = 0; i < NV; ++i) {
+    const int c = lane + 64 * i;
+    v[i] = make_float4(0.f, 0.f, 0.f, 0.f);
+    g[i] = make_float4(0.f, 0.f, 0.f, 0.f);
+    if (c < nv4) {
+      v[i] = *reinterpret_cast<const float4*>(xr + 4 * c);
+      const float4 w = *reinterpret_cast<const float4*>(gamma + 4 * c);
+      float4 t = load4f<TDY>(dyr + 4 * c);
+      float4 ts[3];
+#pragma unroll
+      for (int sp = 1; sp < 4; ++sp) ts[sp - 1] = load4f<TDY>(dyr + (int64_t)min(sp, splits - 1) * split_stride + 4 * c);
+#pragma unroll
+      for (int sp = 1; sp < 4; ++sp) {
+        const float m = sp < splits ? 1.0f : 0.0f;
+        t.x = fmaf(m, ts[sp - 1].x, t.x); t.y = fmaf(m, ts[sp - 1].y, t.y);
+        t.z = fmaf(m, ts[sp - 1].z, t.z); t.w = fmaf(m, ts[sp - 1].w, t.w);
+      }
+      for (int sp = 4; sp < splits; ++sp) {
+        const float4 t2 = load4f<TDY>(dyr + (int64_t)sp * split_stride + 4 * c);
+        t.x += t2.x; t.y += t2.y; t.z += t2.z; t.w += t2.w;
+      }
+      g[i] = make_float4(t.x * w.x, t.y * w.y, t.z * w.z, t.w * w.w);
+    }
+  }
+}
+
+template <int NV, typename EMIT>
+__device__ __forceinline__ void ln_bwd_math(float4 (&v)[NV], const float4 (&g)[NV], const float4 (&rr)[NV], int nv4,
+                                            int lane, int d, float eps, EMIT&& emit) {
+  float s = 0.f;
+#pragma unroll
+  for (int i = 0; i < NV; ++i) s += (v[i].x + v[i].y) + (v[i].z + v[i].w);
+  const float mu = wave_sum(s) / (float)d;
+  float q = 0.f;
+#pragma unroll
+  for (int i = 0; i < NV; ++i) {
+    const int c = lane + 64 * i;
+    if (c < nv4) {
+      v[i].x -= mu; v[i].y -= mu; v[i].z -= mu; v[i].w -= mu;
+      q += (v[i].x * v[i].x + v[i].y * v[i].y) + (v[i].z * v[i].z + v[i].w * v[i].w);
+    }
+  }
+  const float rstd = rsqrtf(wave_sum(q) / (float)d + eps);
+  float sg = 0.f, sgx = 0.f;
+#pragma unroll
+  for (int i = 0; i < NV; ++i) {
+    const int c = lane + 64 * i;
+    if (c < nv4) {
+      v[i].x *= rstd; v[i].y *= rstd; v[i].z *= rstd; v[i].w *= rstd;
+      sg += (g[i].x + g[i].y) + (g[i].z + g[i].w);
+      sgx += (g[i].x * v[i].x + g[i].y * v[i].y) + (g[i].z * v[i].z + g[i].w * v[i].w);
+    }
+  }
+  const float mg = wave_sum(sg) / (float)d;
+  const float mgx = wave_sum(sgx) / (float)d;
+#pragma unroll
+  for (int i = 0; i < NV; ++i) {
+    const int c = lane + 64 * i;
+    if (c < nv4) {
+      float4 o = make_float4(rstd * (g[i].x - mg - v[i].x * mgx), rstd * (g[i].y - mg - v[i].y * mgx),
+                             rstd * (g[i].z - mg - v[i].z * mgx), rstd * (g[i].w - mg - v[i].w * mgx));
+      o.x += rr[i].x; o.y += rr[i].y; o.z += rr[i].z; o.w += rr[i].w;
+      emit(i, c, o);
+    }
+  }
+}
+
 template <typename TDY, typename TC, int NV>
 __device__ __forceinline__ void ln_bwd_row(const TDY* __restrict__ dy, int64_t lddy,
                                            const float* __restrict__ x, int64_t ldx,
@@ -153,34 +225,8 @@
   const int row = blk * RPO_LN_RPB + (threadIdx.x >> 6);
   if (row >= rows) return;
   const int nv4 = d >> 2;
-  const float* xr = x + (int64_t)row * ldx;
-  const TDY* dyr = dy + (int64_t)row * lddy;
   float4 v[NV], g[NV];
-#pragma unroll
-  for (int i = 0; i < NV; ++i) {
-    const int c = lane + 64 * i;
-    v[i] = make_float4(0.f, 0.f, 0.f, 0.f);
-    g[i] = make_float4(0.f, 0.f, 0.f, 0.f);
-    if (c < nv4) {
-      v[i] = *reinterpret_cast<const float4*>(xr + 4 * c);
-      const float4 w = *reinterpret_cast<const float4*>(gamma + 4 * c);
-      float4 t = load4f<TDY>(dyr + 4 * c);
-      float4 ts[3];
-#pragma unroll
-      for (int sp = 1; sp < 4; ++sp) ts[sp - 1] = load4f<TDY>(dyr + (int64_t)min(sp, splits - 1) * split_stride + 4 * c);
-#pragma unroll
-      for (int sp = 1; sp < 4; ++sp) {
-        const float m = sp < splits ? 1.0f : 0.0f;
-        t.x = fmaf(m, ts[sp - 1].x, t.x); t.y = fmaf(m, ts[sp - 1].y, t.y);
-        t.z = fmaf(m, ts[sp - 1].z, t.z); t.w = fmaf(m, ts[sp - 1].w, t.w);
-      }
-      for (int sp = 4; sp < splits; ++sp) {
-        const float4 t2 = load4f<TDY>(dyr + (int64_t)sp * split_stride + 4 * c);
-        t.x += t2.x; t.y += t2.y; t.z += t2.z; t.w += t2.w;
-      }
-      g[i] = make_float4(t.x * w.x, t.y * w.y, t.z * w.z, t.w * w.w);
-    }
-  }
+  ln_bwd_load<TDY, NV>(dy + (int64_t)row * lddy, x + (int64_t)row * ldx, gamma, nv4, lane, splits, split_stride, v, g);
   float4 rr[NV];
 #pragma unroll
   for (int i = 0; i < NV; ++i) {
@@ -188,43 +234,10 @@
     rr[i] = make_float4(0.f, 0.f, 0.f, 0.f);
     if (dres != nullptr && c < nv4) rr[i] = *reinterpret_cast<const float4*>(dres + (int64_t)row * lddres + 4 * c);
   }
-  float s = 0.f;
-#pragma unroll
-  for (int i = 0; i < NV; ++i) s += (v[i].x + v[i].y) + (v[i].z + v[i].w);
-  const float mu = wave_sum(s) / (float)d;
-  float q = 0.f;
-#pragma unroll
-  for (int i = 0; i < NV; ++i) {
-    const int c = lane + 64 * i;
-    if (c < nv4) {
-      v[i].x -= mu; v[i].y -= mu; v[i].z -= mu; v[i].w -= mu;
-      q += (v[i].x * v[i].x + v[i].y * v[i].y) + (v[i].z * v[i].z + v[i].w * v[i].w);
-    }
-  }
-  const float rstd = rsqrtf(wave_sum(q) / (float)d + eps);
-  float sg = 0.f, sgx = 0.f;
-#pragma unroll
-  for (int i = 0; i < NV; ++i) {
-    const int c = lane + 64 * i;
-    if (c < nv4) {
-      v[i].x *= rstd; v[i].y *= rstd; v[i].z *= rstd; v[i].w *= rstd;
-      sg += (g[i].x + g[i].y) + (g[i].z + g[i].w);
-      sgx += (g[i].x * v[i].x + g[i].y * v[i].y) + (g[i].z * v[i].z + g[i].w * v[i].w);
-    }
-  }
-  const float mg = wave_sum(sg) / (float)d;
-  const float mgx = wave_sum(sgx) / (float)d;
-#pragma unroll
-  for (int i = 0; i < NV; ++i) {
-    const int c = lane + 64 * i;
-    if (c < nv4) {
-      float4 o = make_float4(rstd * (g[i].x - mg - v[i].x * mgx), rstd * (g[i].y - mg - v[i].y * mgx),
-                             rstd * (g[i].z - mg - v[i].z * mgx), rstd * (g[i].w - mg - v[i].w * mgx));
-      o.x += rr[i].x; o.y += rr[i].y; o.z += rr[i].z; o.w += rr[i].w;
-      *reinterpret_cast<float4*>(dx + (int64_t)row * lddx + 4 * c) = o;
-      if (dxc != nullptr) ActIO<TC>::st4(dxc + (int64_t)row * ldc + 4 * c, o.x, o.y, o.z, o.w);
-    }
-  }
+  ln_bwd_math<NV>(v, g, rr, nv4, lane, d, eps, [&](int, int c, const float4& o) {
+    *reinterpret_cast<float4*>(dx + (int64_t)row * lddx + 4 * c) = o;
+    if (dxc != nullptr) ActIO<TC>::st4(dxc + (int64_t)row * ldc + 4 * c, o.x, o.y, o.z, o.w);
+  });
 }
 
 template <typename TDY, typename TC, int NV>
@@ -251,6 +264,82 @@
   ln_bwd_row<float, TC, NV>(q.dy, q.lddy, q.x, q.ldx, q.gamma, q.dres, q.lddres, q.dx, q.lddx, static_cast<TC*>(q.dxc),
                             q.ldc, q.rows, q.d, q.eps, q.splits, q.split_stride,
                             second ? (int)blockIdx.x - g.blocks0 : (int)blockIdx.x);
+}
+
+struct GradTail {
+  const float* dy; int64_t lddy; int splits; int64_t split_stride;
+  const float* x; int64_t ldx; const float* gamma; const float* dres; int64_t lddres;
+  const float* x2; int64_t ldx2; const float* gamma2;
+  float* grad; float* p; float* mom; const float* ctl;
+  int G, K, d; float eps, momentum, wd, gs;
+};
+template <int NV>
+__global__ __launch_bounds__(NV > 3 ? 512 : 1024) void grad_tail_kernel(const GradTail a) {
+  extern __shared__ __attribute__((aligned(16))) float tail_rows[];
+  const int lane = threadIdx.x & 63, wave = __builtin_amdgcn_readfirstlane(threadIdx.x >> 6), W = blockDim.x >> 6;
+  const int k = blockIdx.x, d = a.d, nv4 = d >> 2;
+  float acc[4] = {0.f, 0.f, 0.f, 0.f};
+  float p_old[4], m_old[4];
+#pragma unroll
+  for (int j = 0; j < 4; ++j) {
+    const int c = min((int)threadIdx.x + (int)blockDim.x * j, d - 1);
+    p_old[j] = a.p[(int64_t)k * d + c];
+    m_old[j] = a.mom[(int64_t)k * d + c];
+  }
+  for (int g0 = 0; g0 < a.G; g0 += W) {
+    const int grp = g0 + wave;
+    if (grp < a.G) {
+      const int64_t row = (int64_t)grp * a.K + k;
+      float4 v[NV], g[NV], rr[NV], v2[NV], w2[NV], o[NV];
+      ln_bwd_load<float, NV>(a.dy + row * a.lddy, a.x + row * a.ldx, a.gamma, nv4, lane, a.splits, a.split_stride, v, g);
+#pragma unroll
+      for (int i = 0; i < NV; ++i) {
+        const int c = lane + 64 * i;
+        rr[i] = v2[i] = w2[i] = o[i] = make_float4(0.f, 0.f, 0.f, 0.f);
+        if (c < nv4) {
+          if (a.dres != nullptr) rr[i] = *reinterpret_cast<const float4*>(a.dres + row * a.lddres + 4 * c);
+          if (a.x2 != nullptr) {
+            v2[i] = *reinterpret_cast<const float4*>(a.x2 + row * a.ldx2 + 4 * c);
+            w2[i] = *reinterpret_cast<const float4*>(a.gamma2 + 4 * c);
+          }
+        }
+      }
+      ln_bwd_math<NV>(v, g, rr, nv4, lane, d, a.eps, [&](int i, int, const float4& r) { o[i] = r; });
+      if (a.x2 != nullptr) {
+#pragma unroll
+        for (int i = 0; i < NV; ++i) {
+          g[i] = make_float4(o[i].x * w2[i].x, o[i].y * w2[i].y, o[i].z * w2[i].z, o[i].w * w2[i].w);
+          rr[i] = make_float4(0.f, 0.f, 0.f, 0.f);
+        }
+        ln_bwd_math<NV>(v2, g, rr, nv4, lane, d, a.eps, [&](int i, int, const float4& r) { o[i] = r; });
+      }
+#pragma unroll
+      for (int i = 0; i < NV; ++i) {
+        const int c = lane + 64 * i;
+        if (c < nv4) *reinterpret_cast<float4*>(tail_rows + wave * d + 4 * c) = o[i];
+      }
+    }
+    __syncthreads();
+    const int n = min(W, a.G - g0);
+#pragma unroll
+    for (int j = 0; j < 4; ++j) {
+      const int c = threadIdx.x + (int)blockDim.x * j;
+      if (c < d)
+        for (int w = 0; w < n; ++w) acc[j] += tail_rows[w * d + c];
+    }
+    __syncthreads();
+  }
+  const float lr = a.ctl[0];
+  const int first = a.ctl[1] != 0.f;
+#pragma unroll
+  for (int j = 0; j < 4; ++j) {
+    const int c = threadIdx.x + (int)blockDim.x * j;
+    if (c < d) {
+      const int64_t i = (int64_t)k * d + c;
+      a.grad[i] = acc[j];
+      sgd_update_values(p_old[j], m_old[j], acc[j], lr, a.momentum, a.wd, a.gs, first, a.p[i], a.mom[i]);
+    }
+  }
 }
 
 }
@@ -371,6 +460,32 @@
   return rpo_launch_status();
 }
 
+extern "C" int rpo_grad_tail(const float* dy, int64_t lddy, int dy_splits, int64_t dy_split_stride, const float* x,
+                             int64_t ldx, const float* gamma, const float* dres, int64_t lddres, const float* x2,
+                             int64_t ldx2, const float* gamma2, float* grad, float* params, float* mom, const float* ctl,
+                             int groups, int rows, int d, float eps, float momentum, float wd, float grad_scale,
+                             void* stream) {
+  if (!dy || !x || !gamma || !grad || !params || !mom || !ctl || groups <= 0 || rows <= 0 || d <= 0 ||
+      (x2 != nullptr) != (gamma2 != nullptr)) return RPO_E_BADARG;
+  if (d % 4 != 0 || d > 1024) return RPO_E_SHAPE;
+  if (dy_splits < 1) dy_splits = 1;
+  if (dy_splits > 1 && dy_split_stride % 4 != 0) return RPO_E_SHAPE;
+  if (!aligned16(dy) || !aligned16(x) || !aligned16(gamma) || lddy % 4 || ldx % 4) return RPO_E_ALIGN;
+  if (dres && (!aligned16(dres) || lddres % 4)) return RPO_E_ALIGN;
+  if (x2 && (!aligned16(x2) || !aligned16(gamma2) || ldx2 % 4)) return RPO_E_ALIGN;
+  const GradTail a{dy, lddy, dy_splits, dy_split_stride, x, ldx, gamma, dres, lddres, x2, ldx2, gamma2, grad, params, mom, ctl,
+                   groups, rows, d, eps, momentum, wd, grad_scale};
+  const int nv = (d / 4 + 63) / 64;
+  const int waves = groups <= 4 ? 4 : ((groups <= 8 || nv > 3) ? 8 : 16);
+  const dim3 grid(rows), block(64 * waves);
+  const size_t smem = (size_t)waves * d * sizeof(float);
+  hipStream_t s = static_cast<hipStream_t>(stream);
+  if (nv <= 2) hipLaunchKernelGGL(grad_tail_kernel<2>, grid, block, smem, s, a);
+  else if (nv == 3) hipLaunchKernelGGL(grad_tail_kernel<3>, grid, block, smem, s, a);
+  else hipLaunchKernelGGL(grad_tail_kernel<4>, grid, block, smem, s, a);
+  return rpo_launch_status();
+}
+
 extern "C" int rpo_img_embed_norm(float* x_pre, int64_t ldx, const float* cls, const float* pos0, const float* img_prompt,
                                   const float* g_pre, const float* b_pre, float* x0, int64_t ldx0, const float* g1,
                                   const float* b1, void* h, int64_t ldh, int h_dtype, int B, int N, int Kp, int d,
diff --git a/rpo_amd/engine.py b/rpo_amd/engine.py
--- a/rpo_amd/engine.py
+++ b/rpo_amd/engine.py
@@ -18,6 +18,7 @@
 from .engine_multi import MultiEngineMixin
 from .engine_prompt_rows import PromptRowsEngineMixin
 from .engine_rn import RnEngineMixin
+from .engine_tail import GradTailEngineMixin
 
 import contextlib
 
@@ -48,7 +49,7 @@
     w_fc_ln: Optional[torch.Tensor] = None; s_fc: Optional[torch.Tensor] = None; b_fc_ln: Optional[torch.Tensor] = None
 
 
-class Engine(CoopEngineMixin, LpEngineMixin, RnEngineMixin, MultiEngineMixin, PromptRowsEngineMixin):
+class Engine(CoopEngineMixin, LpEngineMixin, RnEngineMixin, MultiEngineMixin, PromptRowsEngineMixin, GradTailEngineMixin):
     def __init__(self, cfg: RPOConfig, state_dict: Dict[str, np.ndarray], tokens: np.ndarray,
                  device: torch.device, act_dtype: torch.dtype = torch.bfloat16, max_batch: int = 32):
         if not torch.cuda.is_available():
@@ -288,6 +289,7 @@
         self.g_img = self.grads[nt:].view(K, dv)
         self.g_text_flat, self.g_img_flat = self.grads[:nt], self.grads[nt:]
         self.side = torch.cuda.Stream(device=dev)
+        self.tail_fused = {"text": False, "img": False}
 
     def hbm_bytes(self) -> int:
         tot = 0
@@ -544,6 +546,7 @@
         tc = lambda n: ({"tile_config": tt[n]} if (tt and n in tt) else {})
         ws = self.use_ws and dxa.shape[0] < 2048
         s_fc, s_q = (SPLIT_FC, SPLIT_Q) if not ws else (2, 1)
+        last_ln, self._last_ln = self._last_ln, None
         if dxa.shape[0] >= 2048:
             s_fc = s_q = 1
         if ws and "RPO_WS_SPLITS" in os.environ:
@@ -566,13 +569,11 @@
             dyq = dy[0] if s_q == 1 else dy[:s_q]
             self._gemm(dq, blk.w_q_t, dyq, EPI_NONE, split_k=s_q,
                        prefetch=blocks[l - 1].w_proj_t if (pf and l > 0) else None, **tc("dq"))
+            if l == 0 and last_ln is not None and last_ln(dyq, x[l], blk.ln1_w, dxb):
+                break
             ops.layernorm_bwd(dyq, x[l], blk.ln1_w, dxb, dxa,
                               None if self.act == torch.float32 else dxc)
         return dxa
-
-    def _image_backward(self, B: int) -> None:
-        self._image_backward_rows(B, 0, B)
-        self._image_backward_finish(B)
 
     def _image_backward_rows(self, B: int, b0: int, b1: int) -> None:
         cfg = self.cfg
@@ -604,7 +605,10 @@
                 ops.attn_readonly_bwd(qkv[Rf + r0:Rf + r1, :dv], qkv[f0:f1, dv:2 * dv], qkv[f0:f1, 2 * dv:], da, dq,
                                       nb, H, N, K, SCALE)
 
+        self._arm_tail("img", B if (b0 == 0 and b1 == B) else 0, self.x_pre[Rf + r0:Rf + r1], self.ln_pre[0])
         dx = self._image_chain(B, b0, b1, attn_bwd, fold_out)
+        self._last_ln = None
+        if self.tail_fused["img"]: return
         ops.layernorm_bwd(dx, self.x_pre[Rf + r0:Rf + r1], self.ln_pre[0], None, dxb)
 
     def _image_chain(self, B: int, b0: int, b1: int, attn_bwd, fold_out: bool) -> torch.Tensor:
@@ -615,10 +619,6 @@
                                    self.du_v[r0:r1], self.da_v[r0:r1], self.dq_v[r0:r1], self.dy_v[:, r0:r1], attn_bwd,
                                    fold_out=fold_out)
 
-    def _image_backward_finish(self, B: int) -> None:
-        if self._multi: return self._m_img_reduce(B)
-        ops.reduce_groups(self.dxb_v[:B * self.cfg.K], self.g_img, B)
-
     def _text_backward(self) -> None:
         self._ws_cfg = self._ws_text_cfg_bwd
         try:
@@ -636,7 +636,10 @@
         ops.layernorm_bwd(self.dy_t[0], self.xt[-1], self.ln_final[0], None, dxa,
                           None if self.act == torch.float32 else dxc)
 
+        self._arm_tail("text", n)
         dx = self._text_chain()
+        self._last_ln = None
+        if self.tail_fused["text"]: return
         if self._multi: return self._m_text_reduce(dx, n)
         ops.reduce_groups(dx, self.g_text, n)
 
diff --git a/rpo_amd/engine_tail.py b/rpo_amd/engine_tail.py
--- /dev/null
+++ b/rpo_amd/engine_tail.py
@@ -0,0 +1,36 @@
+from __future__ import annotations
+
+from typing import Optional
+
+import torch
+
+from . import ops
+
+
+class GradTailEngineMixin:
+    fused_tail = None
+    _last_ln = None
+
+    def _arm_tail(self, which: str, groups: int, x2: Optional[torch.Tensor] = None, gamma2: Optional[torch.Tensor] = None) -> None:
+        self.tail_fused[which] = False
+        ft = None if (self._multi or groups <= 0) else self.fused_tail
+        if ft is None:
+            return
+        nt = self.g_text_flat.numel()
+        half = slice(0, nt) if which == "text" else slice(nt, None)
+        grad = self.g_text if which == "text" else self.g_img
+
+        def last_ln(dy, x, gamma, dres) -> bool:
+            self.tail_fused[which] = ops.grad_tail(dy, x, gamma, dres, x2, gamma2, grad, self.params[half], self.mom[half],
+                                                   ft["ctl"], groups, ft["momentum"], ft["wd"], ft["gs"])
+            return self.tail_fused[which]
+        self._last_ln = last_ln
+
+    def _image_backward(self, B: int) -> None:
+        self._image_backward_rows(B, 0, B)
+        self._image_backward_finish(B)
+
+    def _image_backward_finish(self, B: int) -> None:
+        if self._multi: return self._m_img_reduce(B)
+        if self.tail_fused["img"]: return
+        ops.reduce_groups(self.dxb_v[:B * self.cfg.K], self.g_img, B)
diff --git a/rpo_amd/ops.py b/rpo_amd/ops.py
--- a/rpo_amd/ops.py
+++ b/rpo_amd/ops.py
@@ -567,6 +567,31 @@
     return p
 
 
+def grad_tail(dy: torch.Tensor, x: torch.Tensor, gamma: torch.Tensor, dres: Optional[torch.Tensor],
+              x2: Optional[torch.Tensor], gamma2: Optional[torch.Tensor], grad: torch.Tensor, params: torch.Tensor,
+              mom: torch.Tensor, ctl: torch.Tensor, groups: int, momentum: float, wd: float, grad_scale: float,
+              eps: float = LN_EPS) -> bool:
+    rows, d = grad.shape
+    assert x.shape[0] >= groups * rows and x.shape[1] == d and dy.dtype == torch.float32 and x.dtype == torch.float32
+    assert grad.is_contiguous() and params.is_contiguous() and mom.is_contiguous()
+    assert params.numel() == rows * d and mom.numel() == rows * d
+    assert ctl.dtype == torch.float32 and ctl.numel() >= 2 and ctl.is_contiguous() and ctl.is_cuda
+    assert (x2 is None) == (gamma2 is None) and (x2 is None or (x2.shape[0] >= groups * rows and x2.shape[1] == d))
+    splits, split_stride = 1, 0
+    if dy.dim() == 3:
+        splits, split_stride, lddy = dy.shape[0], dy.stride(0), dy.stride(1)
+    else:
+        lddy = _ld(dy)
+    rc = _lib.load().rpo_grad_tail(dy.data_ptr(), lddy, splits, split_stride, x.data_ptr(), _ld(x), gamma.data_ptr(),
+                                   _p(dres), 0 if dres is None else _ld(dres), _p(x2), 0 if x2 is None else _ld(x2),
+                                   _p(gamma2), grad.data_ptr(), params.data_ptr(), mom.data_ptr(), ctl.data_ptr(),
+                                   groups, rows, d, eps, momentum, wd, grad_scale, _stream())
+    if rc == _lib.E_SHAPE:
+        return False
+    check(rc, "rpo_grad_tail")
+    return True
+
+
 def convert(src: torch.Tensor, dst: torch.Tensor) -> torch.Tensor:
     assert src.dtype == torch.float32 and src.shape == dst.shape
     check(_lib.load().rpo_convert(src.data_ptr(), _ld(src), dst.data_ptr(), dtype_code(dst.dtype), _ld(dst),
diff --git a/rpo_amd/trainer.py b/rpo_amd/trainer.py
--- a/rpo_amd/trainer.py
+++ b/rpo_amd/trainer.py
@@ -36,6 +36,12 @@
     if oc.lr_scheduler == "cosine":
         return 0.5 * oc.lr * (1.0 + math.cos(math.pi * (epoch - warm) / oc.max_epoch))
     return oc.lr
+
+
+def fused_tail_selected(sync_enabled: bool, amp: bool, use_graph: bool, env=None) -> bool:
+    env = os.environ if env is None else env
+    return (use_graph and not sync_enabled and not amp and env.get("RPO_FUSED_TAIL", "1") != "0"
+            and env.get("RPO_ONE_GRAPH") != "1")
 
 
 class RPO(LoopMixin):
@@ -72,6 +78,9 @@
         self._tail_graphs = {}
         self.best_result = -float("inf")
         self._found_inf = None
+        self._fused = {"text": False, "img": False}
+        self._tail_ctl = None
+        self._tail_ctl_host = None
         self.detect_anomaly = os.environ.get("RPO_DETECT_ANOMALY") == "1"
         with torch.cuda.device(self.device):
             self.build_model(state_dict, tokens, act_dtype, prompts)
@@ -111,6 +120,7 @@
 
     def _capture(self) -> None:
         eng, B = self.engine, self.batch_size
+        eng.fused_tail = None
         eng.forward_backward(self._image, self._label)
         torch.cuda.synchronize()
         self._graph_collectives = (self.sync.enabled and self.sync.backend == "nccl"
@@ -133,6 +143,14 @@
         self._bwd_parts = 1
         self._split_collective = (self.sync.enabled and os.environ.get("RPO_ONE_COLLECTIVE") != "1"
                                   and self.sync.backend == "nccl")
+        self._fused = {"text": False, "img": False}
+        if fused_tail_selected(self.sync.enabled, self.amp, self.use_graph) and not self._joint_bwd:
+            if self._tail_ctl is None:
+                self._tail_ctl = torch.zeros(2, dtype=torch.float32, device=self.device)
+            self._tail_ctl_host = None
+            self._sync_ctl()
+            eng.fused_tail = {"ctl": self._tail_ctl, "momentum": self.optim_cfg.momentum, "wd": self.optim_cfg.weight_decay,
+                              "gs": self.sync.grad_scale}
         if self._joint_bwd:
             self._g_bwd = cap(lambda: eng._joint_backward(B))
         else:
@@ -148,6 +166,7 @@
                     torch.cuda.synchronize()
             if not self._text_ar_in_graph:
                 self._g_text_bwd = cap(eng._text_backward)
+            self._fused["text"] = eng.tail_fused["text"]
             P = int(_xenv("RPO_BWD_PARTS", "1"))
             self._bwd_parts = P if (P > 1 and B % P == 0) else 1
             if self._bwd_parts > 1:
@@ -159,6 +178,8 @@
                 self._ev_parts = [torch.cuda.Event() for _ in range(self._bwd_parts - 1)]
             else:
                 self._g_img_bwd = cap(lambda: eng._image_backward(B))
+                self._fused["img"] = eng.tail_fused["img"]
+        eng.fused_tail = None
         self._ev_fork = torch.cuda.Event()
         self._ev_text_fwd = torch.cuda.Event()
         self._ev_head = torch.cuda.Event()
@@ -254,7 +275,7 @@
             self._g_text_bwd.replay()
             if self._split_collective and not self._text_ar_in_graph:
                 self.sync.all_reduce_sum(self.engine.g_text_flat)
-            if self._early_text:
+            if self._early_text and not self._fused["text"]:
                 self._run_tail("text")
             self._ev_text_bwd.record(side)
             if g_patch is not None:
@@ -316,12 +337,18 @@
                         and next_image.is_contiguous())
                 g_patch = self._patch_graph(next_image)
                 self._patch_tag = (next_image.data_ptr(), next_image._version)
+            if self._fused["text"] or self._fused["img"]:
+                self._sync_ctl()
             self._replay(patch_ready, g_patch)
         else:
             eng.forward_backward(self._image, self._label)
         if self.amp and self._found_inf is None:
             self._found_inf = torch.zeros(2, dtype=torch.int32, device=self.device)
-        self._run_tail("img" if (self.use_graph and getattr(self, "_early_text", False)) else "all")
+        fused = self._fused if self.use_graph else {"text": False, "img": False}
+        need_text = not fused["text"] and not (self.use_graph and getattr(self, "_early_text", False))
+        need_img = not fused["img"]
+        if need_text or need_img:
+            self._run_tail("all" if (need_text and need_img) else ("text" if need_text else "img"))
         self._steps += 1
         eng.params_version += 1
         eng.text_f_version = -1
@@ -374,6 +401,14 @@
     def update_lr(self) -> None:
         self.epoch += 1
         self.lr = lr_at_epoch(self.optim_cfg, self.epoch)
+        if self._tail_ctl is not None:
+            self._sync_ctl()
+
+    def _sync_ctl(self) -> None:
+        want = (float(self.lr), 1.0 if self._steps == 0 else 0.0)
+        if want != self._tail_ctl_host:
+            self._tail_ctl.copy_(torch.tensor(want, dtype=torch.float32), non_blocking=False)
+            self._tail_ctl_host = want
 
     def check_finite(self) -> None:
         eng = self.engine
```

New measurement: 11230, median of 3. About the same (+0.1%).
